# ChicyChen/LOCO-Edit

Measured on AMD Instinct MI355X. Metric: edit-directions/sec (top-5 PMP-Jacobian SVD @256^2) + vT cos-sim vs ref, higher is better.
Workload: dtype bf16x3 (split-bf16 MFMA operands, fp32 accumulate + fp32 storage); 1 GPU; CelebA-HQ DDPM 256x256 top-5 local basis (l_eye-sized mask, L=2400), t=0.6T, 12 power iterations, one GPU; multi_gpu_form=single, probes_total=5, probes_per_gpu=5, kept=5, n_iter=12, mask_L=2400, weights=synthetic seed 0, streams=2

## Files before the change

include/loco_hip_diag.h:

```cpp
#ifndef LOCO_HIP_DIAG_H
#define LOCO_HIP_DIAG_H
#include "loco_hip.h"
#ifdef __cplusplus
extern "C" {
#endif

int  loco_bench_conv(loco_ctx* ctx, int32_t cin, int32_t cout, int32_t H, int32_t W, int32_t B, int32_t mode,
                     int32_t taps, int32_t tile, int32_t iters, float* ms_avg, void* stream);

int64_t loco_debug_tensor(loco_ctx* ctx, const char* name, float* dst, int64_t cap, void* stream);

#ifdef __cplusplus
}
#endif
#endif
```

loco-edit_amd/csrc/conv_bf16.hip:

```cpp
#include "kernels.h"
#include <cstdio>
#include <cstdlib>

namespace loco {

enum : int { PR_BF16X3 = 0, PR_F16 = 1 };
template <int PR, int TAPS, int MODE> void launch_tile_b(const ConvArgs& a, hipStream_t st);
template <int PR, int MODE> void launch_kcat_b(const ConvArgs& a, hipStream_t st);
template <int PR, int MODE> void launch_pair_b(const ConvArgs& a, hipStream_t st);
template <int PR, int MODE> void launch_dual_b(const ConvArgs& a, hipStream_t st);
void launch_conv_gemm(const ConvArgs& a, hipStream_t st);

template <int PR>
static void launch_lowp(const ConvArgs& a, int taps, hipStream_t st) {
#ifdef LOCO_DIAG
    if (a.cot_d && (taps != 1 || a.gemm || a.nsplit > 1 || a.Cin2 > 0 || (a.Cout % conv_bf16_tile_couts(a)) != 0 || a.st_kind == ST_TAN || a.st_kind == ST_COT)) {
        fprintf(stderr, "loco: ConvArgs::cot_d on a launch whose epilogue has no norm-cotangent term (taps %d, gemm %d, nsplit %d, Cout %d, st_kind %d)\n",
                taps, a.gemm, a.nsplit, a.Cout, a.st_kind);
        abort();
    }
#endif
    if constexpr (PR == PR_BF16X3) {
        if (taps == 1 && a.gemm) { launch_conv_gemm(a, st); return; }
    }
    if (taps == 9 && a.Cin2 > 0) {
        if (a.mode == CM_GN_SILU) launch_kcat_b<PR, CM_GN_SILU>(a, st);
        else if (a.mode == CM_GN_GELU) launch_kcat_b<PR, CM_GN_GELU>(a, st);
        else launch_kcat_b<PR, CM_TAN_SILU>(a, st);
        return;
    }
#ifdef LOCO_DIAG
    if constexpr (PR == PR_BF16X3) {
        if (taps == 9 && a.dual) {
            switch (a.mode) {
                case CM_NONE: launch_dual_b<PR, CM_NONE>(a, st); break;
                case CM_GN_SILU: launch_dual_b<PR, CM_GN_SILU>(a, st); break;
                case CM_TAN_SILU: launch_dual_b<PR, CM_TAN_SILU>(a, st); break;
                default: launch_dual_b<PR, CM_COT_SILU>(a, st); break;
            }
            return;
        }
    }
#endif
    if constexpr (PR == PR_BF16X3) {
        if (taps == 9 && a.pair) {
            switch (a.mode) {
                case CM_NONE: launch_pair_b<PR, CM_NONE>(a, st); break;
                case CM_GN_SILU: launch_pair_b<PR, CM_GN_SILU>(a, st); break;
                case CM_TAN_SILU: launch_pair_b<PR, CM_TAN_SILU>(a, st); break;
                default: launch_pair_b<PR, CM_COT_SILU>(a, st); break;
            }
            return;
        }
    }
    if (taps == 9) {
        switch (a.mode) {
            case CM_NONE: launch_tile_b<PR, 9, CM_NONE>(a, st); break;
            case CM_GN_SILU: launch_tile_b<PR, 9, CM_GN_SILU>(a, st); break;
            case CM_GN_GELU: launch_tile_b<PR, 9, CM_GN_GELU>(a, st); break;
            case CM_TAN_SILU: launch_tile_b<PR, 9, CM_TAN_SILU>(a, st); break;
            case CM_COT_SILU: launch_tile_b<PR, 9, CM_COT_SILU>(a, st); break;
            default: launch_tile_b<PR, 9, CM_GN>(a, st); break;
        }
    } else {
        switch (a.mode) {
            case CM_NONE: launch_tile_b<PR, 1, CM_NONE>(a, st); break;
            default: launch_tile_b<PR, 1, CM_GN>(a, st); break;
        }
    }
}
void launch_conv_bf16x3(const ConvArgs& a, int taps, hipStream_t st) { launch_lowp<PR_BF16X3>(a, taps, st); }
void launch_conv_f16(const ConvArgs& a, int taps, hipStream_t st) { launch_lowp<PR_F16>(a, taps, st); }

}
```

loco-edit_amd/csrc/conv_bf16_kernel.h:

```cpp
#pragma once
#include "kernels.h"
#include <cstdlib>
#include <type_traits>

namespace loco {


typedef float f32x16 __attribute__((ext_vector_type(16)));
typedef float f32x4 __attribute__((ext_vector_type(4)));
typedef f32x4 f32x4_u __attribute__((aligned(4)));
typedef float f32x2 __attribute__((ext_vector_type(2)));
typedef f32x2 f32x2_u __attribute__((aligned(4)));
typedef __bf16 bf16x8 __attribute__((ext_vector_type(8)));
typedef _Float16 f16x8 __attribute__((ext_vector_type(8)));
typedef short s16x8 __attribute__((ext_vector_type(8)));

enum : int { PR_BF16X3 = 0, PR_F16 = 1 };

constexpr int BKC = 16;
constexpr bool LIVE_MASK = true;
constexpr bool EARLY_W = true;
constexpr int NDUMMY = 8;

__device__ __forceinline__ float sigmoidf2_(float y) { return __builtin_amdgcn_rcpf(1.0f + __expf(-y)); }

__device__ __forceinline__ int idiv_small(int n, int d) {
    int q = (int)((float)n * __builtin_amdgcn_rcpf((float)d));
    const int r = n - q * d;
    q += (r >= d) ? 1 : ((r < 0) ? -1 : 0);
    return q;
}
__device__ __forceinline__ void idivmod_small(int n, int d, int& q, int& r) { q = idiv_small(n, d); r = n - q * d; }

template <int PR>
__device__ __forceinline__ int rec_off(int p, int q) {
    if constexpr (PR == PR_F16) return p * 32 + ((q ^ ((p >> 3) & 1)) << 4);
    else return p * 64 + ((q ^ ((p >> 2) & 3)) << 4);
}
template <int PR> constexpr int halo_pitch() { return PR == PR_F16 ? 48 : 80; }
template <int PR> constexpr int rec_bytes() { return PR == PR_F16 ? 32 : 64; }
template <int PR>
__device__ __forceinline__ int hrec_off(int p, int q) { return p * halo_pitch<PR>() + (q << 4); }

template <int PR>
__device__ __forceinline__ void cvt2(float a, float b, unsigned& hi, unsigned& lo) {
    if constexpr (PR == PR_F16) {
        _Float16 ha = (_Float16)a, hb = (_Float16)b;
        hi = (unsigned)__builtin_bit_cast(unsigned short, ha) | ((unsigned)__builtin_bit_cast(unsigned short, hb) << 16);
        lo = 0;
    } else {
        typedef float f32x2_ __attribute__((ext_vector_type(2)));
        typedef __bf16 bf16x2_ __attribute__((ext_vector_type(2)));
        hi = __builtin_bit_cast(unsigned, __builtin_convertvector((f32x2_){a, b}, bf16x2_));
        const float ha = __builtin_bit_cast(float, hi << 16), hb = __builtin_bit_cast(float, hi & 0xffff0000u);
        float da = a - ha;
        asm volatile("" : "+v"(da));
        const float db = b - hb;
        lo = __builtin_bit_cast(unsigned, __builtin_convertvector((f32x2_){da, db}, bf16x2_));
    }
}

template <int PR>
__device__ __forceinline__ void split8(const float* v, uint4& hi, uint4& lo) {
    cvt2<PR>(v[0], v[1], hi.x, lo.x);
    cvt2<PR>(v[2], v[3], hi.y, lo.y);
    cvt2<PR>(v[4], v[5], hi.z, lo.z);
    cvt2<PR>(v[6], v[7], hi.w, lo.w);
}

constexpr int max_halo(int NT, int taps, bool s2) {
    if (taps == 1) return NT;
    if (NT >= 128) {
        int th = NT / 32;
        return s2 ? (2 * th + 1) * 65 : (th + 2) * 34;
    }
    return s2 ? 5 * 65 : 4 * 34;
}

constexpr int rs_steps(int n, int lw) { int s = 0; while ((1 << s) < lw && (n >> s) > 1) ++s; return s; }
template <int N, int M, int LW>
__device__ __forceinline__ void rs_reduce(float* av, const int lane) {
    if constexpr (M < LW && N > 1) {
        constexpr int H = N / 2;
        const bool up = (lane & M) != 0;
#pragma unroll
        for (int i = 0; i < H; ++i) {
            const float keep = up ? av[i + H] : av[i];
            const float send = up ? av[i] : av[i + H];
            av[i] = keep + __shfl_xor(send, M, 64);
        }
        rs_reduce<H, M * 2, LW>(av, lane);
    } else if constexpr (M < LW) {
#pragma unroll
        for (int i = 0; i < N; ++i) av[i] += __shfl_xor(av[i], M, 64);
        rs_reduce<N, M * 2, LW>(av, lane);
    }
}

constexpr int EPI_COT1 = 1, EPI_STATS = 2;
template <int WM, int WN, int TM, int TN, int EPI = EPI_STATS, class StageRound>
__device__ __forceinline__ void conv_lowp_epilogue_staged(const ConvArgs& a, StageRound&& stage_round, unsigned char* smem_b, const int co0,
                                                          const int oy0, const int ox0, const int TW, const int tile_id, const int b,
                                                          const int split);
template <int WM, int WN, int TM, int TN>
__device__ __forceinline__ void conv_lowp_epilogue_direct(const ConvArgs& a, f32x16 (&acc)[TM][TN], const int co0, const int oy0,
                                                          const int ox0, const int TW, const int b, const int split);
template <int WM, int WN, int TM, int TN, int EPI = EPI_STATS>
__device__ __forceinline__ void conv_lowp_epilogue(const ConvArgs& a, f32x16 (&acc)[TM][TN], unsigned char* smem_b, const int co0,
                                                   const int oy0, const int ox0, const int TW, const int tile_id, const int b,
                                                   const int split) {
    constexpr int NT = WN * TN * 32;
    const int lane = threadIdx.x & 63, wave = threadIdx.x >> 6;
    const int l31 = lane & 31, khalf = lane >> 5, wm = wave / WN, wn = wave % WN;
    if (co0 + WM * TM * 32 <= a.Cout) {
        conv_lowp_epilogue_staged<WM, WN, TM, TN, EPI>(a, [&](const int h, float* S) {
#pragma unroll
            for (int j = 0; j < TN; ++j)
#pragma unroll
                for (int r = 0; r < 16; ++r)
                    S[(wm * 32 + (r & 3) + 8 * (r >> 2) + 4 * khalf) * NT + (wn * TN + j) * 32 + l31] = acc[h][j][r];
        }, smem_b, co0, oy0, ox0, TW, tile_id, b, split);
        return;
    }
    conv_lowp_epilogue_direct<WM, WN, TM, TN>(a, acc, co0, oy0, ox0, TW, b, split);
}
template <int WM, int WN, int TM, int TN, int EPI, class StageRound>
__device__ __forceinline__ void conv_lowp_epilogue_staged(const ConvArgs& a, StageRound&& stage_round, unsigned char* smem_b, const int co0,
                                                          const int oy0, const int ox0, const int TW, const int tile_id, const int b,
                                                          const int split) {
    constexpr int NTHR = WM * WN * 64;
    constexpr bool COT1 = (EPI & EPI_COT1) != 0, STATS = (EPI & EPI_STATS) != 0;
    constexpr int MT = WM * TM * 32;
    constexpr int NT = WN * TN * 32;
    const int tid = threadIdx.x;
    const int lane = tid & 63;
    const int wave = tid >> 6;
    const int l31 = lane & 31;
    const int khalf = lane >> 5;
    const int wm = wave / WN, wn = wave % WN;
    const long out_plane = (long)a.Hout * a.Wout;
    {
        constexpr int SROWS = WM * 32, NQ = NT / 4, NTASK = (SROWS * NQ) / NTHR;
        static_assert((SROWS * NQ) % NTHR == 0 && (NQ & (NQ - 1)) == 0, "epilogue task split");
        float* const S = reinterpret_cast<float*>(smem_b);
        const bool part = a.nsplit > 1;
        float* const ob = part ? a.partial + (((long)split * a.B + b) * a.Cout) * out_plane : a.out + (long)b * a.out_bs;
        const float* const rb = (!part && a.res) ? a.res + (long)b * a.res_bs : nullptr;
        const float* const b2 = (!part && a.bias2) ? a.bias2 + (long)b * a.bias2_bs : nullptr;
        const float* const b1 = part ? nullptr : a.bias;
        const bool accu = !part && a.accumulate;
        const int twsh = 31 - __builtin_clz((unsigned)TW);
        const bool lin_st = STATS && (a.st_kind == ST_TAN || a.st_kind == ST_COT) && !part;
        const bool lin_cot = a.st_kind == ST_COT;
        const bool cot_ep = COT1 && a.cot_d && !part && !lin_st;
        const float* const cot_db = cot_ep ? a.cot_d + (long)b * a.cot_d_bs : nullptr;
        const f32x2* const cot_tb = cot_ep ? reinterpret_cast<const f32x2*>(a.cot_tc + (long)b * a.cot_tc_bs) : nullptr;
        constexpr int RSTEP = NTHR / NQ;
        static_assert(NTHR % NQ == 0 && 32 % RSTEP == 0, "epilogue task rows");
        const int row0 = tid / NQ, quad0 = tid & (NQ - 1);
        const unsigned pix0 = (unsigned)((oy0 + ((quad0 * 4) >> twsh)) * a.Wout + ox0 + ((quad0 * 4) & (TW - 1)));
        auto co_of = [&](int h, int q) -> int { return co0 + row0 + (((q * RSTEP) >> 5) * TM + h) * 32 + ((q * RSTEP) & 31); };
        auto off_of = [&](int h, int q) -> unsigned {
            const unsigned crow = (unsigned)((((q * RSTEP) >> 5) * TM + h) * 32 + ((q * RSTEP) & 31));
            return (unsigned)(co0 + row0) * (unsigned)out_plane + pix0 + crow * (unsigned)out_plane;
        };
        constexpr int NV = 2 * TM * NTASK;
        float av[STATS ? NV : 1];
#pragma unroll
        for (int h = 0; h < TM; ++h) {
            if (h > 0) {
                asm volatile("s_waitcnt lgkmcnt(0)" ::: "memory");
                __builtin_amdgcn_s_barrier();
            }
            stage_round(h, S);
            f32x4 xs[(STATS || COT1) ? NTASK : 1][2];
            f32x4 cd[COT1 ? NTASK : 1];
            if constexpr (COT1) {
                if (cot_ep) {
#pragma unroll
                    for (int q = 0; q < NTASK; ++q) {
                        const unsigned o = off_of(h, q);
                        cd[q] = *reinterpret_cast<const f32x4*>(cot_db + o);
                        const f32x4* sp4 = reinterpret_cast<const f32x4*>(a.cot_sx + o);
                        xs[q][0] = sp4[0];
                        xs[q][1] = sp4[1];
                    }
                }
            }
            if constexpr (STATS) if (lin_st) {
#pragma unroll
                for (int q = 0; q < NTASK; ++q) {
                    const unsigned o = off_of(h, q);
                    if (lin_cot) {
                        const f32x4* sp4 = reinterpret_cast<const f32x4*>(a.st_sx + o);
                        xs[q][0] = sp4[0];
                        xs[q][1] = sp4[1];
                    } else {
                        xs[q][0] = *reinterpret_cast<const f32x4*>(a.st_x + o);
                    }
                }
            }
            asm volatile("s_waitcnt lgkmcnt(0)" ::: "memory");
            __builtin_amdgcn_s_barrier();
            f32x4 v[NTASK], rv[NTASK];
#pragma unroll
            for (int q = 0; q < NTASK; ++q) v[q] = *reinterpret_cast<const f32x4*>(&S[(q * RSTEP + row0) * NT + quad0 * 4]);
            if (rb || accu) {
#pragma unroll
                for (int q = 0; q < NTASK; ++q) {
                    f32x4 t4 = {0.f, 0.f, 0.f, 0.f};
                    if (rb) t4 = a.res_scale * *reinterpret_cast<const f32x4*>(rb + off_of(h, q));
                    if (accu) t4 += *reinterpret_cast<const f32x4*>(ob + off_of(h, q));
                    rv[q] = t4;
                }
#pragma unroll
                for (int q = 0; q < NTASK; ++q) v[q] += rv[q];
            }
            if constexpr (COT1) {
                if (cot_ep) {
#pragma unroll
                    for (int q = 0; q < NTASK; ++q) {
                        const f32x2 tc2 = cot_tb[co_of(h, q)];
                        const float c1 = tc2[0], c2 = tc2[1];
                        v[q][0] += fmaf(xs[q][0][0], cd[q][0], -fmaf(xs[q][0][1], c2, c1));
                        v[q][1] += fmaf(xs[q][0][2], cd[q][1], -fmaf(xs[q][0][3], c2, c1));
                        v[q][2] += fmaf(xs[q][1][0], cd[q][2], -fmaf(xs[q][1][1], c2, c1));
                        v[q][3] += fmaf(xs[q][1][2], cd[q][3], -fmaf(xs[q][1][3], c2, c1));
                    }
                }
            }
#pragma unroll
            for (int q = 0; q < NTASK; ++q) {
                float add = 0.f;
                if (b1) add += b1[co_of(h, q)];
                if (b2) add += b2[co_of(h, q)];
                v[q] += add;
                __builtin_nontemporal_store(v[q], reinterpret_cast<f32x4*>(ob + off_of(h, q)));
            }
            if constexpr (STATS) if (lin_st) {
#pragma unroll
                for (int q = 0; q < NTASK; ++q) {
                    const f32x4 vv = v[q];
                    float s1, s2;
                    if (!lin_cot) {
                        const f32x4 xv = xs[q][0];
                        s1 = (vv[0] + vv[1]) + (vv[2] + vv[3]);
                        s2 = fmaf(xv[0], vv[0], xv[1] * vv[1]) + fmaf(xv[2], vv[2], xv[3] * vv[3]);
                    } else {
                        const float z0 = xs[q][0][0] * vv[0], z1 = xs[q][0][2] * vv[1], z2 = xs[q][1][0] * vv[2], z3 = xs[q][1][2] * vv[3];
                        s1 = (z0 + z1) + (z2 + z3);
                        s2 = fmaf(xs[q][0][1], z0, xs[q][0][3] * z1) + fmaf(xs[q][1][1], z2, xs[q][1][3] * z3);
                    }
                    av[(h * NTASK + q) * 2] = s1;
                    av[(h * NTASK + q) * 2 + 1] = s2;
                }
            }
            if (STATS && a.st_kind == ST_FWD && !part) {
                const int ntile = (a.Hout * a.Wout) / NT;
                float* const sp = a.st_part + (long)b * a.Cout * ntile * 2;
#pragma unroll
                for (int q = 0; q < NTASK; ++q) {
                    const float pivot = __shfl(v[q][0], lane & ~(NQ - 1) & 63, 64);
                    const float d0 = v[q][0] - pivot, d1 = v[q][1] - pivot, d2 = v[q][2] - pivot, d3 = v[q][3] - pivot;
                    float s1 = (d0 + d1) + (d2 + d3);
                    float s2 = (d0 * d0 + d1 * d1) + (d2 * d2 + d3 * d3);
#pragma unroll
                    for (int m = 1; m < (NQ < 64 ? NQ : 64); m <<= 1) {
                        s1 += __shfl_xor(s1, m, 64);
                        s2 += __shfl_xor(s2, m, 64);
                    }
                    const float m = s1 * (1.0f / NT);
                    const int t = q * NTHR + tid;
                    if ((t & (NQ - 1)) == 0)
                        *reinterpret_cast<f32x2*>(sp + ((long)co_of(h, q) * ntile + tile_id) * 2) = f32x2{pivot + m, s2 - s1 * m};
                }
            }
        }
        if constexpr (STATS) if (lin_st) {
            constexpr int LW = NQ < 64 ? NQ : 64, STEPS = rs_steps(NV, LW), LEFT = NV >> STEPS;
            static_assert((NV & (NV - 1)) == 0, "row sums per lane");
            rs_reduce<NV, 1, LW>(av, lane);
            const int gl = lane & (LW - 1);
            if (gl < (1 << STEPS)) {
                int base = 0;
#pragma unroll
                for (int sb = 0; sb < STEPS; ++sb) base += ((gl >> sb) & 1) * (NV >> (sb + 1));
                const int ntile = (a.Hout * a.Wout) / NT;
                float* const sp = a.st_part + (long)b * a.Cout * ntile * 2;
#pragma unroll
                for (int i = 0; i < LEFT; ++i) {
                    const int idx = base + i, hq = idx >> 1;
                    const int h = hq / NTASK, q = hq - h * NTASK;
                    const int row = (q * NTHR + tid) / NQ;
                    const int co = co0 + ((row >> 5) * TM + h) * 32 + (row & 31);
                    sp[((long)co * ntile + tile_id) * 2 + (idx & 1)] = av[i];
                }
            }
        }
    }
}
template <int WM, int WN, int TM, int TN>
__device__ __forceinline__ void conv_lowp_epilogue_direct(const ConvArgs& a, f32x16 (&acc)[TM][TN], const int co0, const int oy0,
                                                          const int ox0, const int TW, const int b, const int split) {
    const int lane = threadIdx.x & 63, wave = threadIdx.x >> 6;
    const int l31 = lane & 31, khalf = lane >> 5, wm = wave / WN, wn = wave % WN;
    const long out_plane = (long)a.Hout * a.Wout;
    const bool full_co = false;
#pragma unroll
    for (int j = 0; j < TN; ++j) {
        int p = (wn * TN + j) * 32 + l31;
        int ty = p / TW, tx = p - ty * TW;
        int oy = oy0 + ty, ox = ox0 + tx;
        const unsigned pix = (unsigned)(oy * a.Wout + ox);
#pragma unroll
        for (int i = 0; i < TM; ++i) {
            const int cob = co0 + (wm * TM + i) * 32 + 4 * khalf;
            if (a.nsplit > 1) {
                float* pb = a.partial + (((long)split * a.B + b) * a.Cout) * out_plane;
#pragma unroll
                for (int r = 0; r < 16; ++r) {
                    int co = cob + (r & 3) + 8 * (r >> 2);
                    if (full_co || co < a.Cout) pb[(long)co * out_plane + pix] = acc[i][j][r];
                }
            } else {
                float* ob = a.out + (long)b * a.out_bs;
                const float* rb = a.res ? a.res + (long)b * a.res_bs : nullptr;
                const float* b2 = a.bias2 ? a.bias2 + (long)b * a.bias2_bs : nullptr;
                if (rb || a.accumulate) {
                    float rv[16];
#pragma unroll
                    for (int r = 0; r < 16; ++r) {
                        int co = cob + (r & 3) + 8 * (r >> 2);
                        const bool ok = full_co || co < a.Cout;
                        const long off = (long)(ok ? co : a.Cout - 1) * out_plane + pix;
                        float t = 0.f;
                        if (rb) t = a.res_scale * rb[off];
                        if (a.accumulate) t += ob[off];
                        rv[r] = t;
                    }
#pragma unroll
                    for (int r = 0; r < 16; ++r) {
                        int co = cob + (r & 3) + 8 * (r >> 2);
                        if (!(full_co || co < a.Cout)) continue;
                        float v = acc[i][j][r] + rv[r];
                        if (a.bias) v += a.bias[co];
                        if (b2) v += b2[co];
                        __builtin_nontemporal_store(v, &ob[(long)co * out_plane + pix]);
                    }
                } else {
#pragma unroll
                    for (int r = 0; r < 16; ++r) {
                        int co = cob + (r & 3) + 8 * (r >> 2);
                        if (!(full_co || co < a.Cout)) continue;
                        float v = acc[i][j][r];
                        if (a.bias) v += a.bias[co];
                        if (b2) v += b2[co];
                        __builtin_nontemporal_store(v, &ob[(long)co * out_plane + pix]);
                    }
                }
            }
        }
    }
}

template <int WM, int WN, int TM, int TN, int RPW>
__device__ __forceinline__ void conv_lowp_epilogue_rounds(const ConvArgs& a, f32x16 (&acc)[TM][TN], float* const S, const int co0,
                                                          const int oy0, const int ox0, const int TW, const int tile_id, const int b) {
    constexpr int NTHR = WM * WN * 64, NT = WN * TN * 32, NQ = NT / 4;
    constexpr int SROWS = WM * RPW, NTASK = (SROWS * NQ) / NTHR, NRB = RPW / 8;
    static_assert((RPW == 8 || RPW == 16 || RPW == 32) && (SROWS * NQ) % NTHR == 0 && NQ == 64, "round geometry");
    const int tid = threadIdx.x, lane = tid & 63, wave = tid >> 6;
    const int l31 = lane & 31, khalf = lane >> 5;
    const int wm = wave / WN, wn = wave % WN;
    const unsigned out_plane = (unsigned)(a.Hout * a.Wout);
    float* const ob = a.out + (long)b * a.out_bs;
    const float* const rb = a.res ? a.res + (long)b * a.res_bs : nullptr;
    const float* const b2 = a.bias2 ? a.bias2 + (long)b * a.bias2_bs : nullptr;
    const bool accu = a.accumulate != 0;
    const int twsh = TW == 32 ? 5 : (TW == 16 ? 4 : 3);
    const int ntile = (a.Hout * a.Wout) / NT;
    float* const sp = (a.st_kind == ST_FWD) ? a.st_part + (long)b * a.Cout * ntile * 2 : nullptr;
#pragma unroll
    for (int h = 0; h < TM; ++h) {
#pragma unroll
        for (int g0 = 0; g0 < 4; g0 += NRB) {
#pragma unroll
            for (int j = 0; j < TN; ++j)
#pragma unroll
                for (int g = 0; g < NRB; ++g)
#pragma unroll
// ... 1015 lines not shown
```

loco-edit_amd/csrc/conv_plan.hip:

```cpp
#include "kernels.h"
#include <cstdio>
#include <cstdlib>

namespace loco {

constexpr int BKC = 16;
constexpr int BKF = 8;

static const int kMT[7] = {128, 128, 32, 64, 128, 128, 128}, kNT[7] = {128, 64, 128, 64, 256, 256, 128};

static int env_int(const char* name, int dflt) {
    const char* e = getenv(name);
    return e ? atoi(e) : dflt;
}
static int diag_switch(const char* name) {
#ifdef LOCO_DIAG
    return env_int(name, 0);
#else
    (void)name;
    return 0;
#endif
}

static int pick_tile(int Cout, int HW) {
    if (HW >= 128) return Cout > 32 ? 0 : 2;
    return Cout > 64 ? 1 : 3;
}

static int conv_pick_nsplit(int Cin, int Cout, int Hout, int Wout, int B) {
    const int t = pick_tile(Cout, Hout * Wout);
    long blocks = (long)((Hout * Wout) / kNT[t]) * ((Cout + kMT[t] - 1) / kMT[t]) * B;
    int nchunks = (Cin + BKF - 1) / BKF;
    if (blocks >= 384 || nchunks < 8) return 1;
    int want = (int)((512 + blocks - 1) / blocks);
    int maxs = nchunks / 4;
    if (want > maxs) want = maxs;
    if (want > 32) want = 32;
    return want < 1 ? 1 : want;
}

static int conv_bf16_pick_tile(int Cout, int HW, int B, int tile_override) {
    if (B <= 1 && HW <= 1024 && HW >= 64 && (Cout % 64) == 0) return 3;
    int t = pick_tile(Cout, HW);
    if (t == 0 && HW >= 256) {
        if (tile_override >= 0) return tile_override;
        return 5;
    }
    return t;
}

constexpr int kTile0MaxHW = 65536;

static int bf16_tile_of(const ConvArgs& a, int tile_override = -1) {
    static const bool two_per_cu = diag_switch("LOCO_CONV_2WG") != 0;
    int tile = conv_bf16_pick_tile(a.Cout, a.Hout * a.Wout, a.B, tile_override);
    if (tile == 4) tile = 5;
    if (tile == 5 && a.taps == 1 && !a.gemm && a.B >= 2 && a.Hout * a.Wout <= kTile0MaxHW) return 0;
    if (tile == 5 && two_per_cu && a.taps == 9 && a.stride == 1 && !a.upsample && !a.zins && (a.Cin % BKC) == 0 &&
        a.in_padded && a.pad == 1 && a.Wout >= 32) return 6;
    if (a.stride == 2 && tile == 5) tile = 0;
    return tile;
}
static int tile_for(const ConvArgs& a, int prec, int tile_override) {
    return prec ? bf16_tile_of(a, tile_override) : pick_tile(a.Cout, a.Hout * a.Wout);
}
static int conv_bf16_tile_pixels(const ConvArgs& a) { return a.gemm ? 256 : kNT[a.tile]; }
int conv_bf16_tile_couts(const ConvArgs& a) { return a.gemm ? 64 * a.gemm_tm : kMT[a.tile]; }

static int conv_bf16_pick_nsplit(int Cin, int Cout, int Hout, int Wout, int B, int chip_share, int taps, int lanes) {
    const int HW = Hout * Wout;
    int t = conv_bf16_pick_tile(Cout, HW, B, -1);
    if (t == 4) t = 5;
    if (taps == 1 && t == 5 && B >= 2 && HW <= kTile0MaxHW) t = 0;
    long blocks = (long)(HW / kNT[t]) * ((Cout + kMT[t] - 1) / kMT[t]) * B;
    int nchunks = (Cin + BKC - 1) / BKC;
    int target = chip_share > 1 ? 256 / chip_share : (lanes == 2 ? 240 : 256);
    if (target < 32) target = 32;
    if (blocks >= target / 2 || nchunks < 8) return 1;
    int want = (int)(target / blocks);
    int maxs = nchunks / 4;
    if (want > maxs) want = maxs;
    if (want > 32) want = 32;
    return want < 1 ? 1 : want;
}

static bool conv_lowp_can_kcat(const ConvArgs& a) {
    static const bool on = env_int("LOCO_KCAT", 1) != 0;
    return on && a.Cin2 > 0 && a.nsplit == 1 && bf16_tile_of(a) == 5 && a.stride == 1 && !a.upsample && !a.zins && a.pad == 1 &&
           (a.Cin % BKC) == 0 && (a.Cin2 % BKC) == 0 && a.in_padded &&
           (a.mode == CM_GN_SILU || a.mode == CM_GN_GELU || a.mode == CM_TAN_SILU);
}
static bool conv_lowp_can_fuse_stats(const ConvArgs& a) {
    return a.nsplit <= 1 && !a.gemm && (a.Cout % conv_bf16_tile_couts(a)) == 0;
}

static bool conv_pair_ok(const ConvArgs& a) {
    static const bool on = env_int("LOCO_CONV_PAIR", 1) != 0;
    if (!on || a.Hout * a.Wout < 16384 || a.taps != 9 || a.Cin2 > 0 || a.nsplit != 1 || a.stride != 1 || a.upsample || a.zins ||
        a.pad != 1 || !a.in_padded || (a.Cin % (2 * BKC)) != 0 || (a.Cout % 128) != 0 || (a.Wout % 32) != 0 || (a.Hout % 8) != 0 ||
        a.pers_groups || a.dual)
        return false;
    if (!(a.mode == CM_NONE || a.mode == CM_GN_SILU || a.mode == CM_TAN_SILU || a.mode == CM_COT_SILU)) return false;
    return a.tile == 5;
}

static bool conv_dual_ok(const ConvArgs& a) {
    static const bool on = diag_switch("LOCO_CONV_DUAL") != 0;
    if (!on || a.taps != 9 || a.Cin2 > 0 || a.nsplit != 1 || a.stride != 1 || a.upsample || a.zins || a.pad != 1 || (a.Cin % BKC) != 0 ||
        !a.in_padded || a.Wout < 32 || (a.Wout % 32) != 0 || (a.Hout % 8) != 0 || (a.Cout % 128) != 0 || a.B < 2 || a.cot_d)
        return false;
    if (!(a.mode == CM_NONE || a.mode == CM_GN_SILU || a.mode == CM_TAN_SILU || a.mode == CM_COT_SILU)) return false;
    if (a.tile != 5) return false;
    const long units = (long)((a.Hout * a.Wout) / 256) * (a.Cout / 128) * (a.B / 2);
    return units >= 192;
}

static ConvArgs conv_shift_batch(const ConvArgs& a, int nb) {
    ConvArgs t = a;
    t.B = a.B - nb;
    t.in += (long)nb * a.in_bs; t.out += (long)nb * a.out_bs;
    if (t.prim) t.prim += (long)nb * a.prim_bs;
    if (t.bias2) t.bias2 += (long)nb * a.bias2_bs;
    if (t.res) t.res += (long)nb * a.res_bs;
    if (t.sc) { t.sc += (long)nb * a.scsh_bs; t.sh += (long)nb * a.scsh_bs; }
    if (t.mr) t.mr += (long)nb * a.mr_bs;
    if (t.tst) t.tst += (long)nb * a.tst_bs;
    if (t.tc) t.tc += (long)nb * a.tc_bs;
    if (t.in2) t.in2 += (long)nb * a.in2_bs;
    if (t.cot_d) { t.cot_d += (long)nb * a.cot_d_bs; t.cot_tc += (long)nb * a.cot_tc_bs; }
    if (t.st_part) t.st_part += (long)nb * a.Cout * ((a.Hout * a.Wout) / conv_bf16_tile_pixels(a)) * 2;
    return t;
}

static void conv_pers_plan(ConvArgs& a) {
    a.pers_groups = 0;
    static const int on = diag_switch("LOCO_CONV_PERS");
    if (!on || a.taps != 9 || a.Cin2 > 0 || a.nsplit != 1 || a.stride != 1 || a.upsample || a.zins || a.pad != 1 || !a.in_padded ||
        (a.Cin % (2 * BKC)) != 0 || (a.Cout % 128) != 0 || a.B < 2 || a.cot_d || bf16_tile_of(a) != 5)
        return;
    if (!(a.mode == CM_NONE || a.mode == CM_GN_SILU || a.mode == CM_GN_GELU ||
          (on == 2 && (a.mode == CM_TAN_SILU || a.mode == CM_COT_SILU)))) return;
    const long wg0 = (long)((a.Hout * a.Wout) / 256) * (a.Cout / 128);
    int G = wg0 >= 256 ? 1 : (int)(256 / wg0);
    if (G > a.B) G = a.B;
    const int per = (a.B + G - 1) / G;
    if (per < 2 || a.B * 10 < G * per * 8 || wg0 * G < 192) return;
    a.pers_groups = G;
}

static void conv_gemm_plan(ConvArgs& a) {
    static const bool on = env_int("LOCO_CONV_GEMM", 1) != 0;
    a.gemm = 0;
    const long HW = (long)a.Hout * a.Wout;
    if (!on || a.stride != 1 || a.upsample || a.zins || (a.Cin % BKC) != 0 || a.Cin < 320 || (HW % 256) != 0 || (a.Wout % 16) != 0 ||
        a.Cout < 128 || !a.partial || a.Cin2 > 0 || !(a.mode == CM_NONE || a.mode == CM_GN) || a.cot_d)
        return;
    {
        const int TW = a.Wout < 32 ? a.Wout : 32;
        if ((256 % TW) != 0 || (a.Wout % TW) != 0 || (a.Hout % (256 / TW)) != 0) return;
    }
    static const int all_shapes = env_int("LOCO_GEMM_ALL", 0);
    if (!all_shapes && !(a.Cout >= 640 && (a.Cout >= 4 * a.Cin || a.Cin >= 2560))) return;
    const int pad256 = (a.Cout + 255) / 256 * 256;
    const int tm = (pad256 * 10 <= a.Cout * 11) ? 4 : 2;
    const int mt = 64 * tm;
    const long tiles = (HW / 256) * ((a.Cout + mt - 1) / mt) * a.B;
    const size_t rec_floats = (size_t)a.B * a.Cin * HW;
    int ns = 1;
    if (tiles < 192) {
        const int nchunks = a.Cin / BKC;
        ns = (int)((256 + tiles - 1) / tiles);
        if (ns > 8) ns = 8;
        while (ns > 1 && nchunks / ns < 8) --ns;
        while (ns > 1 && (size_t)ns * a.B * a.Cout * HW + rec_floats > a.partial_floats) --ns;
    }
    if ((ns > 1 ? (size_t)ns * a.B * a.Cout * HW : 0) + rec_floats > a.partial_floats) return;
    a.gemm = 1; a.gemm_tm = tm; a.nsplit = ns;
}

void conv_plan_family(ConvArgs& a, int prec) {
    if (prec == 1 && a.taps == 1) conv_gemm_plan(a);
    if (prec == 1 && a.taps == 9) conv_pers_plan(a);
}

int conv_plan_parts(ConvArgs& a, int prec, int tile_override, ConvArgs parts[2]) {
    a.dual = 0;
    a.tile = tile_for(a, prec, tile_override);
    a.pair = 0;
    parts[0] = a;
    int n = 1;
    if (prec == 1 && a.taps == 9 && conv_dual_ok(a)) {
        parts[0].B = a.B & ~1;
        parts[0].dual = 1;
        if (a.B & 1) {
            parts[1] = conv_shift_batch(a, a.B - 1);
            parts[1].pers_groups = 0;
            n = 2;
        }
    }
    for (int i = 0; i < n; ++i) {
        ConvArgs& p = parts[i];
        p.tile = tile_for(p, prec, tile_override);
        p.pair = prec == 1 && conv_pair_ok(p);
    }
    return n;
}

static bool short_tail(long per_probe, int B) {
    const long total = per_probe * B, r = total % 256;
    return total > 256 && r > 0 && r <= 160;
}

static int tail_split(const ConvArgs& a, size_t partial_floats, int* split) {
    const long per_probe = (long)((a.Hout * a.Wout) / conv_bf16_tile_pixels(a)) * ((a.Cout + 127) / 128);
    const long r = per_probe * a.B % 256;
    if (!short_tail(per_probe, a.B) || per_probe <= 0 || r % per_probe != 0 || r / per_probe >= a.B) return 0;
    int s = (int)(256 / r);
    if (s > 4) s = 4;
    const int nchunks = (a.Cin + 15) / 16;
    while (s > 1 && nchunks / s < 4) --s;
    const size_t one = (size_t)(r / per_probe) * a.Cout * a.Hout * a.Wout;
    while (s > 1 && (size_t)s * one > partial_floats) --s;
    *split = s;
    return s > 1 ? (int)(r / per_probe) : 0;
}

static int stats_route(const ConvEnv& e, const StatAsk* q, bool want, ConvArgs& x, int s0, int B, int* keep_ntile) {
    if (!q || q->kind == ST_NONE) return SR_NONE;
    const int alone = q->norm ? SR_ALONE : SR_NONE;
    if (!want) return alone;
    if (x.nsplit > 1) return !q->norm ? SR_NONE : ((x.Hout * x.Wout) % 4 == 0 ? SR_SPLITK : SR_ALONE);
    const int ntile = (x.Hout * x.Wout) / conv_bf16_tile_pixels(x);
    const size_t need = (size_t)x.B * x.Cout * ntile * 2;
    const int epi = q->norm ? SR_EPI : SR_KEEP;
    const bool kept = q->keep && s0 == 0 && x.B == B && need <= q->keep_floats;
    if (q->kind == ST_FWD && conv_lowp_can_fuse_stats(x) && (kept || (q->norm && need <= e.stpart_floats))) {
        x.st_part = kept ? q->keep : e.stpart; x.st_kind = ST_FWD;
        if (kept) *keep_ntile = ntile;
        return epi;
    }
    const bool cot_cache = q->kind == ST_COT && q->norm && q->sx;
    if ((q->kind == ST_TAN || cot_cache) && e.fuse_lin && !x.cot_d && conv_lowp_can_fuse_stats(x) && !x.pers_groups &&
        !conv_dual_ok(x)) {
        const size_t lane_off = (size_t)e.lane_s0 * (q->keep_floats / e.max_batch);
        const bool keptl = q->kind == ST_TAN && q->keep && s0 == 0 && x.B == B && lane_off + need <= q->keep_floats;
        if (keptl || (q->norm && need <= e.stpart_floats)) {
            x.st_part = keptl ? q->keep + lane_off : e.stpart; x.st_kind = q->kind; x.st_x = q->prim;
            if (q->kind == ST_COT) x.st_sx = q->sx;
            if (keptl) *keep_ntile = ntile;
            return epi;
        }
    }
    return alone;
}

static ConvLaunch plan_launch(const ConvEnv& e, const StatAsk* q, bool want, const ConvArgs& x, int s0, int B, int* keep_ntile) {
    ConvLaunch l;
    l.args = x;
    l.s0 = s0;
    l.args.tile = tile_for(x, e.prec, -1);
    l.stats = stats_route(e, q, want, l.args, s0, B, keep_ntile);
    if (l.stats == SR_EPI || l.stats == SR_KEEP) l.ntile = (x.Hout * x.Wout) / conv_bf16_tile_pixels(l.args);
    l.nparts = conv_plan_parts(l.args, e.prec, -1, l.parts);
    return l;
}

ConvPlan plan_conv(const ConvEnv& e, const ConvArgs& a0, int taps, const StatAsk* q, const ConvArgs* sc) {
    ConvPlan p;
    ConvArgs a = a0;
    a.taps = taps;
    a.dual = 0; a.pers_groups = 0; a.gemm = 0;
    if (sc) {
        ConvArgs t = a;
        t.nsplit = e.prec >= 1 ? conv_bf16_pick_nsplit(a.Cin, a.Cout, a.Hout, a.Wout, a.B, e.chip_share, 9, e.lanes) : 2;
        t.in2 = sc->in; t.in2_bs = sc->in_bs; t.Cin2 = sc->Cin;
        const long per_probe = (long)((a.Hout * a.Wout) / 256) * ((a.Cout + 127) / 128);
        if (e.prec >= 1 && taps == 9 && !short_tail(per_probe, a.B) && !a.bias2 && conv_lowp_can_kcat(t)) {
            a.in2 = sc->in; a.in2_bs = sc->in_bs; a.Cin2 = sc->Cin; a.in2_padded = sc->in_padded;
            a.wb2 = e.prec == 2 ? sc->wh : sc->wb;
            a.bias2 = sc->bias; a.bias2_bs = 0;
            a.res = nullptr;
        } else {
            p.sc_first = true;
            a.res = sc->out; a.res_bs = sc->out_bs;
        }
    }
    if (e.prec == 2) a.wb = a.wh;
    a.no_deep = e.deep1 ? 0 : 1;
    a.nsplit = e.prec >= 1 ? conv_bf16_pick_nsplit(a.Cin, a.Cout, a.Hout, a.Wout, a.B, e.chip_share, taps, e.lanes)
                           : conv_pick_nsplit(a.Cin, a.Cout, a.Hout, a.Wout, a.B);
    if (a.cot_d) {
        ConvArgs t = a;
        t.tile = bf16_tile_of(t);
        const long per_probe = (long)((a.Hout * a.Wout) / conv_bf16_tile_pixels(t)) * ((a.Cout + 127) / 128);
        p.cot = e.prec >= 1 && taps == 1 && a.nsplit == 1 && !short_tail(per_probe, a.B) && conv_lowp_can_fuse_stats(t);
        if (!p.cot) { a.cot_d = nullptr; a.cot_d_bs = 0; a.cot_sx = nullptr; a.cot_tc = nullptr; a.cot_tc_bs = 0; }
    }
    while (a.nsplit > 1 && (size_t)a.nsplit * a.B * a.Cout * a.Hout * a.Wout > e.partial_floats) a.nsplit >>= 1;
    if (a.nsplit < 1) a.nsplit = 1;
    a.partial = e.partial;
    a.partial_floats = e.partial_floats;
    conv_plan_family(a, e.prec);
    a.tile = tile_for(a, e.prec, -1);
    int split = 1;
    const int tail = e.prec >= 1 && a.nsplit == 1 && a.B >= 2 && !a.gemm && !a.pers_groups ? tail_split(a, e.partial_floats, &split) : 0;
    const bool want = q && q->kind != ST_NONE && e.prec >= 1 && e.fuse_stats;
    if (!tail) {
        p.l[0] = plan_launch(e, q, want, a, 0, a.B, &p.keep_ntile);
        return p;
    }
    const bool per_part = want && q->norm && (q->kind == ST_FWD || (e.fuse_lin && (a.Hout * a.Wout) % 4 == 0));
    p.stats_all = !per_part && q && q->kind != ST_NONE && q->norm;
    const StatAsk* ql = per_part ? q : nullptr;
    const int nb = a.B - tail;
    ConvArgs m = a, t = conv_shift_batch(a, nb);
    m.B = nb;
    t.nsplit = split;
    p.nl = 2;
    p.l[0] = plan_launch(e, ql, want, m, 0, a.B, &p.keep_ntile);
    p.l[1] = plan_launch(e, ql, want, t, nb, a.B, &p.keep_ntile);
    return p;
}

const char* conv_variant_name(const ConvArgs& a, int taps, int prec) {
    static const char* tiles[6] = {"2,2,2,2", "4,1,1,2", "1,4,1,1", "2,2,1,1", "2,2,2,4", "2,4,2,2"};
    static char names[3][2][6][6][56];
    static char others[5][3][6][40];
    const int mode = (a.mode < 0 || a.mode > 5) ? 2 : a.mode;
    const char* other = nullptr;
    int k = 0, v = mode;
    if (prec && taps == 9 && a.Cin2 > 0) other = prec == 1 ? "conv_kcat_bf16x3<2,4,2,2,%d>" : "conv_kcat_f16<2,4,2,2,%d>";
    else if (prec == 1 && taps == 1 && a.gemm) { k = 1; other = "conv_gemm_bf16x3<%d>"; v = a.gemm_tm; }
    else if (prec == 1 && taps == 9 && a.pers_groups > 0 && !a.dual) { k = 2; other = "conv_pers_bf16x3<9,2,4,2,2,%d>"; }
    else if (prec == 1 && taps == 9 && a.pair) { k = 3; other = "conv_pair_bf16x3<%d>"; }
    else if (prec == 1 && taps == 9 && a.dual) { k = 4; other = "conv_dual_bf16x3<%d>"; }
    if (other) {
        char* n = others[k][prec][v];
        if (!n[0]) snprintf(n, 40, other, v);
        return n;
    }
    int t = a.tile == 6 ? 0 : a.tile;
    if (t < 0 || t > 5) t = 0;
    int m = mode;
    if (taps != 9 && m != CM_NONE) m = CM_GN;
    if (!prec && m == CM_GN_GELU) m = CM_GN_SILU;
    char* n = names[prec][taps == 9 ? 0 : 1][t][m];
    static const char* kn[3] = {"conv_mfma_f32", "conv_mfma_bf16x3", "conv_mfma_f16"};
    if (!n[0]) snprintf(n, 56, "%s<%d,%s,%d>", kn[prec], taps, tiles[t], m);
    return n;
}

}
```

loco-edit_amd/csrc/engine.hip:

```cpp
#include <hip/hip_runtime.h>

#include <algorithm>
#include <array>
#include <cmath>
#include <cstdio>
#include <cstdlib>
#include <cstring>
#include <map>
#include <memory>
#include <thread>
#include <atomic>
#include <string>
#include <vector>

#include "../../include/loco_hip.h"
#ifdef LOCO_DIAG
#include "../../include/loco_hip_diag.h"
#endif
#include "kernels.h"
#include "program.h"

using namespace loco;


#define HIPCHK(ctx, call)                                                                    \
    do {                                                                                     \
        hipError_t e_ = (call);                                                              \
        if (e_ != hipSuccess) {                                                              \
            (ctx)->err = std::string(#call) + ": " + hipGetErrorString(e_);                  \
            return -1;                                                                       \
        }                                                                                    \
    } while (0)

namespace {

struct ConvP {
    float* wf = nullptr;
    float* wd = nullptr;
    float* wbf = nullptr;
    float* wbd = nullptr;
    float* whf = nullptr;
    float* whd = nullptr;
    float* bias = nullptr;
    int cin = 0, cout = 0, taps = 0;
};
struct NormW { float* gamma = nullptr; float* beta = nullptr; };

struct OpWeights {
    ConvP c1, c2, nin, qkvc, proj, conv;
    ConvP xqc, xproj;
    ConvP pj_in, to_out1, to_out2, ff1, ff2, pj_out;
    NormW g1, g2, gx;
    float *xkw = nullptr, *xkb = nullptr, *xvw = nullptr, *xvb = nullptr;
    float *xng = nullptr, *xnb = nullptr;
    float *lng[3] = {nullptr, nullptr, nullptr}, *lnb[3] = {nullptr, nullptr, nullptr};
    long tproj_off = 0;
};
struct Weights {
    std::vector<OpWeights> op;
    float *freq = nullptr, *td0w = nullptr, *td0b = nullptr, *td1w = nullptr, *td1b = nullptr;
    float *tp_w = nullptr, *tp_b = nullptr;
    long tproj_total = 0;
    double flops = 0.0;
};

struct Tens : TensPlan {
    float* keep = nullptr; size_t keep_floats = 0; int keep_ntile = 0;
};
struct NormP : NormPlan, NormW {
    bool ready = false;
};
struct Op : OpPlan, OpWeights {
    NormP n1, n2, nx;
    float *xK = nullptr, *xV = nullptr;
};

struct HostParam { std::vector<float> data; std::vector<int64_t> shape; bool loaded = false; };

}


struct loco_ctx {
    loco_unet_cfg cfg;
    std::string err;
    std::map<std::string, HostParam> params;
    bool finalized = false;

    std::shared_ptr<const Program> prog;
    std::shared_ptr<Weights> wts;
    std::vector<Tens> tens;
    std::vector<Op> ops;


    float *arenaP = nullptr, *arenaT = nullptr;
    float *statsP = nullptr, *statsT = nullptr;
    double* red = nullptr;
    bool fuse_cot = true;
    float *stpart = nullptr, *stpart2 = nullptr;
    size_t stpart_floats = 0;
    bool fuse_stats = true;
    bool fuse_xattn = true;
    bool deep1 = true;
    bool flash_attn = true;
    float* attn_delta = nullptr;
    float* partial = nullptr;
    size_t partial_floats = 0;
    const float* bench_out = nullptr; int64_t bench_out_count = 0;
    float *tact = nullptr, *tproj = nullptr;
    float* eps_buf = nullptr;
    float* gx0 = nullptr;
    float* ge = nullptr;
    float* tmpA = nullptr;
    double *G = nullptr, *Q = nullptr, *W = nullptr, *gscratch = nullptr;
    float* alphas = nullptr;
    float* ctx_colbias = nullptr;
    bool has_ctx = false;
    float* cond_add = nullptr;
    float* ctx_norm = nullptr;
    bool has_cond = false;
    float2* sxcache = nullptr;
    int prec = 0;
    std::vector<float*> owned;
    size_t bytes = 0;

    bool primal_ok = false;
    float p_cv = 0.f, p_ce = 0.f;
    uint8_t* mask = nullptr;
    bool has_mask = false;
    uint8_t* mask2 = nullptr;
    bool has_mask2 = false;
    int mask2_from = 0;
    int* mask_idx = nullptr;
    int* mask_L_dev = nullptr;
    long mask_L = 0;
    hipStream_t mask_stream = nullptr;
    int primal_B = 0;
    hipEvent_t ev0 = nullptr, ev1 = nullptr;
    int n_streams = 1;
    hipStream_t st2 = nullptr;
    hipStream_t st2_user = nullptr;
    hipEvent_t ev_fork = nullptr, ev_join = nullptr;
    double* red2 = nullptr;
    struct FwdGraph { hipGraph_t graph = nullptr; hipGraphExec_t exec = nullptr; int calls = 0; };
    std::map<int, FwdGraph> fwd_graphs;
    bool graph_on = false;
    bool gemm_lowp = true;
    unsigned char* gemm_ws[2] = {nullptr, nullptr}; size_t gemm_ws_bytes[2] = {0, 0}; int lane = 0;
    loco_ctx* weights_of = nullptr;
    int forks = 0;
    bool zombie = false;
    bool fuse_lin = true;
    int lanes_active = 1;
    int lane_s0 = 0;
    int chip_share = 1;
    hipStream_t cap_st = nullptr;
    float* xin_buf = nullptr;
    float* t_dev = nullptr;
    bool prof_on = false;
    struct ProfRec { const char* name; double flops; hipEvent_t e0, e1; int cin, cout, h, b, ns, mode, taps; };
    bool prof_shapes = false;
    std::vector<ProfRec> prof;
    std::vector<hipEvent_t> ev_pool;
    size_t ev_used = 0;
    hipEvent_t next_event() {
        if (ev_used == ev_pool.size()) {
            hipEvent_t e; (void)hipEventCreate(&e); ev_pool.push_back(e);
        }
        return ev_pool[ev_used++];
    }
};

namespace {

template <typename T>
int dalloc(loco_ctx* c, T** p, size_t count) {
    void* q = nullptr;
    HIPCHK(c, hipMalloc(&q, count * sizeof(T)));
    *p = reinterpret_cast<T*>(q);
    c->owned.push_back(reinterpret_cast<float*>(q));
    c->bytes += count * sizeof(T);
    return 0;
}

inline float eps_of(const loco_ctx* c, const NormP& n) { return n.eps > 0.f ? n.eps : c->cfg.gn_eps; }


int upload(loco_ctx* c, float** dst, const std::vector<float>& h) {
    if (dalloc(c, dst, h.size() ? h.size() : 1)) return -1;
    HIPCHK(c, hipMemcpy(*dst, h.data(), h.size() * sizeof(float), hipMemcpyHostToDevice));
    return 0;
}

static inline uint16_t f2bf(float f) {
    uint32_t u; std::memcpy(&u, &f, 4);
    u += 0x7FFFu + ((u >> 16) & 1u);
    return (uint16_t)(u >> 16);
}
static inline float bf2f(uint16_t h) {
    uint32_t u = (uint32_t)h << 16; float f; std::memcpy(&f, &u, 4); return f;
}
template <typename F>
static void parallel_for(int n, size_t work, F fn) {
    unsigned nt = std::thread::hardware_concurrency();
    if (nt > 16) nt = 16;
    if ((int)nt > n) nt = (unsigned)n;
    if (nt <= 1 || work < ((size_t)1 << 18)) { for (int i = 0; i < n; ++i) fn(i); return; }
    std::atomic<int> next{0};
    std::vector<std::thread> th;
    for (unsigned t = 0; t < nt; ++t)
        th.emplace_back([&]() { int i; while ((i = next.fetch_add(1)) < n) fn(i); });
    for (auto& t : th) t.join();
}

template <typename F>
static std::vector<float> build_records(int nin, int nout, int taps, F get) {
    int nch = (nin + 15) / 16, noutP = (nout + 31) & ~31;
    std::vector<uint16_t> rec((size_t)nch * taps * noutP * 32, 0);
    parallel_for(nch, (size_t)nin * nout * taps, [&](int ck) {
        for (int t = 0; t < taps; ++t)
            for (int o = 0; o < nout; ++o) {
                uint16_t* r = rec.data() + (((size_t)ck * taps + t) * noutP + o) * 32;
                int sw = (o >> 2) & 3;
                for (int k = 0; k < 16; ++k) {
                    int i = ck * 16 + k;
                    float v = (i < nin) ? get(o, i, t) : 0.f;
                    uint16_t h = f2bf(v);
                    uint16_t l = f2bf(v - bf2f(h));
                    int qh = (k >> 3) ^ sw, ql = (2 + (k >> 3)) ^ sw;
                    r[qh * 8 + (k & 7)] = h;
                    r[ql * 8 + (k & 7)] = l;
                }
            }
    });
    std::vector<float> out(rec.size() / 2);
    std::memcpy(out.data(), rec.data(), rec.size() * 2);
    return out;
}

template <typename F>
static std::vector<float> build_records_f16(int nin, int nout, int taps, F get) {
    int nch = (nin + 15) / 16, noutP = (nout + 31) & ~31;
    std::vector<_Float16> rec((size_t)nch * taps * noutP * 16, (_Float16)0.f);
    parallel_for(nch, (size_t)nin * nout * taps, [&](int ck) {
        for (int t = 0; t < taps; ++t)
            for (int o = 0; o < nout; ++o) {
                _Float16* r = rec.data() + (((size_t)ck * taps + t) * noutP + o) * 16;
                int sw = (o >> 3) & 1;
                for (int k = 0; k < 16; ++k) {
                    int i = ck * 16 + k;
                    float v = (i < nin) ? get(o, i, t) : 0.f;
                    r[((k >> 3) ^ sw) * 8 + (k & 7)] = (_Float16)v;
                }
            }
    });
    std::vector<float> out(rec.size() / 2);
    std::memcpy(out.data(), rec.data(), rec.size() * 2);
    return out;
}

int make_conv(loco_ctx* c, const std::vector<const HostParam*>& ws, const std::vector<const HostParam*>& bs,
              ConvP* out, int row_limit = -1) {
    int cin = (int)ws[0]->shape[1], k = ws[0]->shape.size() > 2 ? (int)ws[0]->shape[2] : 1;
    int taps = ws[0]->shape.size() == 4 ? k * k : k;
    int cout = 0;
    for (auto* w : ws) cout += (int)w->shape[0];
    if (row_limit > 0 && ws.size() == 1 && row_limit < cout) cout = row_limit;
    int coutP = (cout + 31) & ~31, cinP = (cin + 31) & ~31;
    std::vector<float> wf((size_t)cin * taps * coutP, 0.f), wd((size_t)cout * taps * cinP, 0.f), bias(cout);
    int co0 = 0;
    for (size_t wi = 0; wi < ws.size(); ++wi) {
        const HostParam* w = ws[wi];
        int co_n = (int)w->shape[0];
        if (co_n > cout - co0) co_n = cout - co0;
        parallel_for(co_n, (size_t)co_n * cin * taps, [&](int co) {
            for (int ci = 0; ci < cin; ++ci)
                for (int t = 0; t < taps; ++t)
                    wd[((size_t)(co0 + co) * taps + (taps - 1 - t)) * cinP + ci] = w->data[((size_t)co * cin + ci) * taps + t];
        });
        parallel_for(cin, (size_t)co_n * cin * taps, [&](int ci) {
            for (int t = 0; t < taps; ++t)
                for (int co = 0; co < co_n; ++co)
                    wf[((size_t)ci * taps + t) * coutP + co0 + co] = w->data[((size_t)co * cin + ci) * taps + t];
        });
        for (int co = 0; co < co_n; ++co) bias[co0 + co] = bs[wi]->data[co];
        co0 += co_n;
    }
    out->cin = cin; out->cout = cout; out->taps = taps;
    if (upload(c, &out->wf, wf) || upload(c, &out->wd, wd) || upload(c, &out->bias, bias)) return -1;
    auto fwd = [&](int o, int i, int t) { return wf[((size_t)i * taps + t) * coutP + o]; };
    auto dgr = [&](int o, int i, int t) { return wd[((size_t)i * taps + t) * cinP + o]; };
    std::vector<float> rf = build_records(cin, cout, taps, fwd);
    std::vector<float> rd = build_records(cout, cin, taps, dgr);
    if (upload(c, &out->wbf, rf) || upload(c, &out->wbd, rd)) return -1;
    std::vector<float> hf = build_records_f16(cin, cout, taps, fwd);
    std::vector<float> hd = build_records_f16(cout, cin, taps, dgr);
    if (upload(c, &out->whf, hf) || upload(c, &out->whd, hd)) return -1;
    return 0;
}
int make_conv1(loco_ctx* c, const std::string& name, ConvP* out, int row_limit = -1) {
    return make_conv(c, {&c->params[name + ".weight"]}, {&c->params[name + ".bias"]}, out, row_limit);
}
int make_conv1_scaled(loco_ctx* c, const std::string& name, ConvP* out, float s) {
    if (s == 1.f) return make_conv1(c, name, out);
    HostParam w = c->params[name + ".weight"], b = c->params[name + ".bias"];
    for (float& v : w.data) v *= s;
    for (float& v : b.data) v *= s;
    return make_conv(c, {&w}, {&b}, out);
}
int make_norm(loco_ctx* c, const std::string& name, NormW* n) {
    if (upload(c, &n->gamma, c->params[name + ".weight"].data)) return -1;
    if (upload(c, &n->beta, c->params[name + ".bias"].data)) return -1;
    return 0;
}

int bind_weights(loco_ctx* c) {
    const Weights& W = *c->wts;
    for (size_t i = 0; i < c->ops.size(); ++i) {
        Op& v = c->ops[i];
        static_cast<OpWeights&>(v) = W.op[i];
        static_cast<NormW&>(v.n1) = v.g1; static_cast<NormW&>(v.n2) = v.g2; static_cast<NormW&>(v.nx) = v.gx;
    }
    if (dalloc(c, &c->tact, (size_t)c->cfg.ch * 4) || dalloc(c, &c->tproj, (size_t)(W.tproj_total > 0 ? W.tproj_total : 1))) return -1;
    c->finalized = true;
    return 0;
}

int finalize_params(loco_ctx* c) {
    if (c->finalized) return 0;
    for (const ParamDecl& d : c->prog->params)
        if (!c->params[d.name].loaded) { c->err = "parameter not loaded: " + d.name; return -1; }
    Weights& W = *c->wts;
    const loco_unet_cfg& cfg = c->cfg;
    int temb_ch = cfg.ch * 4;
    const bool adm = cfg.arch == 1;
    const std::string te0 = adm ? "time_embed.0" : "temb.dense.0", te1 = adm ? "time_embed.2" : "temb.dense.1";
    if (cfg.arch < 2) {
        if (upload(c, &W.td0w, c->params[te0 + ".weight"].data)) return -1;
        if (upload(c, &W.td0b, c->params[te0 + ".bias"].data)) return -1;
        if (upload(c, &W.td1w, c->params[te1 + ".weight"].data)) return -1;
        if (upload(c, &W.td1b, c->params[te1 + ".bias"].data)) return -1;
    }
    {
        int half = cfg.ch / 2;
        std::vector<float> f(half);
        for (int i = 0; i < half; ++i) {
            float x;
            if (adm) x = ((float)(-std::log(10000.0)) * (float)i) / (float)half;
            else x = (float)i * (float)(-(std::log(10000.0) / (double)(half - 1)));
            f[i] = (float)std::exp((double)x);
        }
        if (upload(c, &W.freq, f)) return -1;
    }
    std::vector<float> tpw, tpb;
    for (size_t oi = 0; oi < W.op.size(); ++oi) {
        const OpPlan& op = c->prog->ops[oi];
        OpWeights& ow = W.op[oi];
        switch (op.kind) {
            case OP_CONV_IN: case OP_CONV: if (make_conv1(c, op.pn_conv, &ow.conv)) return -1; break;
            case OP_RES: {
                if (make_norm(c, op.pn_n1, &ow.g1) || make_norm(c, op.pn_n2, &ow.g2)) return -1;
                if (make_conv1(c, op.pn_c1, &ow.c1) || make_conv1_scaled(c, op.pn_c2, &ow.c2, c->prog->res_scale)) return -1;
                if (op.has_nin && make_conv1_scaled(c, op.pn_skip, &ow.nin, c->prog->res_scale)) return -1;
                if (!op.has_temb) break;
                ow.tproj_off = (long)tpb.size();
                auto& w = c->params[op.pn_emb + ".weight"].data;
                auto& b = c->params[op.pn_emb + ".bias"].data;
                tpw.insert(tpw.end(), w.begin(), w.end());
                tpb.insert(tpb.end(), b.begin(), b.end());
                break;
            }
            case OP_ATTN: {
                if (make_norm(c, op.pn_n1, &ow.g1)) return -1;
                if (adm) {
                    if (make_conv1(c, op.pn_qkv, &ow.qkvc)) return -1;
                } else if (make_conv(c, {&c->params[op.name + ".q.weight"], &c->params[op.name + ".k.weight"],
                                         &c->params[op.name + ".v.weight"]},
                                     {&c->params[op.name + ".q.bias"], &c->params[op.name + ".k.bias"],
                                      &c->params[op.name + ".v.bias"]}, &ow.qkvc)) return -1;
                if (make_conv1(c, op.pn_proj, &ow.proj)) return -1;
                if (op.added_kv) {
                    const int C = c->tens[op.in].C, NH = op.heads, CH = C / NH, D = c->cfg.context_dim;
                    const HostParam& w = c->params[op.name + ".encoder_kv.weight"];
                    const HostParam& b = c->params[op.name + ".encoder_kv.bias"];
                    std::vector<float> kw((size_t)C * D), vw((size_t)C * D), kb(C), vb(C);
                    for (int h = 0; h < NH; ++h)
                        for (int i = 0; i < CH; ++i) {
                            const size_t rk = (size_t)h * 2 * CH + i, rv = rk + CH, r = (size_t)h * CH + i;
                            std::copy(w.data.begin() + rk * D, w.data.begin() + (rk + 1) * D, kw.begin() + r * D);
                            std::copy(w.data.begin() + rv * D, w.data.begin() + (rv + 1) * D, vw.begin() + r * D);
                            kb[r] = b.data[rk]; vb[r] = b.data[rv];
                        }
                    if (upload(c, &ow.xkw, kw) || upload(c, &ow.xkb, kb) || upload(c, &ow.xvw, vw) || upload(c, &ow.xvb, vb) ||
                        upload(c, &ow.xng, c->params[op.name + ".norm_encoder.weight"].data) ||
                        upload(c, &ow.xnb, c->params[op.name + ".norm_encoder.bias"].data)) return -1;
                }
                if (op.has_x) {
                    const std::string x = op.name + ".xattn";
                    if (make_norm(c, x + ".norm", &ow.gx) || make_conv1(c, x + ".q", &ow.xqc) ||
                        make_conv1(c, x + ".proj_out", &ow.xproj)) return -1;
                    if (upload(c, &ow.xkw, c->params[x + ".k.weight"].data) || upload(c, &ow.xkb, c->params[x + ".k.bias"].data) ||
                        upload(c, &ow.xvw, c->params[x + ".v.weight"].data) || upload(c, &ow.xvb, c->params[x + ".v.bias"].data))
                        return -1;
                }
                break;
            }
            case OP_DOWN: case OP_UP: if (make_conv1(c, op.pn_conv, &ow.conv)) return -1; break;
            case OP_XFMR: {
                const int C = c->tens[op.in].C, NH = op.heads, CH = C / NH;
                const std::string b = op.name + ".transformer_blocks.0";
                HostParam zb; zb.shape = {8 * C}; zb.data.assign((size_t)8 * C, 0.f);
                auto nobias = [&](const std::string& w, ConvP* out) { return make_conv(c, {&c->params[w + ".weight"]}, {&zb}, out); };
                if (make_norm(c, op.pn_n1, &ow.g1) || make_conv1(c, op.name + ".proj_in", &ow.pj_in) ||
                    make_conv1(c, op.name + ".proj_out", &ow.pj_out)) return -1;
                const char* lnn[3] = {".norm1", ".norm2", ".norm3"};
                for (int i = 0; i < 3; ++i)
                    if (upload(c, &ow.lng[i], c->params[b + lnn[i] + ".weight"].data) ||
                        upload(c, &ow.lnb[i], c->params[b + lnn[i] + ".bias"].data)) return -1;
                {
                    HostParam w; w.shape = {3 * C, C}; w.data.resize((size_t)3 * C * C);
                    const char* nm[3] = {".attn1.to_q.weight", ".attn1.to_k.weight", ".attn1.to_v.weight"};
                    for (int which = 0; which < 3; ++which) {
                        const std::vector<float>& src = c->params[b + nm[which]].data;
                        for (int h = 0; h < NH; ++h)
                            for (int j = 0; j < CH; ++j)
                                std::memcpy(&w.data[((size_t)(h * 3 + which) * CH + j) * C], &src[(size_t)(h * CH + j) * C], (size_t)C * 4);
                    }
                    if (make_conv(c, {&w}, {&zb}, &ow.qkvc)) return -1;
                }
                if (make_conv1(c, b + ".attn1.to_out.0", &ow.to_out1) || nobias(b + ".attn2.to_q", &ow.xqc) ||
                    make_conv1(c, b + ".attn2.to_out.0", &ow.to_out2) || make_conv1(c, b + ".ff.net.0.proj", &ow.ff1) ||
                    make_conv1(c, b + ".ff.net.2", &ow.ff2)) return -1;
                std::vector<float> z0((size_t)C, 0.f);
                if (upload(c, &ow.xkw, c->params[b + ".attn2.to_k.weight"].data) || upload(c, &ow.xkb, z0) ||
                    upload(c, &ow.xvw, c->params[b + ".attn2.to_v.weight"].data) || upload(c, &ow.xvb, z0)) return -1;
                break;
            }
            case OP_OUT:
                if (make_norm(c, op.pn_n1, &ow.g1) || make_conv1(c, op.pn_conv, &ow.conv, cfg.out_ch)) return -1;
                break;
        }
    }
    W.tproj_total = (long)tpb.size();
    if (upload(c, &W.tp_w, tpw) || upload(c, &W.tp_b, tpb)) return -1;
    double fl = 0.0;
    for (size_t oi = 0; oi < W.op.size(); ++oi) {
        const OpPlan& op = c->prog->ops[oi];
        const OpWeights& ow = W.op[oi];
        auto convf = [&](const ConvP& p, int H, int W) { fl += 2.0 * p.cin * p.cout * p.taps * (double)H * W; };
        const Tens& to = c->tens[op.out];
        switch (op.kind) {
            case OP_CONV_IN: case OP_CONV: case OP_DOWN: case OP_UP: case OP_OUT: convf(ow.conv, to.H, to.W); break;
            case OP_RES:
                convf(ow.c1, to.H, to.W); convf(ow.c2, to.H, to.W);
                if (op.has_nin) convf(ow.nin, to.H, to.W);
                break;
            case OP_XFMR: {
                for (const ConvP* p : {&ow.pj_in, &ow.qkvc, &ow.to_out1, &ow.xqc, &ow.to_out2, &ow.ff1, &ow.ff2, &ow.pj_out}) convf(*p, to.H, to.W);
                double T = (double)to.H * to.W;
                fl += 2.0 * 2.0 * T * T * to.C + 2.0 * 2.0 * T * c->cfg.context_len * to.C;
                break;
            }
            case OP_ATTN: {
                convf(ow.qkvc, to.H, to.W); convf(ow.proj, to.H, to.W);
                double T = (double)to.H * to.W;
                fl += 2.0 * 2.0 * T * T * to.C;
                if (op.has_x) {
                    convf(ow.xqc, to.H, to.W); convf(ow.xproj, to.H, to.W);
                    fl += 2.0 * 2.0 * T * c->cfg.context_len * to.C;
                }
                break;
            }
        }
    }
    W.flops = fl;
    for (auto& kv : c->params) { std::vector<float>().swap(kv.second.data); }
    return bind_weights(c);
}

struct Pass {
    loco_ctx* c;
    hipStream_t st;
    int B;
    float* arena;
    float* stats;
    float* T(int id) const { return arena + c->tens[id].off; }
    long bs() const { return c->prog->per_sample; }
};

static void drop_graphs(loco_ctx* c) {
    for (auto& kv : c->fwd_graphs) {
        if (kv.second.exec) (void)hipGraphExecDestroy(kv.second.exec);
        if (kv.second.graph) (void)hipGraphDestroy(kv.second.graph);
    }
    c->fwd_graphs.clear();
}
inline unsigned char* gemm_ws_get(loco_ctx* c, size_t need, hipStream_t st) {
    const int l = c->lane;
    if (c->gemm_ws_bytes[l] >= need) return c->gemm_ws[l];
    hipStreamCaptureStatus cs = hipStreamCaptureStatusNone;
    if (hipStreamIsCapturing(st, &cs) != hipSuccess || cs != hipStreamCaptureStatusNone) return nullptr;
    if (c->gemm_ws[l]) {
        (void)hipDeviceSynchronize();
        drop_graphs(c);
        (void)hipFree(c->gemm_ws[l]);
        c->bytes -= c->gemm_ws_bytes[l];
        c->gemm_ws[l] = nullptr; c->gemm_ws_bytes[l] = 0;
    }
    void* p = nullptr;
    if (hipMalloc(&p, need) != hipSuccess) { (void)hipGetLastError(); return nullptr; }
    c->gemm_ws[l] = static_cast<unsigned char*>(p); c->gemm_ws_bytes[l] = need; c->bytes += need;
    return c->gemm_ws[l];
}
inline bool attn_gemm_rec(const loco_ctx* c, const GemmArgs& g) { return c->prec >= 1 && c->gemm_lowp && gemm_rec_eligible(g); }
inline void attn_gemm(loco_ctx* c, const GemmArgs& g, hipStream_t st) {
    if (attn_gemm_rec(c, g)) {
        if (unsigned char* ws = gemm_ws_get(c, gemm_rec_ws_bytes(g), st)) { launch_gemm_rec(g, ws, st); return; }
    }
    if (c->prec >= 1 && c->gemm_lowp && gemm_prefers_bf16x3(g)) launch_gemm_bf16x3(g, st); else launch_gemm(g, st);
}

void conv_defaults(ConvArgs& a) {
    std::memset(&a, 0, sizeof(a));
    a.stride = 1; a.pad = 1; a.nsplit = 1; a.mode = CM_NONE; a.res_scale = 1.f;
}

struct NS { float *sc, *sh, *mr, *tst, *tc; };
NS nstats(const loco_ctx* c, float* base, const NormP& n) {
    NS s;
    s.sc = base + n.soff; s.sh = s.sc + n.C; s.mr = s.sh + n.C; s.tst = s.mr + 2 * c->cfg.gn_groups;
    s.tc = s.tst + 2 * c->cfg.gn_groups;
    return s;
}

struct StatReq {
    int kind = ST_NONE;
    NormP* n = nullptr;
    float* stats = nullptr;
    const float* prim = nullptr;
    const float* ss_scale = nullptr; const float* ss_shift = nullptr;
    float* keep = nullptr; size_t keep_floats = 0; int* keep_ntile = nullptr;
};

void stats_standalone(loco_ctx* c, const StatReq& rq, const float* x, long xbs, int B, int HW, int s0, hipStream_t st) {
    const NormP& n = *rq.n;
    const long SB = c->prog->stats_per_sample;
    const int G = c->cfg.gn_groups;
    if (rq.kind == ST_FWD) {
        NS s = nstats(c, rq.stats + (long)s0 * SB, n);
        launch_gn_stats(x, xbs, B, n.C, HW, G, eps_of(c, n), n.gamma, n.beta, s.mr, s.sc, s.sh, SB, c->red, st, rq.ss_scale,
                        rq.ss_shift);
    } else {
        NS sp = nstats(c, c->statsP, n);
        NS stt = nstats(c, rq.stats + (long)s0 * SB, n);
        launch_gn_tstats(x, xbs, rq.prim, 0, B, n.C, HW, G, sp.sc, sp.sh, sp.mr, 0, 0, rq.kind == ST_TAN ? 0 : 1, stt.tst,
                         stt.tc, SB, c->red, st, c->cfg.act);
    }
}

bool run_conv(loco_ctx* c, const ConvArgs& a0, int taps, hipStream_t st, const StatReq* rq = nullptr,
              const ConvArgs* second = nullptr) {
    const size_t span = (size_t)c->cfg.max_batch * c->prog->per_sample;
    auto padded = [&](const float* p) { return (p >= c->arenaP && p < c->arenaP + span) || (p >= c->arenaT && p < c->arenaT + span); };
    ConvArgs a = a0, sc;
    a.act = c->cfg.act;
    if (a.mode == CM_GN_SILU && c->cfg.act == ACT_GELU) a.mode = CM_GN_GELU;
    a.in_padded = padded(a.in);
    if (second) { sc = *second; sc.in_padded = padded(sc.in); }
    ConvEnv e;
    e.prec = c->prec; e.chip_share = c->chip_share; e.lanes = c->lanes_active; e.lane_s0 = c->lane_s0;
    e.partial = c->partial; e.partial_floats = c->partial_floats; e.stpart = c->stpart; e.stpart_floats = c->stpart_floats;
    e.fuse_stats = c->fuse_stats; e.fuse_lin = c->fuse_lin; e.deep1 = c->deep1; e.max_batch = c->cfg.max_batch;
    StatAsk q;
    if (rq) {
        q.kind = rq->kind; q.norm = rq->n != nullptr; q.prim = rq->prim; q.keep = rq->keep; q.keep_floats = rq->keep_floats;
        if (rq->n && rq->n->sx_off >= 0 && c->sxcache) q.sx = c->sxcache + rq->n->sx_off;
    }
    const ConvPlan p = plan_conv(e, a, taps, rq ? &q : nullptr, second ? &sc : nullptr);
    if (p.sc_first) run_conv(c, *second, 1, st);
    if (rq && rq->kind != ST_NONE && rq->n) rq->n->ready = true;
    if (rq && rq->keep_ntile) *rq->keep_ntile = p.keep_ntile;
    const int HWo = a.Hout * a.Wout, Gn = c->cfg.gn_groups;
    const long SBs = c->prog->stats_per_sample;
    auto timed = [&](const char* name, double flops, const ConvArgs& y, auto&& launch) {
        loco_ctx::ProfRec r;
        if (c->prof_on) {
            r.name = name; r.flops = flops;
            r.cin = y.Cin; r.cout = y.Cout; r.h = y.Hout; r.b = y.B; r.ns = y.nsplit; r.mode = y.mode; r.taps = taps;
            r.e0 = c->next_event(); r.e1 = c->next_event();
            (void)hipEventRecord(r.e0, st);
        }
        launch();
        if (c->prof_on) { (void)hipEventRecord(r.e1, st); c->prof.push_back(r); }
    };
    for (int li = 0; li < p.nl; ++li) {
        const ConvLaunch& l = p.l[li];
        const ConvArgs& x = l.args;
        for (int pi = 0; pi < l.nparts; ++pi) {
            const ConvArgs& y = l.parts[pi];
            double flops = 2.0 * (y.Cin * taps + y.Cin2) * y.Cout * (double)y.Hout * y.Wout * y.B;
            if (y.zins) flops *= 0.25;
            timed(c->prof_on ? conv_variant_name(y, taps, c->prec) : nullptr, flops, y, [&] {
                if (c->prec == 1) launch_conv_bf16x3(y, taps, st);
                else if (c->prec == 2) launch_conv_f16(y, taps, st);
                else launch_conv(y, taps, st);
            });
        }
        if (x.nsplit > 1) {
            timed("conv_splitk_reduce", 0.0, x, [&] {
                if (l.stats != SR_SPLITK) { launch_conv_splitk_reduce(x, st); return; }
                const NormP& n = *rq->n;
                NS sp = nstats(c, c->statsP, n);
                NS so = nstats(c, rq->stats + (long)l.s0 * SBs, n);
                launch_conv_splitk_reduce_stats(x, rq->kind, Gn, eps_of(c, n), n.gamma, n.beta, so.mr, so.sc, so.sh, SBs, rq->ss_scale,
                                                rq->ss_shift, rq->prim, sp.sc, sp.sh, sp.mr, so.tst, so.tc, SBs, c->red, st);
            });
        }
        if (l.stats == SR_ALONE) stats_standalone(c, *rq, x.out, x.out_bs, x.B, HWo, l.s0, st);
        if (l.stats == SR_EPI) {
            const NormP& n = *rq->n;
            NS so = nstats(c, rq->stats + (long)l.s0 * SBs, n);
            if (rq->kind != ST_FWD) {
                NS sp = nstats(c, c->statsP, n);
                launch_gn_lin_fused_finalize(rq->kind, x.st_part, n.C, l.ntile, nullptr, 0, x.B, n.C, HWo, Gn, sp.mr, so.tst, so.tc,
                                             SBs, st);
            } else {
                launch_gn_fused_finalize(x.st_part, l.ntile, x.B, n.C, HWo, Gn, eps_of(c, n), n.gamma, n.beta, so.mr, so.sc, so.sh,
                                         SBs, rq->ss_scale, rq->ss_shift, st);
            }
        }
    }
    if (p.stats_all) stats_standalone(c, *rq, a.out, a.out_bs, a.B, HWo, 0, st);
    return p.cot;
}

inline void setw(ConvArgs& a, const ConvP& p, bool dgrad) {
    a.w = dgrad ? p.wd : p.wf;
    a.wb = dgrad ? (const void*)p.wbd : (const void*)p.wbf;
    a.wh = dgrad ? (const void*)p.whd : (const void*)p.whf;
}

NormP* consumer_norm(loco_ctx* c, int tid) {
    const Tens& t = c->tens[tid];
    if (t.cons_op < 0) return nullptr;
    Op& op = c->ops[t.cons_op];
    return t.cons_norm == 2 ? &op.nx : &op.n1;
}
StatReq req_fwd(NormP* n, float* stats, const float* ss_scale = nullptr, const float* ss_shift = nullptr) {
    StatReq r;
    if (n) { r.kind = ST_FWD; r.n = n; r.stats = stats; r.ss_scale = ss_scale; r.ss_shift = ss_shift; }
    return r;
}
StatReq req_lin(loco_ctx* c, int kind, NormP* n, const float* prim) {
    StatReq r;
    if (n) { r.kind = kind; r.n = n; r.stats = c->statsT; r.prim = prim; }
    return r;
}
void clear_ready(loco_ctx* c) {
    for (auto& op : c->ops) op.n1.ready = op.n2.ready = op.nx.ready = false;
    for (auto& t : c->tens) t.keep_ntile = 0;
}
StatReq req_fwd_of(loco_ctx* c, int tid, float* stats) {
    StatReq r = req_fwd(consumer_norm(c, tid), stats);
    Tens& t = c->tens[tid];
    if (t.cat_of >= 0 && t.keep) {
        r.kind = ST_FWD; r.stats = stats;
        r.keep = t.keep; r.keep_floats = t.keep_floats; r.keep_ntile = &t.keep_ntile;
    }
    return r;
}
bool cat_fused_stats(loco_ctx* c, const NormP& n, int tid, float* stats, int B, hipStream_t st) {
    const Tens& q = c->tens[tid];
    if (q.cat_a < 0 || c->prec < 1 || !c->fuse_stats) return false;
    const Tens& A = c->tens[q.cat_a];
    const Tens& Bt = c->tens[q.cat_b];
    if (A.keep_ntile <= 0 || Bt.keep_ntile <= 0) return false;
    NS s = nstats(c, stats, n);
    launch_gn_fused_finalize_cat(A.keep, A.C, A.keep_ntile, Bt.keep, Bt.keep_ntile, B, q.C, q.H * q.W, c->cfg.gn_groups,
                                 eps_of(c, n), n.gamma, n.beta, s.mr, s.sc, s.sh, c->prog->stats_per_sample, st);
    return true;
}

bool cat_fused_tstats(loco_ctx* c, const NormP& n, int tid, int B, hipStream_t st) {
    const Tens& q = c->tens[tid];
    if (q.cat_a < 0 || c->prec < 1 || !c->fuse_stats || !c->fuse_lin) return false;
    const Tens& A = c->tens[q.cat_a];
    const Tens& Bt = c->tens[q.cat_b];
    if (A.keep_ntile <= 0 || Bt.keep_ntile <= 0) return false;
    NS sp = nstats(c, c->statsP, n);
    NS stt = nstats(c, c->statsT, n);
    const size_t MB = c->cfg.max_batch;
    launch_gn_lin_fused_finalize(ST_TAN, A.keep + c->lane_s0 * (A.keep_floats / MB), A.C, A.keep_ntile,
                                 Bt.keep + c->lane_s0 * (Bt.keep_floats / MB), Bt.keep_ntile, B, q.C, q.H * q.W,
                                 c->cfg.gn_groups, sp.mr, stt.tst, stt.tc, c->prog->stats_per_sample, st);
    return true;
}

void gn_forward_stats(const Pass& p, const NormP& n, const float* x, long xbs, int HW) {
    NS s = nstats(p.c, p.stats, n);
    launch_gn_stats(x, xbs, p.B, n.C, HW, p.c->cfg.gn_groups, eps_of(p.c, n), n.gamma, n.beta, s.mr, s.sc, s.sh,
                    p.c->prog->stats_per_sample, p.c->red, p.st);
}


struct XA {
    loco_ctx* c; const Op* op; hipStream_t st; int B; int C, T, NH, CH, Lp;
    float scale;
};
XA xa_of(loco_ctx* c, const Op& op, int B, hipStream_t st) {
    XA x; x.c = c; x.op = &op; x.st = st; x.B = B;
    const Tens& t = c->tens[op.in];
    x.C = t.C; x.T = t.H * t.W; x.NH = op.heads; x.CH = x.C / x.NH; x.Lp = c->prog->ctx_Lp;
    x.scale = 1.0f / std::sqrt((float)x.CH);
    return x;
}
void xa_scores(const XA& x, const float* X, long x_bs, const float* K, float* S, long s_bs, float alpha, bool mask) {
    GemmArgs g; std::memset(&g, 0, sizeof(g));
    g.A = X; g.sam = 1; g.sak = x.T; g.sab = x_bs; g.sah = (long)x.CH * x.T;
    g.Bm = K; g.sbk = x.Lp; g.sbn = 1; g.sbb = 0; g.sbh = (long)x.CH * x.Lp;
    g.C = S; g.scm = x.Lp; g.scn = 1; g.scb = s_bs; g.sch = (long)x.T * x.Lp;
    g.M = x.T; g.N = x.Lp; g.K = x.CH; g.batch = x.B; g.batch2 = x.NH; g.alpha = alpha; g.beta = 0.f;
    g.colbias = mask ? x.c->ctx_colbias : nullptr;
    launch_gemm(g, x.st);
}
void xa_values(const XA& x, const float* K, const float* S, long s_bs, float* O, long o_bs) {
    GemmArgs g; std::memset(&g, 0, sizeof(g));
    g.A = K; g.sam = x.Lp; g.sak = 1; g.sab = 0; g.sah = (long)x.CH * x.Lp;
    g.Bm = S; g.sbk = 1; g.sbn = x.Lp; g.sbb = s_bs; g.sbh = (long)x.T * x.Lp;
    g.C = O; g.scm = x.T; g.scn = 1; g.scb = o_bs; g.sch = (long)x.CH * x.T;
    g.M = x.CH; g.N = x.T; g.K = x.Lp; g.batch = x.B; g.batch2 = x.NH; g.alpha = 1.f; g.beta = 0.f;
    launch_gemm(g, x.st);
}
bool xa_fused(const XA& x, int kind, const float* X, long x_bs, const float* K1, const float* K2, float* P, long p_bs,
              float* O, long o_bs) {
    loco_ctx* c = x.c;
    if (!c->fuse_xattn || !xattn_fused_supported(x.T, x.CH, c->cfg.context_len, x.Lp)) return false;
    XAttnArgs a; std::memset(&a, 0, sizeof(a));
    a.T = x.T; a.NH = x.NH; a.B = x.B; a.CH = x.CH; a.L = c->cfg.context_len; a.Lp = x.Lp; a.fwd = kind == 0;
    a.alpha = x.scale; a.X = X; a.x_bs = x_bs; a.K1 = K1; a.K2 = K2; a.P = P; a.p_bs = p_bs; a.O = O; a.o_bs = o_bs;
    launch_xattn_fused(a, x.st);
    return true;
}
void xa_conv1x1(loco_ctx* c, const ConvP& w, bool dgrad, const float* in, long in_bs, float* out, long out_bs, int C, int H,
                int W, int B, const float* res, long res_bs, bool with_bias, hipStream_t st, const StatReq* rq = nullptr) {
    ConvArgs a; conv_defaults(a);
    a.in = in; a.in_bs = in_bs; a.Cin = C; a.Hin = H; a.Win = W;
    setw(a, w, dgrad); a.pad = 0;
    if (with_bias) a.bias = w.bias;
    a.res = res; a.res_bs = res_bs;
    a.out = out; a.out_bs = out_bs; a.Cout = C; a.Hout = H; a.Wout = W; a.B = B;
    run_conv(c, a, 1, st, rq);
}

struct SA { loco_ctx* c; const Op* op; int B, T, NH, CH; hipStream_t st; };
void sa_forward(const SA& s, float* ar) {
    loco_ctx* c = s.c;
    const long PS = c->prog->per_sample, HS = 3L * s.CH * s.T, SS = (long)s.T * s.T;
    float* q = ar + c->tens[s.op->qkv].off; float* k = q + (long)s.CH * s.T; float* v = k + (long)s.CH * s.T;
    float* S = ar + c->tens[s.op->S].off; float* o = ar + c->tens[s.op->o].off;
    GemmArgs g; std::memset(&g, 0, sizeof(g));
    g.A = q; g.sam = 1; g.sak = s.T; g.sab = PS; g.sah = HS;
    g.Bm = k; g.sbk = s.T; g.sbn = 1; g.sbb = PS; g.sbh = HS;
    g.C = S; g.scm = s.T; g.scn = 1; g.scb = PS; g.sch = SS;
    g.M = s.T; g.N = s.T; g.K = s.CH; g.batch = s.B; g.batch2 = s.NH; g.alpha = 1.0f / std::sqrt((float)s.CH); g.beta = 0.f;
    attn_gemm(c, g, s.st);
    launch_softmax_rows(S, (long)s.NH * s.T, s.T, s.st, s.B, PS);
    GemmArgs h; std::memset(&h, 0, sizeof(h));
    h.A = v; h.sam = s.T; h.sak = 1; h.sab = PS; h.sah = HS;
    h.Bm = S; h.sbk = 1; h.sbn = s.T; h.sbb = PS; h.sbh = SS;
    h.C = o; h.scm = s.T; h.scn = 1; h.scb = PS; h.sch = (long)s.CH * s.T;
    h.M = s.CH; h.N = s.T; h.K = s.T; h.batch = s.B; h.batch2 = s.NH; h.alpha = 1.f; h.beta = 0.f;
    attn_gemm(c, h, s.st);
}
void sa_tangent(const SA& s) {
    loco_ctx* c = s.c;
    const int T = s.T, CH = s.CH, NH = s.NH, B = s.B;
    const long PS = c->prog->per_sample, HS = 3L * CH * T, SS = (long)T * T;
    float* q = c->arenaP + c->tens[s.op->qkv].off; float* k = q + (long)CH * T; float* v = k + (long)CH * T;
    float* dq = c->arenaT + c->tens[s.op->qkv].off; float* dk = dq + (long)CH * T; float* dv = dk + (long)CH * T;
    float* SP = c->arenaP + c->tens[s.op->S].off; float* ST = c->arenaT + c->tens[s.op->S].off;
    float* oP = c->arenaP + c->tens[s.op->o].off; float* oT = c->arenaT + c->tens[s.op->o].off;
    const float scale = 1.0f / std::sqrt((float)CH);
    if (c->flash_attn && c->prec >= 1 && attn_flash_supported(T, CH)) {
        AttnFlashArgs fa; std::memset(&fa, 0, sizeof(fa));
        fa.ws = reinterpret_cast<unsigned char*>(c->partial); fa.ws_bytes = c->partial_floats * sizeof(float);
        fa.T = T; fa.NH = NH; fa.B = B; fa.CH = CH; fa.scale = scale; fa.q = q; fa.k = k; fa.v = v; fa.hs = HS; fa.P = SP; fa.o = oP;
        fa.dq = dq; fa.dk = dk; fa.dv = dv; fa.bs_d = PS; fa.out = oT; fa.bs_out = PS;
        launch_attn_flash_tangent(fa, s.st);
        return;
    }
    GemmArgs g; std::memset(&g, 0, sizeof(g));
    g.A = dq; g.sam = 1; g.sak = T; g.sab = PS; g.sah = HS;
// ... 515 lines not shown
                g.C = TT(op.S); g.scm = T; g.scn = 1; g.scb = PS; g.sch = SS;
                g.M = T; g.N = T; g.K = CH; g.batch = B; g.batch2 = NH; g.alpha = 1.f; g.beta = 0.f;
                bool kcat = T <= 256;
                if (!kcat && !flash) { GemmArgs g2 = g; g2.A2 = q; g2.Bm2 = dk; g2.sbb2 = PS; kcat = attn_gemm_rec(c, g2); }
                if (kcat) { g.A2 = q; g.sab2 = 0; g.Bm2 = dk; g.sbb2 = PS; }
                if (!flash) {
                attn_gemm(c, g, st);
                if (!kcat) { g.A = q; g.sab = 0; g.Bm = dk; g.sbb = PS; g.beta = 1.f; attn_gemm(c, g, st); }
                launch_softmax_jac(TT(op.S), TP(op.S), (long)NH * T, T, (long)NH * T, 1.0f / std::sqrt((float)CH), st, B, PS);
                }
                GemmArgs h; std::memset(&h, 0, sizeof(h));
                h.A = dv; h.sam = T; h.sak = 1; h.sab = PS; h.sah = HS;
                h.Bm = TP(op.S); h.sbk = 1; h.sbn = T; h.sbb = 0; h.sbh = SS;
                h.C = TT(op.o); h.scm = T; h.scn = 1; h.scb = PS; h.sch = (long)CH * T;
                h.M = CH; h.N = T; h.K = T; h.batch = B; h.batch2 = NH; h.alpha = 1.f; h.beta = 0.f;
                if (kcat) { h.A2 = v; h.sab2 = 0; h.Bm2 = TT(op.S); h.sbb2 = PS; }
                if (!flash) {
                attn_gemm(c, h, st);
                if (!kcat) { h.A = v; h.sab = 0; h.Bm = TT(op.S); h.sbb = PS; h.beta = 1.f; attn_gemm(c, h, st); }
                }
                ConvArgs pr; conv_defaults(pr);
                pr.in = TT(op.o); pr.in_bs = PS; pr.Cin = C; pr.Hin = to.H; pr.Win = to.W;
                setw(pr, op.proj, false); pr.pad = 0; pr.res = TT(op.in); pr.res_bs = PS;
                pr.out = TT(op.has_x ? op.xmid : op.out); pr.out_bs = PS; pr.Cout = C; pr.Hout = to.H; pr.Wout = to.W; pr.B = B;
                {
                    const StatReq rq = next_tan(op.has_x ? op.xmid : op.out);
                    run_conv(c, pr, 1, st, &rq);
                }
                if (op.has_x) {
                    const XA x = xa_of(c, op, B, st);
                    if (!op.nx.ready) tangent_stats(c, op.nx, TT(op.xmid), PS, TP(op.xmid), HW, B, st);
                    op.nx.ready = false;
                    NS spx = nstats(c, c->statsP, op.nx);
                    NS stx = nstats(c, c->statsT, op.nx);
                    launch_gn_apply(1, TT(op.xmid), PS, TP(op.xmid), 0, nullptr, 0, TT(op.xhn), PS, 0, B, C, HW,
                                    cfg.gn_groups, spx.sc, spx.sh, spx.mr, 0, 0, stx.tst, c->prog->stats_per_sample, st);
                    xa_conv1x1(c, op.xqc, false, TT(op.xhn), PS, TT(op.xq), PS, C, to.H, to.W, B, nullptr, 0, false, st);
                    if (!xa_fused(x, 1, TT(op.xq), PS, op.xK, op.xV, TP(op.xS), 0, TT(op.xo), PS)) {
                        xa_scores(x, TT(op.xq), PS, op.xK, TT(op.xS), PS, 1.f, false);
                        launch_softmax_jac(TT(op.xS), TP(op.xS), (long)NH * T, x.Lp, (long)NH * T, x.scale, st, B, PS);
                        xa_values(x, op.xV, TT(op.xS), PS, TT(op.xo), PS);
                    }
                    const StatReq rqx = next_tan(op.out);
                    xa_conv1x1(c, op.xproj, false, TT(op.xo), PS, TT(op.out), PS, C, to.H, to.W, B, TT(op.xmid), PS, false, st, &rqx);
                }
                break;
            }
            case OP_XFMR: {
                const int C = to.C, T = HW, NH = op.heads, H = to.H, W = to.W;
                auto XP = [&](int i) { return TP(op.xt[i]); };
                auto XT_ = [&](int i) { return TT(op.xt[i]); };
                if (!op.n1.ready) tangent_stats(c, op.n1, TT(op.in), PS, TP(op.in), HW, B, st);
                op.n1.ready = false;
                NS sp = nstats(c, c->statsP, op.n1);
                NS stt = nstats(c, c->statsT, op.n1);
                launch_gn_apply(1, TT(op.in), PS, TP(op.in), 0, nullptr, 0, XT_(X_G0), PS, 0, B, C, HW,
                                cfg.gn_groups, sp.sc, sp.sh, sp.mr, 0, 0, stt.tst, c->prog->stats_per_sample, st);
                lin1x1(c, op.pj_in, false, XT_(X_G0), PS, C, XT_(X_H0), PS, C, H, W, B, nullptr, 0, false, st);
                const SA sa{c, &op, B, T, NH, C / NH, st};
                const XA xa = xa_of(c, op, B, st);
                launch_ln_tan(XT_(X_H0), PS, XP(X_H0), XP(X_LN1), B, C, T, op.lng[0], XT_(X_A1), PS, st);
                lin1x1(c, op.qkvc, false, XT_(X_A1), PS, C, XT_(X_QKV), PS, 3 * C, H, W, B, nullptr, 0, false, st);
                sa_tangent(sa);
                lin1x1(c, op.to_out1, false, XT_(X_O), PS, C, XT_(X_H1), PS, C, H, W, B, XT_(X_H0), PS, false, st);
                launch_ln_tan(XT_(X_H1), PS, XP(X_H1), XP(X_LN2), B, C, T, op.lng[1], XT_(X_A2), PS, st);
                lin1x1(c, op.xqc, false, XT_(X_A2), PS, C, XT_(X_XQ), PS, C, H, W, B, nullptr, 0, false, st);
                if (!xa_fused(xa, 1, XT_(X_XQ), PS, op.xK, op.xV, XP(X_XS), 0, XT_(X_XO), PS)) {
                    xa_scores(xa, XT_(X_XQ), PS, op.xK, XT_(X_XS), PS, 1.f, false);
                    launch_softmax_jac(XT_(X_XS), XP(X_XS), (long)NH * T, xa.Lp, (long)NH * T, xa.scale, st, B, PS);
                    xa_values(xa, op.xV, XT_(X_XS), PS, XT_(X_XO), PS);
                }
                lin1x1(c, op.to_out2, false, XT_(X_XO), PS, C, XT_(X_H2), PS, C, H, W, B, XT_(X_H1), PS, false, st);
                launch_ln_tan(XT_(X_H2), PS, XP(X_H2), XP(X_LN3), B, C, T, op.lng[2], XT_(X_A3), PS, st);
                lin1x1(c, op.ff1, false, XT_(X_A3), PS, C, XT_(X_F), PS, 8 * C, H, W, B, nullptr, 0, false, st);
                launch_geglu(1, XT_(X_F), PS, XP(X_F), B, 4L * C * T, XT_(X_GG), PS, st);
                lin1x1(c, op.ff2, false, XT_(X_GG), PS, 4 * C, XT_(X_H3), PS, C, H, W, B, XT_(X_H2), PS, false, st);
                const StatReq rq = next_tan(op.out);
                lin1x1(c, op.pj_out, false, XT_(X_H3), PS, C, TT(op.out), PS, C, H, W, B, TT(op.in), PS, false, st, &rq);
                break;
            }
            case OP_DOWN: case OP_UP: {
                const Tens& ti = c->tens[op.in];
                ConvArgs a; conv_defaults(a);
                a.in = TT(op.in); a.in_bs = PS; a.Cin = ti.C; a.Hin = ti.H; a.Win = ti.W;
                setw(a, op.conv, false);
                if (op.kind == OP_DOWN) { a.stride = 2; a.pad = op.sym_down ? 1 : 0; } else { a.upsample = 1; }
                a.out = TT(op.out); a.out_bs = PS; a.Cout = to.C; a.Hout = to.H; a.Wout = to.W; a.B = B;
                const StatReq rq = next_tan(op.out);
                run_conv(c, a, 9, st, &rq);
                break;
            }
            case OP_OUT: {
                const Tens& ti = c->tens[op.in];
                if (!op.n1.ready) tangent_stats(c, op.n1, TT(op.in), PS, TP(op.in), ti.H * ti.W, B, st);
                op.n1.ready = false;
                ConvArgs a; conv_defaults(a);
                a.in = TT(op.in); a.in_bs = PS; a.Cin = ti.C; a.Hin = ti.H; a.Win = ti.W;
                setw(a, op.conv, false);
                set_tan(c, a, op.n1, TP(op.in));
                a.out = TT(op.out); a.out_bs = PS; a.Cout = to.C; a.Hout = to.H; a.Wout = to.W; a.B = B;
                run_conv(c, a, 9, st);
                break;
            }
        }
    }
    return 0;
}

void cot_stats(loco_ctx* c, const NormP& n, const float* d, long dbs, const float* x, int HW, int B, int kind,
               hipStream_t st) {
    NS sp = nstats(c, c->statsP, n);
    NS stt = nstats(c, c->statsT, n);
    launch_gn_tstats(d, dbs, x, 0, B, n.C, HW, c->cfg.gn_groups, sp.sc, sp.sh, sp.mr, 0, 0, kind, stt.tst,
                     stt.tc, c->prog->stats_per_sample, c->red, st, c->cfg.act);
}

int cotangent_pass(loco_ctx* c, const float* ge, const float* gx0, float* Aout, int B, hipStream_t st) {
    const loco_unet_cfg& cfg = c->cfg;
    const long PS = c->prog->per_sample;
    const int G = cfg.gn_groups;
    auto TP = [&](int id) { return c->arenaP + c->tens[id].off; };
    auto TG = [&](int id) { return c->arenaT + c->tens[id].off; };
    auto GO = [&](const Op& o) -> const float* { return o.out == c->prog->eps_t ? ge : TG(o.out); };
    auto GOS = [&](const Op& o) -> long { return o.out == c->prog->eps_t ? (long)c->prog->n_out : PS; };
    clear_ready(c);
    for (int oi = (int)c->ops.size() - 1; oi >= 0; --oi) {
        Op& op = c->ops[oi];
        const Tens& to = c->tens[op.out];
        const int HW = to.H * to.W;
        switch (op.kind) {
            case OP_OUT: {
                const Tens& ti = c->tens[op.in];
                ConvArgs a; conv_defaults(a);
                a.in = GO(op); a.in_bs = GOS(op); a.Cin = to.C; a.Hin = to.H; a.Win = to.W;
                setw(a, op.conv, true);
                a.out = TG(op.a1); a.out_bs = PS; a.Cout = ti.C; a.Hout = ti.H; a.Wout = ti.W; a.B = B;
                {
                    const StatReq rq = req_lin(c, ST_COT, &op.n1, TP(op.in));
                    run_conv(c, a, 9, st, &rq);
                    op.n1.ready = false;
                }
                NS sp = nstats(c, c->statsP, op.n1);
                NS stt = nstats(c, c->statsT, op.n1);
                launch_gn_apply(2, TG(op.a1), PS, TP(op.in), 0, nullptr, 0, TG(op.in), PS, 0, B, ti.C, ti.H * ti.W, G,
                                sp.sc, sp.sh, sp.mr, 0, 0, stt.tst, c->prog->stats_per_sample, st, cfg.act);
                break;
            }
            case OP_UP: {
                const Tens& ti = c->tens[op.in];
                ConvArgs a; conv_defaults(a);
                a.in = TG(op.out); a.in_bs = PS; a.Cin = to.C; a.Hin = to.H; a.Win = to.W;
                setw(a, op.conv, true);
                a.out = TG(op.up); a.out_bs = PS; a.Cout = ti.C; a.Hout = to.H; a.Wout = to.W; a.B = B;
                run_conv(c, a, 9, st);
                launch_pool2x2_sum(TG(op.up), PS, TG(op.in), PS, 0, B, ti.C, ti.H, ti.W, st);
                break;
            }
            case OP_DOWN: {
                const Tens& ti = c->tens[op.in];
                ConvArgs a; conv_defaults(a);
                a.in = TG(op.out); a.in_bs = PS; a.Cin = to.C; a.Hin = to.H; a.Win = to.W;
                setw(a, op.conv, true); a.zins = 1; a.pad = op.sym_down ? 1 : 2; a.accumulate = op.in_is_skip ? 1 : 0;
                a.out = TG(op.in); a.out_bs = PS; a.Cout = ti.C; a.Hout = ti.H; a.Wout = ti.W; a.B = B;
                run_conv(c, a, 9, st);
                break;
            }
            case OP_RES: {
                const Tens& ti = c->tens[op.in];
                const int HWi = ti.H * ti.W;
                ConvArgs a; conv_defaults(a);
                a.in = TG(op.out); a.in_bs = PS; a.Cin = to.C; a.Hin = to.H; a.Win = to.W;
                setw(a, op.c2, true);
                a.out = TG(op.h1); a.out_bs = PS; a.Cout = to.C; a.Hout = to.H; a.Wout = to.W; a.B = B;
                {
                    const StatReq rq2 = req_lin(c, ST_COT, &op.n2, TP(op.h1));
                    run_conv(c, a, 9, st, &rq2);
                    op.n2.ready = false;
                }
                ConvArgs b; conv_defaults(b);
                b.in = TG(op.h1); b.in_bs = PS; b.Cin = to.C; b.Hin = to.H; b.Win = to.W;
                setw(b, op.c1, true);
                set_tan(c, b, op.n2, TP(op.h1));
                b.mode = CM_COT_SILU;
                b.out_bs = PS; b.Cout = ti.C; b.Hout = to.H; b.Wout = to.W; b.B = B;
                if (op.updown == 0) {
                    b.out = TG(op.a1);
                    const StatReq rq1 = req_lin(c, ST_COT, &op.n1, TP(op.in));
                    run_conv(c, b, 9, st, &rq1);
                } else if (op.updown == 1) {
                    b.out = TG(op.ap);
                    run_conv(c, b, 9, st);
                    launch_upsample2x(TG(op.ap), PS, TG(op.a1), PS, 0, 0.25f, B, ti.C, to.H, to.W, st);
                } else {
                    b.out = TG(op.xu);
                    run_conv(c, b, 9, st);
                    launch_pool2x2_sum(TG(op.xu), PS, TG(op.a1), PS, 0, B, ti.C, ti.H, ti.W, st);
                }
                if (!op.n1.ready) cot_stats(c, op.n1, TG(op.a1), PS, TP(op.in), HWi, B, 1, st);
                op.n1.ready = false;
                NS sp = nstats(c, c->statsP, op.n1);
                NS stt = nstats(c, c->statsT, op.n1);
                int acc = op.in_is_skip ? 1 : 0;
                const float* gsk = TG(op.out);
                bool cot_in_epilogue = false;
                if (op.has_nin) {
                    ConvArgs n; conv_defaults(n);
                    n.in = TG(op.out); n.in_bs = PS; n.Cin = to.C; n.Hin = to.H; n.Win = to.W;
                    setw(n, op.nin, true); n.pad = 0;
                    n.Cout = ti.C; n.Hout = to.H; n.Wout = to.W; n.B = B; n.out_bs = PS;
                    n.out = TG(op.in); n.accumulate = acc;
                    if (op.updown == 0 && c->prec >= 1 && c->fuse_cot && op.n1.sx_off >= 0 && c->sxcache) {
                        n.cot_d = TG(op.a1); n.cot_d_bs = PS; n.cot_sx = c->sxcache + op.n1.sx_off;
                        n.cot_tc = stt.tc; n.cot_tc_bs = c->prog->stats_per_sample;
                    }
                    cot_in_epilogue = run_conv(c, n, 1, st);
                    gsk = nullptr;
                }
                if (op.updown == 0) {
                    if (cot_in_epilogue) {  }
                    else if (op.has_nin)
                        launch_gn_apply(2, TG(op.a1), PS, TP(op.in), 0, nullptr, 0, TG(op.in), PS, 1, B, ti.C, HWi, G,
                                        sp.sc, sp.sh, sp.mr, 0, 0, stt.tst, c->prog->stats_per_sample, st, cfg.act);
                    else
                        launch_gn_apply(2, TG(op.a1), PS, TP(op.in), 0, gsk, PS, TG(op.in), PS, acc, B, ti.C, HWi, G,
                                        sp.sc, sp.sh, sp.mr, 0, 0, stt.tst, c->prog->stats_per_sample, st, cfg.act, c->prog->res_scale);
                } else {
                    launch_gn_apply(2, TG(op.a1), PS, TP(op.in), 0, nullptr, 0, TG(op.in), PS, acc, B, ti.C, HWi, G,
                                    sp.sc, sp.sh, sp.mr, 0, 0, stt.tst, c->prog->stats_per_sample, st, cfg.act);
                    if (op.updown == 1) launch_upsample2x(gsk, PS, TG(op.in), PS, 1, 0.25f * c->prog->res_scale, B, ti.C, to.H, to.W, st);
                    else launch_pool2x2_sum(gsk, PS, TG(op.in), PS, 1, B, ti.C, ti.H, ti.W, st, c->prog->res_scale);
                }
                break;
            }
            case OP_ATTN: {
                const int C = to.C, T = HW, NH = op.heads, CH = C / NH;
                const long HS = 3L * CH * T, SS = (long)T * T, OS = (long)CH * T;
                float* q = TP(op.qkv); float* k = q + (long)CH * T; float* v = k + (long)CH * T;
                float* gq = TG(op.qkv); float* gk = gq + (long)CH * T; float* gv = gk + (long)CH * T;
                const int so = op.has_x ? op.xmid : op.out;
                if (op.has_x) {
                    const XA x = xa_of(c, op, B, st);
                    xa_conv1x1(c, op.xproj, true, TG(op.out), PS, TG(op.xo), PS, C, to.H, to.W, B, nullptr, 0, false, st);
                    if (!xa_fused(x, 1, TG(op.xo), PS, op.xV, op.xK, TP(op.xS), 0, TG(op.xq), PS)) {
                        xa_scores(x, TG(op.xo), PS, op.xV, TG(op.xS), PS, 1.f, false);
                        launch_softmax_jac(TG(op.xS), TP(op.xS), (long)NH * T, x.Lp, (long)NH * T, x.scale, st, B, PS);
                        xa_values(x, op.xK, TG(op.xS), PS, TG(op.xq), PS);
                    }
                    xa_conv1x1(c, op.xqc, true, TG(op.xq), PS, TG(op.xhn), PS, C, to.H, to.W, B, nullptr, 0, false, st);
                    cot_stats(c, op.nx, TG(op.xhn), PS, TP(op.xmid), HW, B, 2, st);
                    NS spx = nstats(c, c->statsP, op.nx);
                    NS stx = nstats(c, c->statsT, op.nx);
                    launch_gn_apply(3, TG(op.xhn), PS, TP(op.xmid), 0, TG(op.out), PS, TG(op.xmid), PS, 0, B, C, HW, G,
                                    spx.sc, spx.sh, spx.mr, 0, 0, stx.tst, c->prog->stats_per_sample, st);
                }
                ConvArgs pr; conv_defaults(pr);
                pr.in = TG(so); pr.in_bs = PS; pr.Cin = C; pr.Hin = to.H; pr.Win = to.W;
                setw(pr, op.proj, true); pr.pad = 0;
                pr.out = TG(op.o); pr.out_bs = PS; pr.Cout = C; pr.Hout = to.H; pr.Wout = to.W; pr.B = B;
                run_conv(c, pr, 1, st);
                const bool flash = (c->flash_attn && c->prec >= 1 && attn_flash_supported(T, CH)) || op.added_kv;
                if (op.added_kv) akv_cotangent(akv_of(c, op, B, st));
                else if (flash) {
                    AttnFlashArgs fa; std::memset(&fa, 0, sizeof(fa));
                    fa.ws = reinterpret_cast<unsigned char*>(c->partial); fa.ws_bytes = c->partial_floats * sizeof(float);
                    fa.T = T; fa.NH = NH; fa.B = B; fa.CH = CH; fa.scale = 1.0f / std::sqrt((float)CH);
                    fa.q = q; fa.k = k; fa.v = v; fa.hs = HS; fa.P = TP(op.S); fa.o = TP(op.o);
                    fa.go = TG(op.o); fa.bs_go = PS; fa.gq = gq; fa.gk = gk; fa.gv = gv; fa.bs_g = PS; fa.delta = c->attn_delta;
                    launch_attn_flash_cotangent(fa, st);
                }
                GemmArgs g; std::memset(&g, 0, sizeof(g));
                g.A = TG(op.o); g.sam = T; g.sak = 1; g.sab = PS; g.sah = OS;
                g.Bm = TP(op.S); g.sbk = T; g.sbn = 1; g.sbb = 0; g.sbh = SS;
                g.C = gv; g.scm = T; g.scn = 1; g.scb = PS; g.sch = HS;
                g.M = CH; g.N = T; g.K = T; g.batch = B; g.batch2 = NH; g.alpha = 1.f; g.beta = 0.f;
                if (!flash) attn_gemm(c, g, st);
                GemmArgs h; std::memset(&h, 0, sizeof(h));
                h.A = TG(op.o); h.sam = 1; h.sak = T; h.sab = PS; h.sah = OS;
                h.Bm = v; h.sbk = T; h.sbn = 1; h.sbb = 0; h.sbh = HS;
                h.C = TG(op.S); h.scm = T; h.scn = 1; h.scb = PS; h.sch = SS;
                h.M = T; h.N = T; h.K = CH; h.batch = B; h.batch2 = NH; h.alpha = 1.f; h.beta = 0.f;
                if (!flash) {
                attn_gemm(c, h, st);
                launch_softmax_jac(TG(op.S), TP(op.S), (long)NH * T, T, (long)NH * T, 1.0f / std::sqrt((float)CH), st, B, PS);
                }
                GemmArgs gq_; std::memset(&gq_, 0, sizeof(gq_));
                gq_.A = k; gq_.sam = T; gq_.sak = 1; gq_.sab = 0; gq_.sah = HS;
                gq_.Bm = TG(op.S); gq_.sbk = 1; gq_.sbn = T; gq_.sbb = PS; gq_.sbh = SS;
                gq_.C = gq; gq_.scm = T; gq_.scn = 1; gq_.scb = PS; gq_.sch = HS;
                gq_.M = CH; gq_.N = T; gq_.K = T; gq_.batch = B; gq_.batch2 = NH; gq_.alpha = 1.f; gq_.beta = 0.f;
                if (!flash) attn_gemm(c, gq_, st);
                GemmArgs gk_ = gq_;
                gk_.A = q; gk_.Bm = TG(op.S); gk_.sbk = T; gk_.sbn = 1; gk_.C = gk;
                if (!flash) attn_gemm(c, gk_, st);
                ConvArgs a; conv_defaults(a);
                a.in = TG(op.qkv); a.in_bs = PS; a.Cin = 3 * C; a.Hin = to.H; a.Win = to.W;
                setw(a, op.qkvc, true); a.pad = 0;
                a.out = TG(op.hn); a.out_bs = PS; a.Cout = C; a.Hout = to.H; a.Wout = to.W; a.B = B;
                run_conv(c, a, 1, st);
                cot_stats(c, op.n1, TG(op.hn), PS, TP(op.in), HW, B, 2, st);
                NS sp = nstats(c, c->statsP, op.n1);
                NS stt = nstats(c, c->statsT, op.n1);
                launch_gn_apply(3, TG(op.hn), PS, TP(op.in), 0, TG(so), PS, TG(op.in), PS,
                                op.in_is_skip ? 1 : 0, B, C, HW, G, sp.sc, sp.sh, sp.mr, 0, 0, stt.tst, c->prog->stats_per_sample, st);
                break;
            }
            case OP_XFMR: {
                const int C = to.C, T = HW, NH = op.heads, H = to.H, W = to.W;
                auto XP = [&](int i) { return TP(op.xt[i]); };
// ... 660 lines not shown
    launch_latent_sample(moments, noise, scale, z, B, c->prog->n_out / 2, (hipStream_t)stream);
    HIPCHK(c, hipGetLastError());
    return 0;
}

int loco_lincomb(loco_ctx* c, const float* const* src, const float* coef, int32_t n, float* out, int64_t count,
                 void* stream) {
    if (!c) return -2;
    if (n < 1 || n > 4) { c->err = "lincomb: 1..4 terms"; return -2; }
    launch_lincomb(src, coef, n, out, (long)count, (hipStream_t)stream);
    HIPCHK(c, hipGetLastError());
    return 0;
}

int loco_diffedit_mask(loco_ctx* c, const float* eps_a, const float* eps_b, float scale, int32_t B, int32_t C, int64_t HW,
                       int32_t rule, float* m_out, uint8_t* mask_out, void* stream) {
    if (!c) return -2;
    if (!eps_a || !eps_b || !mask_out || B < 1 || C < 1 || HW < 1) { c->err = "diffedit_mask: bad arguments"; return -2; }
    if (rule != 0 && rule != 1) { c->err = "diffedit_mask: rule is 0 (reference) or 1 (intended)"; return -2; }
    float* ws = reinterpret_cast<float*>(c->gscratch);
    const size_t cap = 2 * ((((size_t)c->prog->n_in + 255) / 256) * 64 * 64 + 4096);
    float* m = m_out;
    if (!m) {
        if (1024 + (size_t)HW > cap) { c->err = "diffedit_mask: map larger than the reduction workspace; pass m_out"; return -2; }
        m = ws + 1024;
    }
    hipStream_t st = (hipStream_t)stream;
    launch_diffedit_mask(eps_a, eps_b, scale, B, C, (long)HW, rule, m, mask_out, ws, ws + 768, st);
    HIPCHK(c, hipGetLastError());
    float status[3] = {0.f, 0.f, 0.f};
    HIPCHK(c, hipMemcpyAsync(status, ws + 768, sizeof(status), hipMemcpyDeviceToHost, st));
    HIPCHK(c, hipStreamSynchronize(st));
    if (status[0] == 1.f) {
        c->err = "diffedit_mask: constant map (max == min = " + std::to_string(status[1]) + "): the two noise predictions do not differ";
        return -4;
    }
    if (status[0] != 0.f) { c->err = "diffedit_mask: non-finite map"; return -5; }
    return 0;
}

int loco_cfg_masked_step(loco_ctx* c, const float* x, const float* eps_for, const float* eps_edit, const float* eps_null,
                         float g, float at, float at_next, const uint8_t* mask, int32_t B, int64_t n, float* x_next,
                         void* stream) {
    if (!c) return -2;
    if (!x || !eps_for || !eps_edit || !eps_null || !mask || !x_next || B < 1 || n < 1) {
        c->err = "cfg_masked_step: bad arguments";
        return -2;
    }
    float s1, s2, s3, ce, cn;
    sched_coeffs(at, at_next, 0.f, &s1, &s2, &s3, &ce, &cn);
    launch_cfg_masked_step(x, eps_for, eps_edit, eps_null, mask, x_next, B, (long)n, g, s2, s1, s3, ce, (hipStream_t)stream);
    HIPCHK(c, hipGetLastError());
    return 0;
}

#ifdef LOCO_DIAG
}
__global__ void diag_fill_records(unsigned char* rec, long nrec, int wpitch, unsigned seed, float scale) {
    const long r = (long)blockIdx.x * 256 + threadIdx.x;
    if (r >= nrec) return;
    const int idx = (int)(r % wpitch);
    unsigned short hi[16], lo[16];
    for (int k = 0; k < 16; ++k) {
        unsigned h = (unsigned)(r * 16 + k) * 2654435761u + seed * 40503u;
        h ^= h >> 15; h *= 2246822519u; h ^= h >> 13; h *= 3266489917u; h ^= h >> 16;
        const float v = scale * ((float)(h & 0xffffff) * (1.0f / 8388608.0f) - 1.0f);
        const __bf16 hb = (__bf16)v;
        const __bf16 lb = (__bf16)(v - (float)hb);
        hi[k] = __builtin_bit_cast(unsigned short, hb);
        lo[k] = __builtin_bit_cast(unsigned short, lb);
    }
    const int sw = (idx >> 2) & 3;
    unsigned short* base = reinterpret_cast<unsigned short*>(rec + r * 64);
    for (int k = 0; k < 8; ++k) {
        base[((0 ^ sw) << 3) + k] = hi[k];
        base[((1 ^ sw) << 3) + k] = hi[8 + k];
        base[((2 ^ sw) << 3) + k] = lo[k];
        base[((3 ^ sw) << 3) + k] = lo[8 + k];
    }
}
extern "C" {
int loco_bench_conv(loco_ctx* c, int32_t cin, int32_t cout, int32_t H, int32_t W, int32_t B, int32_t mode,
                    int32_t taps, int32_t tile, int32_t iters, float* ms_avg, void* stream) {
    if (!c) return -2;
    if (finalize_params(c)) return -3;
    hipStream_t st = (hipStream_t)stream;
    const long HW = (long)H * W;
    const long in_e = (long)cin * HW, out_e = (long)cout * HW;
    if ((in_e + out_e) * B > (long)c->cfg.max_batch * c->prog->per_sample || 2 * in_e > (long)c->prog->per_sample ||
        in_e > c->prog->sx_total) { c->err = "bench_conv: shape exceeds the arenas"; return -2; }
    float* in = c->arenaT;
    float* out = c->arenaT + in_e * B;
    const int bz = getenv("LOCO_BENCH_ZERO") ? atoi(getenv("LOCO_BENCH_ZERO")) : 0;
    const float zs = (bz & 1) ? 0.0f : 1.0f, zw = (bz & 2) ? 0.0f : 1.0f;
    launch_fill_random(in, in_e * B, 1u, zs, st);
    launch_fill_random(c->arenaP, in_e, 2u, zs, st);
    launch_fill_random(reinterpret_cast<float*>(c->sxcache), 2 * in_e, 3u, zs, st);
    launch_fill_random(c->statsP, c->prog->stats_per_sample, 4u, 1.0f, st);
    launch_fill_random(c->statsT, c->prog->stats_per_sample * B, 5u, 0.01f, st);
    size_t wfl = (size_t)((cin + 15) / 16) * 16 * taps * ((cout + 31) & ~31);
    if (wfl * 2 > c->partial_floats) { c->err = "bench_conv: weights exceed workspace"; return -2; }
    float* wf = c->partial + c->partial_floats - wfl * 2;
    launch_fill_random(wf, (long)wfl * 2, 6u, 0.05f * zw, st);
    if (c->prec == 1) {
        const long nrec = (long)((cin + 15) / 16) * taps * ((cout + 31) & ~31);
        hipLaunchKernelGGL(diag_fill_records, dim3((unsigned)((nrec + 255) / 256)), dim3(256), 0, st,
                           reinterpret_cast<unsigned char*>(wf), nrec, (cout + 31) & ~31, 7u, 0.05f * zw);
    }
    ConvArgs a; conv_defaults(a);
    a.in = in; a.in_bs = in_e; a.Cin = cin; a.Hin = H; a.Win = W;
    a.prim = c->arenaP; a.prim_bs = 0; a.sx = c->sxcache;
    a.w = wf; a.wb = wf; a.wh = wf;
    a.out = out; a.out_bs = out_e; a.Cout = cout; a.Hout = H; a.Wout = W; a.B = B;
    a.mode = mode; a.pad = taps == 9 ? 1 : 0; a.in_padded = 1; a.taps = taps;
    a.sc = c->statsP; a.sh = c->statsP + cin; a.scsh_bs = 0; a.mr = c->statsP + 2 * cin; a.mr_bs = 0;
    a.gamma_ = c->statsP; a.tst = c->statsT; a.tst_bs = c->prog->stats_per_sample; a.cpg = cin / c->cfg.gn_groups;
    a.tc = c->statsT + 64; a.tc_bs = c->prog->stats_per_sample;
    if (a.cpg < 1) a.cpg = 1;
    a.nsplit = 1; a.partial = c->partial;
    a.partial_floats = c->partial_floats - wfl * 2;
    if (getenv("LOCO_BENCH_COT") && atoi(getenv("LOCO_BENCH_COT")) && taps == 1) {
        if ((in_e + 2 * out_e) * B > (long)c->cfg.max_batch * c->prog->per_sample || out_e > c->prog->sx_total ||
            2L * cout > c->prog->stats_per_sample) { c->err = "bench_conv: cot operands exceed the arenas"; return -2; }
        launch_fill_random(out + out_e * B, out_e * B, 8u, zs, st);
        if (out_e > in_e) launch_fill_random(reinterpret_cast<float*>(c->sxcache), 2 * out_e, 3u, zs, st);
        a.cot_d = out + out_e * B; a.cot_d_bs = out_e; a.cot_sx = c->sxcache; a.cot_tc = c->statsT; a.cot_tc_bs = c->prog->stats_per_sample;
    }
    if (getenv("LOCO_BENCH_ACC") && atoi(getenv("LOCO_BENCH_ACC"))) a.accumulate = 1;
    conv_plan_family(a, c->prec);
    if (const char* e = getenv("LOCO_DUAL_WHATIF")) a.no_deep = atoi(e);
    ConvArgs parts[2];
    const int nparts = conv_plan_parts(a, c->prec, tile, parts);
    auto run = [&]() {
        for (int pi = 0; pi < nparts; ++pi) {
            if (c->prec == 1) launch_conv_bf16x3(parts[pi], taps, st);
            else if (c->prec == 2) launch_conv_f16(parts[pi], taps, st);
            else launch_conv(parts[pi], taps, st);
        }
        launch_conv_splitk_reduce(a, st);
    };
    run();
    HIPCHK(c, hipEventRecord(c->ev0, st));
    for (int i = 0; i < iters; ++i) run();
    HIPCHK(c, hipEventRecord(c->ev1, st));
    HIPCHK(c, hipEventSynchronize(c->ev1));
    c->bench_out = out; c->bench_out_count = (int64_t)out_e * B;
    float ms = 0.f;
    HIPCHK(c, hipEventElapsedTime(&ms, c->ev0, c->ev1));
    *ms_avg = ms / iters;
    HIPCHK(c, hipGetLastError());
    return 0;
}

#endif

int loco_set_streams(loco_ctx* c, int32_t n) {
    if (!c || (n != 1 && n != 2)) return -2;
    c->n_streams = n;
    return 0;
}

int loco_set_chip_share(loco_ctx* c, int32_t n) {
    if (!c || n < 1 || n > 8) return -2;
    c->chip_share = n;
    return 0;
}

int loco_set_side_stream(loco_ctx* c, void* stream) {
    if (!c) return -2;
    c->st2_user = (hipStream_t)stream;
    return 0;
}

int loco_profile_enable(loco_ctx* c, int32_t on) {
    if (!c) return -2;
    c->prof_on = on != 0;
    c->prof_shapes = on == 2;
    if (on) { c->prof.clear(); c->ev_used = 0; }
    return 0;
}

int loco_profile_report(loco_ctx* c, char* buf, int64_t cap) {
    if (!c || !buf || cap < 1) return -2;
    HIPCHK(c, hipDeviceSynchronize());
    std::map<std::string, std::array<double, 3>> agg;
    for (auto& r : c->prof) {
        float ms = 0.f;
        if (hipEventElapsedTime(&ms, r.e0, r.e1) != hipSuccess) continue;
        std::string key = r.name;
        if (c->prof_shapes) {
            char sb[96];
            snprintf(sb, sizeof(sb), "|t%d_m%d_ci%d_co%d_h%d_b%d_s%d", r.taps, r.mode, r.cin, r.cout, r.h, r.b, r.ns);
            key += sb;
        }
        auto& a = agg[key];
        a[0] += 1.0; a[1] += ms; a[2] += r.flops;
    }
    std::string out;
    char line[256];
    for (auto& kv : agg) {
        snprintf(line, sizeof(line), "%s %.0f %.6f %.6e\n", kv.first.c_str(), kv.second[0], kv.second[1], kv.second[2]);
        out += line;
    }
    if ((int64_t)out.size() + 1 > cap) { c->err = "profile buffer too small"; return -4; }
    std::memcpy(buf, out.c_str(), out.size() + 1);
    return 0;
}

#ifdef LOCO_DIAG
int64_t loco_debug_tensor(loco_ctx* c, const char* name, float* dst, int64_t cap, void* stream) {
    if (!c) return -2;
    std::string nm(name);
    if (nm == "bench_out") {
        if (!c->bench_out) { c->err = "no loco_bench_conv yet"; return -3; }
        int64_t cnt = cap < c->bench_out_count ? cap : c->bench_out_count;
        HIPCHK(c, hipMemcpyAsync(dst, c->bench_out, (size_t)cnt * sizeof(float), hipMemcpyDeviceToDevice, (hipStream_t)stream));
        return cnt;
    }
    if (nm == "workspace") {
        int64_t cnt = cap < (int64_t)c->partial_floats ? cap : (int64_t)c->partial_floats;
        HIPCHK(c, hipMemcpyAsync(dst, c->partial, (size_t)cnt * sizeof(float), hipMemcpyDeviceToDevice, (hipStream_t)stream));
        return cnt;
    }
    int arena = 0;
    if (nm.rfind("T:", 0) == 0) { arena = 1; nm = nm.substr(2); }
    bool want_h1 = false;
    if (nm.rfind("h1:", 0) == 0) { want_h1 = true; nm = nm.substr(3); }
    for (auto& op : c->ops) {
        if (op.name != nm) continue;
        int id = want_h1 ? op.h1 : op.out;
        if (id < 0) return -3;
        const Tens& t = c->tens[id];
        int64_t cnt = (int64_t)t.C * t.H * t.W;
        int B = arena ? 1 : (c->primal_B > 0 ? c->primal_B : 1);
        if (cnt * B > cap) { c->err = "debug buffer too small"; return -4; }
        float* base = (arena ? c->arenaT : c->arenaP) + t.off;
        launch_copy(base, c->prog->per_sample, dst, cnt, 0, B, cnt, (hipStream_t)stream);
        return cnt * B;
    }
    c->err = "no such op: " + nm;
    return -3;
}

#endif

}
```

loco-edit_amd/csrc/kernels.h:

```cpp
#pragma once
#include <hip/hip_runtime.h>
#include <stdint.h>

namespace loco {

struct DeviceOnce { bool seen[64] = {}; };
inline bool first_on_device(DeviceOnce& f) {
    int d = 0;
    (void)hipGetDevice(&d);
    d &= 63;
    if (f.seen[d]) return false;
    f.seen[d] = true;
    return true;
}


enum ConvMode : int {
    CM_NONE = 0,
    CM_GN_SILU = 1,
    CM_GN = 2,
    CM_TAN_SILU = 3,
    CM_COT_SILU = 4,
    CM_GN_GELU = 5,
};
enum ActKind : int { ACT_SILU = 0, ACT_GELU = 1 };
__device__ __forceinline__ float act_fwd(float y, int act) {
    if (act == ACT_GELU) return 0.5f * y * (1.0f + erff(y * 0.70710678118654752f));
    return y * (1.0f / (1.0f + __expf(-y)));
}
__device__ __forceinline__ float act_der(float y, int act) {
    if (act == ACT_GELU) return 0.5f * (1.0f + erff(y * 0.70710678118654752f)) + y * 0.39894228040143268f * __expf(-0.5f * y * y);
    const float sg = 1.0f / (1.0f + __expf(-y));
    return sg * (1.0f + y * (1.0f - sg));
}

enum StatKind : int { ST_NONE = 0, ST_FWD = 1, ST_TAN = 2, ST_COT = 3 };

struct ConvArgs {
    const float* in; long in_bs; int Cin, Hin, Win;
    const float* prim; long prim_bs;
    const float* w;
    const void* wb;
    const void* wh;
    const float2* sx;
    float* out; long out_bs; int Cout, Hout, Wout;
    const float* bias;
    const float* bias2; long bias2_bs;
    const float* res; long res_bs;
    const float* sc; const float* sh; long scsh_bs;
    const float* mr; long mr_bs;
    const float* gamma_;
    const float* tst; long tst_bs;
    const float* tc; long tc_bs;
    int cpg;
    int mode;
    int stride;
    int pad;
    int upsample;
    int zins;
    int in_padded;
    int accumulate;
    int nsplit;
    int taps;
    int no_deep;
    float* partial;
    int B;
    float* st_part; int st_kind;
    const float* st_x; const float2* st_sx;
    const float* in2; long in2_bs; int Cin2; int in2_padded;
    const void* wb2;
    const float* cot_d; long cot_d_bs; const float2* cot_sx; const float* cot_tc; long cot_tc_bs;
    int act;
    float res_scale;
    int dual;
    int gemm, gemm_tm;
    size_t partial_floats;
    int pers_groups;
    int tile, pair;
};

void launch_conv(const ConvArgs& a, int taps, hipStream_t st);
void launch_conv_bf16x3(const ConvArgs& a, int taps, hipStream_t st);
void launch_conv_f16(const ConvArgs& a, int taps, hipStream_t st);
void launch_conv_splitk_reduce(const ConvArgs& a, hipStream_t st);

struct ConvEnv {
    int prec = 1;
    int chip_share = 1;
    int lanes = 1, lane_s0 = 0;
    float* partial = nullptr; size_t partial_floats = 0;
    float* stpart = nullptr; size_t stpart_floats = 0;
    bool fuse_stats = true, fuse_lin = true, deep1 = true;
    int max_batch = 1;
};

struct StatAsk {
    int kind = ST_NONE;
    bool norm = false;
    const float2* sx = nullptr;
    const float* prim = nullptr;
    float* keep = nullptr; size_t keep_floats = 0;
};

enum StatRoute : int {
    SR_NONE = 0,
    SR_EPI = 1,
    SR_SPLITK = 2,
    SR_ALONE = 3,
    SR_KEEP = 4,
};

struct ConvLaunch {
    ConvArgs args;
    ConvArgs parts[2]; int nparts = 1;
    int s0 = 0;
    int stats = SR_NONE;
    int ntile = 0;
};

struct ConvPlan {
    bool sc_first = false;
    int nl = 1;
    ConvLaunch l[2];
    bool stats_all = false;
    int keep_ntile = 0;
    bool cot = false;
};

ConvPlan plan_conv(const ConvEnv& env, const ConvArgs& a, int taps, const StatAsk* ask, const ConvArgs* shortcut);
void conv_plan_family(ConvArgs& a, int prec);
int conv_plan_parts(ConvArgs& a, int prec, int tile_override, ConvArgs parts[2]);

int conv_bf16_tile_couts(const ConvArgs& a);
const char* conv_variant_name(const ConvArgs& a, int taps, int prec);

void launch_fill_random(float* p, long count, unsigned seed, float scale, hipStream_t st);
void launch_gn_cache(const float* x, int C, int HW, int cpg, const float* sc, const float* sh, const float* mr,
                     float2* sx, hipStream_t st, int act = 0);

struct GemmArgs {
    const float* A; long sam, sak, sab;
    const float* Bm; long sbk, sbn, sbb;
    float* C; long scm, scn, scb;
    const float* bias;
    const float* colbias;
    const float* R; long srb;
    int M, N, K, batch;
    float alpha, beta;
    int batch2; long sah, sbh, sch;
    const float* A2; long sab2; const float* Bm2; long sbb2;
};
void launch_gemm(const GemmArgs& g, hipStream_t st);
enum GemmAct : int { GEMM_ACT_NONE = 0, GEMM_ACT_QUICK_GELU = 1, GEMM_ACT_GELU = 2 };
void launch_gemm_fixed(const GemmArgs& g, int act, hipStream_t st);
void launch_gemm_bf16x3(const GemmArgs& g, hipStream_t st);
bool gemm_prefers_bf16x3(const GemmArgs& g);
bool gemm_rec_eligible(const GemmArgs& g);
size_t gemm_rec_ws_bytes(const GemmArgs& g);
void launch_gemm_rec(const GemmArgs& g, unsigned char* ws, hipStream_t st);

struct AttnFlashArgs {
    int T, NH, B, CH; float scale;
    const float *q, *k, *v; long hs;
    const float* P;
    const float* o;
    const float *dq, *dk, *dv; long bs_d;
    float* out; long bs_out;
    const float* go; long bs_go;
    float *gq, *gk, *gv; long bs_g;
    float* delta;
    int Lt; const float *kt, *vt;
    unsigned char* ws; size_t ws_bytes;
};
size_t attn_flash_ws_bytes(const AttnFlashArgs& a);
bool attn_flash_supported(int T, int CH);
bool attn_flash_text_supported(int T, int CH, int Lt);
void launch_attn_flash_tangent(const AttnFlashArgs& a, hipStream_t st);
void launch_attn_flash_cotangent(const AttnFlashArgs& a, hipStream_t st);

void launch_ln_fwd(const float* x, long xbs, int B, int C, int T, const float* gamma, const float* beta, float eps, float* y,
                   long ybs, float* stats, long sbs, hipStream_t st);
void launch_ln_tan(const float* dx, long dbs, const float* xprim, const float* sprim, int B, int C, int T, const float* gamma,
                   float* dy, long ybs, hipStream_t st);
void launch_ln_cot(const float* gy, long gbs, const float* xprim, const float* sprim, int B, int C, int T, const float* gamma,
                   const float* base, long base_bs, float* gx, long xbs, hipStream_t st);
struct XAttnArgs {
    int T, NH, B, CH, L, Lp, fwd;
    float alpha;
    const float* X; long x_bs;
    const float* K1; const float* K2;
    float* P; long p_bs;
    float* O; long o_bs;
};
bool xattn_fused_supported(int T, int CH, int L, int Lp);
void launch_xattn_fused(const XAttnArgs& a, hipStream_t st);
void launch_geglu(int kind, const float* in, long in_bs, const float* fprim, int B, long n4, float* out, long out_bs,
                  hipStream_t st);

void launch_gn_stats(const float* x, long bs, int B, int C, int HW, int G, float eps,
                     const float* gamma, const float* beta,
                     float* mr, float* sc, float* sh, long stats_bs, double* scratch, hipStream_t st,
                     const float* ss_scale = nullptr, const float* ss_shift = nullptr);
void launch_gn_fused_finalize_cat(const float* partA, int C1, int ntA, const float* partB, int ntB, int B, int C, int HW, int G,
                                  float eps, const float* gamma, const float* beta, float* mr, float* sc, float* sh,
                                  long stats_bs, hipStream_t st);
void launch_gn_fused_finalize(const float* part, int ntile, int B, int C, int HW, int G, float eps, const float* gamma,
                              const float* beta, float* mr, float* sc, float* sh, long stats_bs, const float* ss_scale,
                              const float* ss_shift, hipStream_t st);
void launch_gn_lin_fused_finalize(int kind, const float* partA, int C1, int ntA, const float* partB, int ntB, int B, int C, int HW,
                                  int G, const float* mr, float* tst, float* tc, long tst_bs, hipStream_t st);
void launch_conv_splitk_reduce_stats(const ConvArgs& a, int kind, int G, float eps, const float* gamma, const float* beta,
                                     float* mr, float* sc, float* sh, long stats_bs, const float* ss_scale,
                                     const float* ss_shift, const float* prim, const float* sc_prim, const float* sh_prim,
                                     const float* mr_prim, float* tst, float* tc, long tst_bs, double* scratch,
                                     hipStream_t st);
void launch_gn_tstats(const float* d, long d_bs, const float* x, long x_bs, int B, int C, int HW, int G,
                      const float* sc, const float* sh, const float* mr, long pbs_c, long pbs_g,
                      int kind, float* tst, float* tc, long tst_bs, double* scratch, hipStream_t st, int act = 0);
void launch_gn_apply(int kind, const float* d, long d_bs, const float* x, long x_bs,
                     const float* base, long base_bs, float* out, long out_bs, int accumulate,
                     int B, int C, int HW, int G, const float* sc, const float* sh, const float* mr,
                     long pbs_c, long pbs_g, const float* tst, long tst_bs, hipStream_t st, int act = 0,
                     float base_scale = 1.0f);

void launch_ctx_groupnorm(const float* tok, int L, int D, int G, float eps, const float* gamma, const float* beta,
                          float* out, hipStream_t st);

void launch_softmax_rows(float* S, long rows, int T, hipStream_t st, int B = 1, long bs = 0);
void launch_softmax_jac(float* dS, const float* P, long rows, int T, long p_rows, float scale, hipStream_t st,
                        int B = 1, long bs = 0);

// ... 55 lines not shown
```

loco-edit_amd/hip.py:

```python
from __future__ import annotations

import ctypes as C
import os
from typing import Dict, Optional

import numpy as np
import torch

from .config import UNetConfig

_LIB_PATH = os.environ.get("LOCO_HIP_LIB") or os.path.join(os.path.dirname(os.path.abspath(__file__)), "libloco_hip.so")
_lib = None

DIAG_SYMBOLS = ["loco_bench_conv", "loco_debug_tensor"]

SYMBOLS = [
    "loco_version", "loco_device_count", "loco_create", "loco_fork", "loco_destroy", "loco_last_error",
    "loco_load_param", "loco_params_missing", "loco_unet_forward", "loco_ddim_step", "loco_sched_step",
    "loco_pmp_primal", "loco_pmp_set_second_mask", "loco_pmp_jvp", "loco_pmp_vjp", "loco_orthonormalize", "loco_qr_rows",
    "loco_convergence", "loco_convergence_rows", "loco_null_project", "loco_edit_axpy", "loco_mask_gather", "loco_mask_count",
    "loco_unet_flops", "loco_workspace_bytes", "loco_clock_stamp", "loco_set_side_stream", "loco_timer_start", "loco_timer_stop",
    "loco_profile_enable", "loco_profile_report", "loco_set_precision", "loco_get_precision", "loco_set_streams", "loco_set_chip_share",
    "loco_set_cond", "loco_set_context", "loco_lincomb", "loco_masked_axpby", "loco_latent_sample",
    "loco_text_create", "loco_text_load_param", "loco_text_params_missing", "loco_text_encode", "loco_text_last_error",
    "loco_text_destroy", "loco_t5_create", "loco_text_encode_masked",
    "loco_diffedit_mask", "loco_cfg_masked_step",
]

DIFFEDIT_RULES = {"reference": 0, "intended": 1}


class LocoCfg(C.Structure):
    _fields_ = [
        ("struct_size", C.c_int32), ("resolution", C.c_int32), ("in_channels", C.c_int32), ("out_ch", C.c_int32), ("ch", C.c_int32),
        ("num_levels", C.c_int32), ("ch_mult", C.c_int32 * 8), ("num_res_blocks", C.c_int32),
        ("num_attn_res", C.c_int32), ("attn_resolutions", C.c_int32 * 8), ("gn_groups", C.c_int32),
        ("gn_eps", C.c_float), ("max_batch", C.c_int32),
        ("arch", C.c_int32), ("num_head_channels", C.c_int32), ("learn_sigma", C.c_int32),
        ("context_dim", C.c_int32), ("context_len", C.c_int32),
        ("scale_shift_norm", C.c_int32), ("resblock_updown", C.c_int32), ("num_heads", C.c_int32),
        ("transformer_depth", C.c_int32),
        ("act", C.c_int32), ("res_scale", C.c_float), ("added_kv", C.c_int32),
    ]


class LocoTextCfg(C.Structure):
    _fields_ = [("vocab", C.c_int32), ("width", C.c_int32), ("layers", C.c_int32), ("heads", C.c_int32), ("ffn", C.c_int32),
                ("positions", C.c_int32), ("act", C.c_int32), ("ln_eps", C.c_float)]


class LocoT5Cfg(C.Structure):
    _fields_ = [("vocab", C.c_int32), ("d_model", C.c_int32), ("d_kv", C.c_int32), ("heads", C.c_int32), ("d_ff", C.c_int32),
                ("layers", C.c_int32), ("positions", C.c_int32), ("buckets", C.c_int32), ("max_distance", C.c_int32),
                ("act", C.c_int32), ("ln_eps", C.c_float)]


def library_path() -> str:
    return _LIB_PATH


def load_library():
    global _lib
    if _lib is not None:
        return _lib
    if not os.path.exists(_LIB_PATH):
        raise RuntimeError(
            f"{_LIB_PATH} not found: build it with `python -c 'import __graft_entry__ as g; g.build()'` "
            "(hipcc --offload-arch=gfx950). There is no CPU fallback.")
    lib = C.CDLL(_LIB_PATH)
    vp, i32, i64, f32 = C.c_void_p, C.c_int32, C.c_int64, C.c_float
    lib.loco_version.restype = C.c_char_p
    lib.loco_device_count.restype = C.c_int
    lib.loco_create.argtypes = [C.POINTER(LocoCfg), C.POINTER(vp)]
    if hasattr(lib, "loco_fork"):
        lib.loco_fork.argtypes = [vp, C.c_int32, C.POINTER(vp)]
    lib.loco_destroy.argtypes = [vp]
    lib.loco_destroy.restype = None
    lib.loco_last_error.argtypes = [vp]
    lib.loco_last_error.restype = C.c_char_p
    lib.loco_load_param.argtypes = [vp, C.c_char_p, vp, C.POINTER(i64), i32, i32]
    lib.loco_params_missing.argtypes = [vp]
    lib.loco_unet_forward.argtypes = [vp, vp, f32, i32, vp, vp]
    lib.loco_ddim_step.argtypes = [vp, vp, f32, f32, f32, f32, vp, i32, vp, vp]
    lib.loco_sched_step.argtypes = [vp, vp, vp, f32, f32, f32, vp, i64, vp, vp, vp]
    lib.loco_pmp_primal.argtypes = [vp, vp, f32, f32, vp, i32, vp]
    lib.loco_pmp_set_second_mask.argtypes = [vp, vp, i32, vp]
    lib.loco_pmp_jvp.argtypes = [vp, vp, i32, vp, vp]
    lib.loco_pmp_vjp.argtypes = [vp, vp, i32, vp, vp]
    lib.loco_orthonormalize.argtypes = [vp, vp, i32, i64, vp, vp]
    lib.loco_qr_rows.argtypes = [vp, vp, i32, i64, vp]
    lib.loco_convergence.argtypes = [vp, vp, vp, i64, f32, vp, vp]
    lib.loco_convergence_rows.argtypes = [vp, vp, vp, i32, i64, f32, vp, vp]
    lib.loco_null_project.argtypes = [vp, vp, i32, vp, i32, i64, vp, vp]
    lib.loco_edit_axpy.argtypes = [vp, vp, vp, C.POINTER(f32), i32, i64, vp, vp]
    lib.loco_mask_gather.argtypes = [vp, vp, i32, vp, vp]
    lib.loco_mask_count.argtypes = [vp]
    lib.loco_mask_count.restype = i64
    lib.loco_clock_stamp.argtypes = [vp, vp, vp]
    lib.loco_set_side_stream.argtypes = [vp, vp]
    lib.loco_unet_flops.argtypes = [vp]
    lib.loco_unet_flops.restype = C.c_double
    lib.loco_workspace_bytes.argtypes = [vp]
    lib.loco_workspace_bytes.restype = i64
    lib.loco_timer_start.argtypes = [vp, vp]
    lib.loco_timer_stop.argtypes = [vp, vp, C.POINTER(f32)]
    lib.loco_set_precision.argtypes = [vp, i32]
    lib.loco_get_precision.argtypes = [vp]
    lib.loco_set_streams.argtypes = [vp, i32]
    lib.loco_set_chip_share.argtypes = [vp, i32]
    lib.loco_set_cond.argtypes = [vp, vp, vp]
    lib.loco_set_context.argtypes = [vp, vp, vp]
    lib.loco_masked_axpby.argtypes = [vp, vp, vp, f32, f32, i32, vp, vp]
    lib.loco_latent_sample.argtypes = [vp, vp, vp, f32, i32, vp, vp]
    lib.loco_lincomb.argtypes = [vp, C.POINTER(vp), C.POINTER(f32), i32, vp, i64, vp]
    lib.loco_diffedit_mask.argtypes = [vp, vp, vp, f32, i32, i32, i64, i32, vp, vp, vp]
    lib.loco_cfg_masked_step.argtypes = [vp, vp, vp, vp, vp, f32, f32, f32, vp, i32, i64, vp, vp]
    lib.loco_profile_enable.argtypes = [vp, i32]
    lib.loco_profile_report.argtypes = [vp, C.c_char_p, i64]
    if hasattr(lib, "loco_text_create"):
        lib.loco_text_create.argtypes = [C.POINTER(LocoTextCfg), i32, i32, C.POINTER(vp)]
        lib.loco_text_load_param.argtypes = [vp, C.c_char_p, vp, C.POINTER(i64), i32]
        lib.loco_text_params_missing.argtypes = [vp]
        lib.loco_text_encode.argtypes = [vp, vp, i32, vp, vp]
        lib.loco_text_last_error.argtypes = [vp]
        lib.loco_text_last_error.restype = C.c_char_p
        lib.loco_text_destroy.argtypes = [vp]
        lib.loco_text_destroy.restype = None
    if hasattr(lib, "loco_t5_create"):
        lib.loco_t5_create.argtypes = [C.POINTER(LocoT5Cfg), i32, i32, C.POINTER(vp)]
        lib.loco_text_encode_masked.argtypes = [vp, vp, C.POINTER(i32), i32, vp, vp]
    if hasattr(lib, "loco_bench_conv"):
        lib.loco_bench_conv.argtypes = [vp, i32, i32, i32, i32, i32, i32, i32, i32, i32, C.POINTER(f32), vp]
        lib.loco_debug_tensor.argtypes = [vp, C.c_char_p, vp, i64, vp]
        lib.loco_debug_tensor.restype = i64
    _lib = lib
    return lib


def _ptr(t: Optional[torch.Tensor]):
    return None if t is None else C.c_void_p(t.data_ptr())


def _stream():
    return C.c_void_p(torch.cuda.current_stream().cuda_stream)


def _chk_dev(t: torch.Tensor, dtype=torch.float32):
    if not t.is_cuda:
        raise ValueError("loco_hip operates on device tensors only")
    if t.dtype != dtype:
        raise ValueError(f"expected {dtype}, got {t.dtype}")
    if not t.is_contiguous():
        raise ValueError("tensor must be contiguous")


def c_cfg(cfg: UNetConfig, max_batch: int) -> LocoCfg:
    c = LocoCfg()
    c.struct_size = C.sizeof(LocoCfg)
    c.resolution, c.in_channels, c.out_ch, c.ch = cfg.resolution, cfg.in_channels, cfg.out_ch, cfg.ch
    c.num_levels = len(cfg.ch_mult)
    for i, m in enumerate(cfg.ch_mult):
        c.ch_mult[i] = m
    c.num_res_blocks = cfg.num_res_blocks
    c.num_attn_res = len(cfg.attn_resolutions)
    for i, r in enumerate(cfg.attn_resolutions):
        c.attn_resolutions[i] = r
    c.gn_groups, c.gn_eps, c.max_batch = cfg.gn_groups, cfg.gn_eps, int(max_batch)
    c.arch = {"ddpm": 0, "adm": 1, "dec": 2, "enc": 3}[cfg.arch]
    c.num_head_channels, c.learn_sigma = cfg.num_head_channels, int(cfg.learn_sigma)
    c.context_dim, c.context_len = cfg.context_dim, cfg.context_len
    c.scale_shift_norm, c.resblock_updown = int(cfg.scale_shift_norm), int(cfg.resblock_updown)
    c.num_heads, c.transformer_depth = cfg.num_heads, cfg.transformer_depth
    c.act, c.res_scale, c.added_kv = {"silu": 0, "gelu": 1}[cfg.act], float(cfg.res_scale), int(cfg.added_kv)
    return c


class LocoEngine:

    def __init__(self, cfg: UNetConfig, max_batch: int = 8, device: Optional[torch.device] = None):
        self.lib = load_library()
        if not torch.cuda.is_available() or self.lib.loco_device_count() < 1:
            raise RuntimeError("loco_hip: no HIP device visible; the hot path has no CPU fallback")
        self.device = torch.device(device if device is not None else "cuda:0")
        torch.cuda.set_device(self.device)
        self.cfg = cfg
        self.max_batch = int(max_batch)
        c = c_cfg(cfg, self.max_batch)
        self._ctx = C.c_void_p()
        rc = self.lib.loco_create(C.byref(c), C.byref(self._ctx))
        if rc != 0:
            msg = self.lib.loco_last_error(self._ctx).decode() if self._ctx else "?"
            raise RuntimeError(f"loco_create failed ({rc}): {msg}")
        self.n = cfg.n
        self.n_out = cfg.n_out

    def fork(self, max_batch: Optional[int] = None) -> "LocoEngine":
        child = object.__new__(LocoEngine)
        child.lib, child.cfg, child.device = self.lib, self.cfg, self.device
        child.max_batch = int(max_batch or self.max_batch)
        child.n, child.n_out = self.n, self.n_out
        for k, v in self.__dict__.items():
            if k not in child.__dict__ and k != "_ctx":
                child.__dict__[k] = v
        child._ctx = C.c_void_p()
        torch.cuda.set_device(self.device)
        rc = self.lib.loco_fork(self._ctx, child.max_batch, C.byref(child._ctx))
        if rc != 0:
            msg = self.lib.loco_last_error(child._ctx).decode() if child._ctx else self.lib.loco_last_error(self._ctx).decode()
            raise RuntimeError(f"loco_fork failed ({rc}): {msg}")
        return child

    def __del__(self):
        try:
            if getattr(self, "_ctx", None):
                self.lib.loco_destroy(self._ctx)
                self._ctx = None
        except Exception:
            pass

    def _check(self, rc, what):
        if rc != 0:
            raise RuntimeError(f"{what} failed ({rc}): {self.lib.loco_last_error(self._ctx).decode()}")

    def load_state_dict(self, sd: Dict[str, "np.ndarray | torch.Tensor"]):
        for name, v in sd.items():
            if self.cfg.encoder_dim > 0 and name.startswith(("encoder_proj.", "encoder_pooling.")):
                continue
            a = v.detach().cpu().numpy() if isinstance(v, torch.Tensor) else np.asarray(v)
            a = np.ascontiguousarray(a, dtype=np.float32)
            shape = (C.c_int64 * a.ndim)(*a.shape)
            rc = self.lib.loco_load_param(self._ctx, name.encode(), a.ctypes.data_as(C.c_void_p), shape, a.ndim, 0)
            self._check(rc, f"loco_load_param({name})")
        miss = self.lib.loco_params_missing(self._ctx)
        if miss != 0:
            raise RuntimeError(f"{miss} parameters missing: {self.lib.loco_last_error(self._ctx).decode()}")

    def _chk_input(self, x: torch.Tensor):
        want = (self.cfg.in_channels, self.cfg.resolution, self.cfg.resolution)
        if x.dim() != 4 or tuple(x.shape[1:]) != want:
            raise ValueError(f"input must be [B, {want[0]}, {want[1]}, {want[2]}], got {tuple(x.shape)}")

    def unet_forward(self, x: torch.Tensor, t: float, out: Optional[torch.Tensor] = None) -> torch.Tensor:
        _chk_dev(x)
        self._chk_input(x)
        if out is not None:
            _chk_dev(out)
            if out.numel() != x.shape[0] * self.n_out:
                raise ValueError(f"out must hold {x.shape[0]} x {self.n_out} elements, got {tuple(out.shape)}")
            eps = out
        elif self.cfg.arch in ("dec", "enc"):
            eps = torch.empty(x.shape[0], self.cfg.out_ch, self.cfg.out_resolution, self.cfg.out_resolution,
                              device=x.device, dtype=torch.float32)
        else:
            eps = torch.empty_like(x)
        self._check(self.lib.loco_unet_forward(self._ctx, _ptr(x), float(t), x.shape[0], _ptr(eps), _stream()),
                    "loco_unet_forward")
        return eps

    def ddim_step(self, x, t, at, at_next, eta=0.0, noise=None, out=None):
        _chk_dev(x)
        self._chk_input(x)
        if noise is not None:
            _chk_dev(noise)
        out = torch.empty_like(x) if out is None else out
        self._check(self.lib.loco_ddim_step(self._ctx, _ptr(x), float(t), float(at), float(at_next), float(eta),
                                            _ptr(noise), x.shape[0], _ptr(out), _stream()), "loco_ddim_step")
        return out

    def sched_step(self, x, et, at, at_next, eta=0.0, noise=None, want_x0=False):
        _chk_dev(x)
        _chk_dev(et)
        out = torch.empty_like(x)
        x0 = torch.empty_like(x) if want_x0 else None
        self._check(self.lib.loco_sched_step(self._ctx, _ptr(x), _ptr(et), float(at), float(at_next), float(eta),
                                             _ptr(noise), x.numel(), _ptr(out), _ptr(x0), _stream()),
                    "loco_sched_step")
        return out, x0

    def pmp_primal(self, x, t, at, mask: Optional[torch.Tensor] = None, use_et: bool = False):
        _chk_dev(x)
        if x.numel() != self.n:
            raise ValueError(f"the linearisation point is one sample of {self.n} elements, got {tuple(x.shape)}")
        m8 = None
        if mask is not None:
            m8 = mask.to(device=x.device, dtype=torch.uint8).contiguous().view(-1)
            if m8.numel() != self.n_out:
                raise ValueError("mask must have C*H*W elements (of the network output)")
# ... 103 lines not shown
            if emb_add.numel() != 4 * self.cfg.ch:
                raise ValueError("conditioning embedding must have 4*ch elements")
        self._check(self.lib.loco_set_cond(self._ctx, _ptr(emb_add), _stream()), "loco_set_cond")

    def set_context(self, tokens: torch.Tensor):
        _chk_dev(tokens)
        if tuple(tokens.shape) != (self.cfg.context_len, self.cfg.context_dim):
            raise ValueError(f"context must be [{self.cfg.context_len}, {self.cfg.context_dim}], got {tuple(tokens.shape)}")
        self._check(self.lib.loco_set_context(self._ctx, _ptr(tokens), _stream()), "loco_set_context")
        torch.cuda.current_stream().synchronize()

    def masked_axpby(self, V: torch.Tensor, E: torch.Tensor, cv: float, ce: float) -> torch.Tensor:
        _chk_dev(V)
        _chk_dev(E)
        out = torch.empty_like(V)
        self._check(self.lib.loco_masked_axpby(self._ctx, _ptr(V), _ptr(E), float(cv), float(ce), V.shape[0], _ptr(out),
                                               _stream()), "loco_masked_axpby")
        return out

    def latent_sample(self, moments: torch.Tensor, noise: Optional[torch.Tensor], scale: float) -> torch.Tensor:
        _chk_dev(moments)
        B, C2, h, w = moments.shape
        if C2 * h * w != self.n_out:
            raise ValueError(f"moments must be [B, {self.cfg.out_ch}, ...] of this encoder, got {tuple(moments.shape)}")
        if noise is not None:
            _chk_dev(noise)
            if tuple(noise.shape) != (B, C2 // 2, h, w):
                raise ValueError(f"noise must be {(B, C2 // 2, h, w)}, got {tuple(noise.shape)}")
        z = torch.empty(B, C2 // 2, h, w, device=moments.device, dtype=torch.float32)
        self._check(self.lib.loco_latent_sample(self._ctx, _ptr(moments), _ptr(noise) if noise is not None else None,
                                                float(scale), B, _ptr(z), _stream()), "loco_latent_sample")
        return z

    def lincomb(self, terms, out: Optional[torch.Tensor] = None) -> torch.Tensor:
        for _, t in terms:
            _chk_dev(t)
        out = torch.empty_like(terms[0][1]) if out is None else out
        n = len(terms)
        ptrs = (C.c_void_p * n)(*[t.data_ptr() for _, t in terms])
        coef = (C.c_float * n)(*[float(c) for c, _ in terms])
        self._check(self.lib.loco_lincomb(self._ctx, ptrs, coef, n, _ptr(out), out.numel(), _stream()), "loco_lincomb")
        return out

    def diffedit_mask(self, eps_a: torch.Tensor, eps_b: torch.Tensor, scale: float, rule: str = "reference",
                      want_map: bool = False):
        _chk_dev(eps_a)
        _chk_dev(eps_b)
        if eps_a.shape != eps_b.shape or eps_a.dim() < 3:
            raise ValueError(f"two [B, C, ...] tensors of one shape, got {tuple(eps_a.shape)} and {tuple(eps_b.shape)}")
        if rule not in DIFFEDIT_RULES:
            raise ValueError(f"rule must be one of {sorted(DIFFEDIT_RULES)}, got {rule!r}")
        B, Cc = eps_a.shape[0], eps_a.shape[1]
        HW = eps_a.numel() // (B * Cc)
        mask = torch.empty(HW, device=eps_a.device, dtype=torch.uint8)
        m = torch.empty(HW, device=eps_a.device, dtype=torch.float32) if want_map else None
        rc = self.lib.loco_diffedit_mask(self._ctx, _ptr(eps_a), _ptr(eps_b), float(scale), B, Cc, HW, DIFFEDIT_RULES[rule],
                                         _ptr(m), _ptr(mask), _stream())
        if rc in (-4, -5):
            raise ValueError(self.lib.loco_last_error(self._ctx).decode())
        self._check(rc, "loco_diffedit_mask")
        return (mask, m) if want_map else mask

    def cfg_masked_step(self, x, ef, ee, en, g: float, at: float, at_next: float, mask: torch.Tensor,
                        out: Optional[torch.Tensor] = None) -> torch.Tensor:
        for t_ in (x, ef, ee, en):
            _chk_dev(t_)
            if t_.shape != x.shape:
                raise ValueError(f"x and the three noise predictions must share a shape, got {tuple(t_.shape)} vs {tuple(x.shape)}")
        _chk_dev(mask, torch.uint8)
        B = x.shape[0]
        n = x.numel() // B
        if mask.numel() != n:
            raise ValueError(f"mask must hold the {n} elements of one frame, got {tuple(mask.shape)}")
        if out is None:
            out = torch.empty_like(x)
        else:
            _chk_dev(out)
            if out.shape != x.shape:
                raise ValueError(f"out must be {tuple(x.shape)}, got {tuple(out.shape)}")
        self._check(self.lib.loco_cfg_masked_step(self._ctx, _ptr(x), _ptr(ef), _ptr(ee), _ptr(en), float(g), float(at),
                                                  float(at_next), _ptr(mask), B, n, _ptr(out), _stream()),
                    "loco_cfg_masked_step")
        return out

    def version(self) -> str:
        return self.lib.loco_version().decode()

    def clock_stamp(self) -> torch.Tensor:
        out = torch.zeros(2, device=self.device, dtype=torch.int64)
        self._check(self.lib.loco_clock_stamp(self._ctx, _ptr(out), _stream()), "loco_clock_stamp")
        return out

    @staticmethod
    def sclk_mhz(stamp0: torch.Tensor, stamp1: torch.Tensor) -> float:
        d = (stamp1 - stamp0).tolist()
        return 100.0 * d[0] / max(d[1], 1)

    def unet_flops(self) -> float:
        return float(self.lib.loco_unet_flops(self._ctx))

    def workspace_bytes(self) -> int:
        return int(self.lib.loco_workspace_bytes(self._ctx))

    def timer_start(self):
        self._check(self.lib.loco_timer_start(self._ctx, _stream()), "loco_timer_start")

    def timer_stop(self) -> float:
        ms = C.c_float()
        self._check(self.lib.loco_timer_stop(self._ctx, _stream(), C.byref(ms)), "loco_timer_stop")
        return float(ms.value)

    PRECISIONS = {"f32": 0, "bf16x3": 1, "f16": 2}

    def set_precision(self, mode: str):
        self._check(self.lib.loco_set_precision(self._ctx, self.PRECISIONS[mode]), "loco_set_precision")

    def set_streams(self, n: int):
        self._check(self.lib.loco_set_streams(self._ctx, int(n)), "loco_set_streams")

    def set_chip_share(self, n: int):
        self._check(self.lib.loco_set_chip_share(self._ctx, int(n)), "loco_set_chip_share")

    def set_side_stream(self, stream: "Optional[torch.cuda.Stream]"):
        self._side_stream = stream
        ptr = C.c_void_p(stream.cuda_stream) if stream is not None else None
        self._check(self.lib.loco_set_side_stream(self._ctx, ptr), "loco_set_side_stream")

    def set_streams_measured(self, n: int):
        if n == 2:
            from .tloco import BranchStreams
            side = BranchStreams._pick(1, self.device)
            if not side:
                self.set_streams(1)
                return 1
            self.set_side_stream(side[0])
        self.set_streams(n)
        return n

    def get_precision(self) -> str:
        m = self.lib.loco_get_precision(self._ctx)
        return {v: k for k, v in self.PRECISIONS.items()}[m]

    def _need_diag(self, sym):
        if not hasattr(self.lib, sym):
            raise RuntimeError(f"{sym} is a diagnostic of include/loco_hip_diag.h: build `make -C loco-edit_amd/csrc diag` "
                               "and set LOCO_HIP_LIB=<repo>/loco-edit_amd/libloco_hip_diag.so")

    def bench_conv(self, cin, cout, H, W, B, mode, taps=9, tile=-1, iters=20) -> float:
        self._need_diag("loco_bench_conv")
        ms = C.c_float()
        self._check(self.lib.loco_bench_conv(self._ctx, cin, cout, H, W, B, mode, taps, tile, iters, C.byref(ms),
                                             _stream()), "loco_bench_conv")
        return float(ms.value)

    def profile_enable(self, on):
        self._check(self.lib.loco_profile_enable(self._ctx, int(on)), "loco_profile_enable")

    def profile_report(self):
        buf = C.create_string_buffer(1 << 18)
        self._check(self.lib.loco_profile_report(self._ctx, buf, len(buf)), "loco_profile_report")
        out = {}
        for line in buf.value.decode().splitlines():
            name, n, ms, fl = line.rsplit(" ", 3)
            out[name] = dict(launches=int(float(n)), ms=float(ms), flops=float(fl))
        return out

    def debug_tensor(self, name: str, numel: int) -> torch.Tensor:
        self._need_diag("loco_debug_tensor")
        dst = torch.empty(numel, device=self.device, dtype=torch.float32)
        got = self.lib.loco_debug_tensor(self._ctx, name.encode(), _ptr(dst), numel, _stream())
        if got < 0:
            raise RuntimeError(f"loco_debug_tensor({name}) failed: {self.lib.loco_last_error(self._ctx).decode()}")
        return dst[:got]


class LocoTextEngine:

    def __init__(self, cfg, max_prompts: int = 8, device: Optional[torch.device] = None):
        self.lib = load_library()
        if not torch.cuda.is_available() or self.lib.loco_device_count() < 1:
            raise RuntimeError("loco_hip: no HIP device visible; the text encoder has no CPU fallback")
        self.device = torch.device(device if device is not None else "cuda:0")
        if self.device.index is None:
            self.device = torch.device("cuda", torch.cuda.current_device())
        self.cfg, self.max_prompts = cfg, int(max_prompts)
        self.is_t5 = hasattr(cfg, "d_kv")
        self._t = C.c_void_p()
        if self.is_t5:
            if cfg.act != "gated-gelu":
                raise ValueError(f"feed_forward_proj {cfg.act!r}: the T5 encoder builds gated-gelu only")
            c = LocoT5Cfg(vocab=cfg.vocab, d_model=cfg.d_model, d_kv=cfg.d_kv, heads=cfg.heads, d_ff=cfg.d_ff, layers=cfg.layers,
                          positions=cfg.positions, buckets=cfg.buckets, max_distance=cfg.max_distance, act=0, ln_eps=cfg.ln_eps)
            rc, what = self.lib.loco_t5_create(C.byref(c), self.device.index, self.max_prompts, C.byref(self._t)), "loco_t5_create"
        else:
            c = LocoTextCfg(vocab=cfg.vocab, width=cfg.width, layers=cfg.layers, heads=cfg.heads, ffn=cfg.ffn,
                            positions=cfg.positions, act={"quick_gelu": 0, "gelu": 1}[cfg.act], ln_eps=cfg.ln_eps)
            rc, what = self.lib.loco_text_create(C.byref(c), self.device.index, self.max_prompts, C.byref(self._t)), "loco_text_create"
        if rc != 0:
            raise RuntimeError(f"{what} failed ({rc}): {self.lib.loco_text_last_error(None).decode()}")

    def __del__(self):
        try:
            if getattr(self, "_t", None):
                self.lib.loco_text_destroy(self._t)
                self._t = None
        except Exception:
            pass

    def _check(self, rc, what):
        if rc != 0:
            raise RuntimeError(f"{what} failed ({rc}): {self.lib.loco_text_last_error(self._t).decode()}")

    def load_params(self, sd: Dict[str, "np.ndarray | torch.Tensor"]):
        if any(isinstance(v, torch.Tensor) and v.is_cuda for v in sd.values()):
            torch.cuda.synchronize()
        for name, v in sd.items():
            t = torch.as_tensor(np.asarray(v) if not isinstance(v, torch.Tensor) else v).detach().to(torch.float32).contiguous()
            if not t.is_cuda:
                t = t.cpu()
            shape = (C.c_int64 * max(t.dim(), 1))(*t.shape)
            self._check(self.lib.loco_text_load_param(self._t, name.encode(), C.c_void_p(t.data_ptr()), shape, t.dim()),
                        f"loco_text_load_param({name})")

    def check_complete(self):
        missing = self.lib.loco_text_params_missing(self._t)
        if missing:
            raise RuntimeError(f"text encoder: {missing} parameters missing ({self.lib.loco_text_last_error(self._t).decode()})")

    def load_state_dict(self, sd: Dict[str, "np.ndarray | torch.Tensor"]):
        self.load_params(sd)
        self.check_complete()

    @property
    def width(self) -> int:
        return self.cfg.d_model if self.is_t5 else self.cfg.width

    def encode_ids(self, ids: torch.Tensor, out: Optional[torch.Tensor] = None, lens=None) -> torch.Tensor:
        ids = torch.as_tensor(ids)
        if ids.dim() != 2 or ids.shape[1] != self.cfg.positions:
            raise ValueError(f"ids must be [n, {self.cfg.positions}], got {tuple(ids.shape)}")
        n = ids.shape[0]
        ids = ids.to(device=self.device, dtype=torch.int32).contiguous()
        if out is None:
            out = torch.empty(n, self.cfg.positions, self.width, device=self.device, dtype=torch.float32)
        _chk_dev(out)
        if tuple(out.shape) != (n, self.cfg.positions, self.width):
            raise ValueError(f"out must be [{n}, {self.cfg.positions}, {self.width}], got {tuple(out.shape)}")
        with torch.cuda.device(self.device):
            if lens is None and not self.is_t5:
                self._check(self.lib.loco_text_encode(self._t, _ptr(ids), n, _ptr(out), _stream()), "loco_text_encode")
            else:
                larr = None
                if lens is not None:
                    lens = [int(v) for v in (lens.tolist() if isinstance(lens, torch.Tensor) else lens)]
                    if len(lens) != n:
                        raise ValueError(f"lens must hold {n} lengths, got {len(lens)}")
                    larr = (C.c_int32 * n)(*lens)
                self._check(self.lib.loco_text_encode_masked(self._t, _ptr(ids), larr, n, _ptr(out), _stream()),
                            "loco_text_encode_masked")
        return out
```

Measured before the change: 19.98 edit-directions/s.

## Add polyphase conv kernels for upsample, zero-insert and pooled-gradient convs

Adds a polyphase bf16x3 MFMA conv kernel that splits nearest-upsample and zero-inserted 3x3 convolutions into four output phases. Each phase uses folded 2x2 (or fewer) effective taps, so MACs on inserted zeros and duplicated pixels are skipped. A gather variant computes the upsample-block cotangent directly at the pooled resolution using 4x4 folded weights. This removes the full-resolution dgrad conv plus the separate pool2x2 sum. The cost is precomputed folded weight buffers, strided scalar stores in the epilogue, and a new code path that must match the reference numerically.

```diff
diff --git a/include/loco_hip_diag.h b/include/loco_hip_diag.h
--- a/include/loco_hip_diag.h
+++ b/include/loco_hip_diag.h
@@ -10,6 +10,9 @@
 
 int64_t loco_debug_tensor(loco_ctx* ctx, const char* name, float* dst, int64_t cap, void* stream);
 
+int  loco_debug_updown_conv(loco_ctx* ctx, int32_t kind, int32_t cin, int32_t cout, int32_t H, int32_t W, int32_t B,
+                            const float* w_host, const float* in_dev, float* out_dev, void* stream);
+
 #ifdef __cplusplus
 }
 #endif
diff --git a/loco-edit_amd/csrc/conv_bf16.hip b/loco-edit_amd/csrc/conv_bf16.hip
--- a/loco-edit_amd/csrc/conv_bf16.hip
+++ b/loco-edit_amd/csrc/conv_bf16.hip
@@ -10,6 +10,7 @@
 template <int PR, int MODE> void launch_pair_b(const ConvArgs& a, hipStream_t st);
 template <int PR, int MODE> void launch_dual_b(const ConvArgs& a, hipStream_t st);
 void launch_conv_gemm(const ConvArgs& a, hipStream_t st);
+void launch_poly_b(const ConvArgs& a, hipStream_t st);
 
 template <int PR>
 static void launch_lowp(const ConvArgs& a, int taps, hipStream_t st) {
@@ -22,6 +23,9 @@
 #endif
     if constexpr (PR == PR_BF16X3) {
         if (taps == 1 && a.gemm) { launch_conv_gemm(a, st); return; }
+    }
+    if constexpr (PR == PR_BF16X3) {
+        if (taps == 9 && a.poly) { launch_poly_b(a, st); return; }
     }
     if (taps == 9 && a.Cin2 > 0) {
         if (a.mode == CM_GN_SILU) launch_kcat_b<PR, CM_GN_SILU>(a, st);
diff --git a/loco-edit_amd/csrc/conv_bf16_inst_l.hip b/loco-edit_amd/csrc/conv_bf16_inst_l.hip
--- /dev/null
+++ b/loco-edit_amd/csrc/conv_bf16_inst_l.hip
@@ -0,0 +1 @@
+#include "conv_poly_kernel.h"
diff --git a/loco-edit_amd/csrc/conv_bf16_kernel.h b/loco-edit_amd/csrc/conv_bf16_kernel.h
--- a/loco-edit_amd/csrc/conv_bf16_kernel.h
+++ b/loco-edit_amd/csrc/conv_bf16_kernel.h
@@ -98,10 +98,10 @@
 }
 
 constexpr int EPI_COT1 = 1, EPI_STATS = 2;
-template <int WM, int WN, int TM, int TN, int EPI = EPI_STATS, class StageRound>
+template <int WM, int WN, int TM, int TN, int EPI = EPI_STATS, int OSTR = 1, class StageRound>
 __device__ __forceinline__ void conv_lowp_epilogue_staged(const ConvArgs& a, StageRound&& stage_round, unsigned char* smem_b, const int co0,
                                                           const int oy0, const int ox0, const int TW, const int tile_id, const int b,
-                                                          const int split);
+                                                          const int split, const int ph = 0);
 template <int WM, int WN, int TM, int TN>
 __device__ __forceinline__ void conv_lowp_epilogue_direct(const ConvArgs& a, f32x16 (&acc)[TM][TN], const int co0, const int oy0,
                                                           const int ox0, const int TW, const int b, const int split);
@@ -124,10 +124,11 @@
     }
     conv_lowp_epilogue_direct<WM, WN, TM, TN>(a, acc, co0, oy0, ox0, TW, b, split);
 }
-template <int WM, int WN, int TM, int TN, int EPI, class StageRound>
+template <int WM, int WN, int TM, int TN, int EPI, int OSTR, class StageRound>
 __device__ __forceinline__ void conv_lowp_epilogue_staged(const ConvArgs& a, StageRound&& stage_round, unsigned char* smem_b, const int co0,
                                                           const int oy0, const int ox0, const int TW, const int tile_id, const int b,
-                                                          const int split) {
+                                                          const int split, const int ph) {
+    static_assert(OSTR == 1 || (OSTR == 2 && !(EPI & EPI_COT1)), "output stride of the staged epilogue");
     constexpr int NTHR = WM * WN * 64;
     constexpr bool COT1 = (EPI & EPI_COT1) != 0, STATS = (EPI & EPI_STATS) != 0;
     constexpr int MT = WM * TM * 32;
@@ -158,7 +159,12 @@
         constexpr int RSTEP = NTHR / NQ;
         static_assert(NTHR % NQ == 0 && 32 % RSTEP == 0, "epilogue task rows");
         const int row0 = tid / NQ, quad0 = tid & (NQ - 1);
-        const unsigned pix0 = (unsigned)((oy0 + ((quad0 * 4) >> twsh)) * a.Wout + ox0 + ((quad0 * 4) & (TW - 1)));
+        const unsigned pix0 = OSTR == 1 ? (unsigned)((oy0 + ((quad0 * 4) >> twsh)) * a.Wout + ox0 + ((quad0 * 4) & (TW - 1)))
+                                        : (unsigned)((2 * (oy0 + ((quad0 * 4) >> twsh)) + (ph >> 1)) * a.Wout + 2 * (ox0 + ((quad0 * 4) & (TW - 1))) + (ph & 1));
+        auto ld4 = [](const float* p) -> f32x4 {
+            if constexpr (OSTR == 1) return *reinterpret_cast<const f32x4*>(p);
+            else return f32x4{p[0], p[2], p[4], p[6]};
+        };
         auto co_of = [&](int h, int q) -> int { return co0 + row0 + (((q * RSTEP) >> 5) * TM + h) * 32 + ((q * RSTEP) & 31); };
         auto off_of = [&](int h, int q) -> unsigned {
             const unsigned crow = (unsigned)((((q * RSTEP) >> 5) * TM + h) * 32 + ((q * RSTEP) & 31));
@@ -196,7 +202,7 @@
                         xs[q][0] = sp4[0];
                         xs[q][1] = sp4[1];
                     } else {
-                        xs[q][0] = *reinterpret_cast<const f32x4*>(a.st_x + o);
+                        xs[q][0] = ld4(a.st_x + o);
                     }
                 }
             }
@@ -209,8 +215,8 @@
 #pragma unroll
                 for (int q = 0; q < NTASK; ++q) {
                     f32x4 t4 = {0.f, 0.f, 0.f, 0.f};
-                    if (rb) t4 = a.res_scale * *reinterpret_cast<const f32x4*>(rb + off_of(h, q));
-                    if (accu) t4 += *reinterpret_cast<const f32x4*>(ob + off_of(h, q));
+                    if (rb) t4 = a.res_scale * ld4(rb + off_of(h, q));
+                    if (accu) t4 += ld4(ob + off_of(h, q));
                     rv[q] = t4;
                 }
 #pragma unroll
@@ -235,7 +241,12 @@
                 if (b1) add += b1[co_of(h, q)];
                 if (b2) add += b2[co_of(h, q)];
                 v[q] += add;
-                __builtin_nontemporal_store(v[q], reinterpret_cast<f32x4*>(ob + off_of(h, q)));
+                if constexpr (OSTR == 1) {
+                    __builtin_nontemporal_store(v[q], reinterpret_cast<f32x4*>(ob + off_of(h, q)));
+                } else {
+                    float* const o4 = ob + off_of(h, q);
+                    o4[0] = v[q][0]; o4[2] = v[q][1]; o4[4] = v[q][2]; o4[6] = v[q][3];
+                }
             }
             if constexpr (STATS) if (lin_st) {
 #pragma unroll
diff --git a/loco-edit_amd/csrc/conv_plan.hip b/loco-edit_amd/csrc/conv_plan.hip
--- a/loco-edit_amd/csrc/conv_plan.hip
+++ b/loco-edit_amd/csrc/conv_plan.hip
@@ -56,7 +56,7 @@
     int tile = conv_bf16_pick_tile(a.Cout, a.Hout * a.Wout, a.B, tile_override);
     if (tile == 4) tile = 5;
     if (tile == 5 && a.taps == 1 && !a.gemm && a.B >= 2 && a.Hout * a.Wout <= kTile0MaxHW) return 0;
-    if (tile == 5 && two_per_cu && a.taps == 9 && a.stride == 1 && !a.upsample && !a.zins && (a.Cin % BKC) == 0 &&
+    if (tile == 5 && two_per_cu && a.taps == 9 && a.stride == 1 && !a.pool2 && !a.upsample && !a.zins && (a.Cin % BKC) == 0 &&
         a.in_padded && a.pad == 1 && a.Wout >= 32) return 6;
     if (a.stride == 2 && tile == 5) tile = 0;
     return tile;
@@ -96,7 +96,7 @@
 
 static bool conv_pair_ok(const ConvArgs& a) {
     static const bool on = env_int("LOCO_CONV_PAIR", 1) != 0;
-    if (!on || a.Hout * a.Wout < 16384 || a.taps != 9 || a.Cin2 > 0 || a.nsplit != 1 || a.stride != 1 || a.upsample || a.zins ||
+    if (!on || a.Hout * a.Wout < 16384 || a.taps != 9 || a.Cin2 > 0 || a.nsplit != 1 || a.stride != 1 || a.upsample || a.zins || a.pool2 ||
         a.pad != 1 || !a.in_padded || (a.Cin % (2 * BKC)) != 0 || (a.Cout % 128) != 0 || (a.Wout % 32) != 0 || (a.Hout % 8) != 0 ||
         a.pers_groups || a.dual)
         return false;
@@ -104,9 +104,25 @@
     return a.tile == 5;
 }
 
+static int conv_poly_ok(const ConvArgs& a) {
+    static const bool on = env_int("LOCO_CONV_POLY", 1) != 0;
+    if (!on || a.taps != 9 || a.stride != 1 || a.Cin2 > 0 || a.nsplit != 1 || a.mode != CM_NONE || !a.in_padded || (a.Cin % BKC) != 0 ||
+        (a.Cout % 128) != 0 || a.pers_groups || a.dual || a.gemm || a.cot_d || a.tile != 5)
+        return 0;
+    if (a.pool2) {
+        return (!a.upsample && !a.zins && a.pad == 1 && a.wb_poly && (a.Wout % 32) == 0 && (a.Hout % 8) == 0 && a.Hin == 2 * a.Hout &&
+                a.Win == 2 * a.Wout) ? 2 : 0;
+    }
+    if ((a.upsample != 0) == (a.zins != 0) || (a.Win % 32) != 0 || (a.Hin % 8) != 0 || a.Hout != 2 * a.Hin || a.Wout != 2 * a.Win ||
+        a.st_kind == ST_COT)
+        return 0;
+    if (a.upsample ? (a.pad != 1 || !a.wb_poly) : (a.pad != 1 && a.pad != 2)) return 0;
+    return 1;
+}
+
 static bool conv_dual_ok(const ConvArgs& a) {
     static const bool on = diag_switch("LOCO_CONV_DUAL") != 0;
-    if (!on || a.taps != 9 || a.Cin2 > 0 || a.nsplit != 1 || a.stride != 1 || a.upsample || a.zins || a.pad != 1 || (a.Cin % BKC) != 0 ||
+    if (!on || a.taps != 9 || a.Cin2 > 0 || a.nsplit != 1 || a.stride != 1 || a.upsample || a.zins || a.pool2 || a.pad != 1 || (a.Cin % BKC) != 0 ||
         !a.in_padded || a.Wout < 32 || (a.Wout % 32) != 0 || (a.Hout % 8) != 0 || (a.Cout % 128) != 0 || a.B < 2 || a.cot_d)
         return false;
     if (!(a.mode == CM_NONE || a.mode == CM_GN_SILU || a.mode == CM_TAN_SILU || a.mode == CM_COT_SILU)) return false;
@@ -135,7 +151,7 @@
 static void conv_pers_plan(ConvArgs& a) {
     a.pers_groups = 0;
     static const int on = diag_switch("LOCO_CONV_PERS");
-    if (!on || a.taps != 9 || a.Cin2 > 0 || a.nsplit != 1 || a.stride != 1 || a.upsample || a.zins || a.pad != 1 || !a.in_padded ||
+    if (!on || a.taps != 9 || a.Cin2 > 0 || a.nsplit != 1 || a.stride != 1 || a.upsample || a.zins || a.pool2 || a.pad != 1 || !a.in_padded ||
         (a.Cin % (2 * BKC)) != 0 || (a.Cout % 128) != 0 || a.B < 2 || a.cot_d || bf16_tile_of(a) != 5)
         return;
     if (!(a.mode == CM_NONE || a.mode == CM_GN_SILU || a.mode == CM_GN_GELU ||
@@ -187,6 +203,7 @@
     a.dual = 0;
     a.tile = tile_for(a, prec, tile_override);
     a.pair = 0;
+    a.poly = 0;
     parts[0] = a;
     int n = 1;
     if (prec == 1 && a.taps == 9 && conv_dual_ok(a)) {
@@ -202,6 +219,7 @@
         ConvArgs& p = parts[i];
         p.tile = tile_for(p, prec, tile_override);
         p.pair = prec == 1 && conv_pair_ok(p);
+        p.poly = prec == 1 ? conv_poly_ok(p) : 0;
     }
     return n;
 }
@@ -303,7 +321,7 @@
     conv_plan_family(a, e.prec);
     a.tile = tile_for(a, e.prec, -1);
     int split = 1;
-    const int tail = e.prec >= 1 && a.nsplit == 1 && a.B >= 2 && !a.gemm && !a.pers_groups ? tail_split(a, e.partial_floats, &split) : 0;
+    const int tail = e.prec >= 1 && a.nsplit == 1 && a.B >= 2 && !a.gemm && !a.pers_groups && !a.pool2 ? tail_split(a, e.partial_floats, &split) : 0;
     const bool want = q && q->kind != ST_NONE && e.prec >= 1 && e.fuse_stats;
     if (!tail) {
         p.l[0] = plan_launch(e, q, want, a, 0, a.B, &p.keep_ntile);
@@ -325,7 +343,7 @@
 const char* conv_variant_name(const ConvArgs& a, int taps, int prec) {
     static const char* tiles[6] = {"2,2,2,2", "4,1,1,2", "1,4,1,1", "2,2,1,1", "2,2,2,4", "2,4,2,2"};
     static char names[3][2][6][6][56];
-    static char others[5][3][6][40];
+    static char others[6][3][6][40];
     const int mode = (a.mode < 0 || a.mode > 5) ? 2 : a.mode;
     const char* other = nullptr;
     int k = 0, v = mode;
@@ -334,6 +352,7 @@
     else if (prec == 1 && taps == 9 && a.pers_groups > 0 && !a.dual) { k = 2; other = "conv_pers_bf16x3<9,2,4,2,2,%d>"; }
     else if (prec == 1 && taps == 9 && a.pair) { k = 3; other = "conv_pair_bf16x3<%d>"; }
     else if (prec == 1 && taps == 9 && a.dual) { k = 4; other = "conv_dual_bf16x3<%d>"; }
+    else if (prec == 1 && taps == 9 && a.poly) { k = 5; other = "conv_mfma_bf16x3<9,2,4,2,2,%d,poly>"; }
     if (other) {
         char* n = others[k][prec][v];
         if (!n[0]) snprintf(n, 40, other, v);
diff --git a/loco-edit_amd/csrc/conv_poly.h b/loco-edit_amd/csrc/conv_poly.h
--- /dev/null
+++ b/loco-edit_amd/csrc/conv_poly.h
@@ -0,0 +1,56 @@
+#pragma once
+
+#if defined(__HIPCC__)
+#define LOCO_POLY_HD __host__ __device__ inline
+#else
+#define LOCO_POLY_HD inline
+#endif
+
+namespace loco {
+
+LOCO_POLY_HD int poly_axis(const int upsample, const int pad, const int p, int k[2], int d[2]) {
+    if (upsample) { k[0] = 0; k[1] = 1; d[0] = p - 1; d[1] = p; return 2; }
+    if ((p + pad) & 1) { k[0] = k[1] = 1; d[0] = d[1] = (p - pad + 1) >> 1; return 1; }
+    k[0] = 0; k[1] = 2; d[0] = (p - pad) >> 1; d[1] = (p - pad + 2) >> 1;
+    return 2;
+}
+
+LOCO_POLY_HD int poly_up_set(const int p, const int j, int k[2]) {
+    if (p == 0) {
+        if (j == 0) { k[0] = k[1] = 0; return 1; }
+        k[0] = 1; k[1] = 2; return 2;
+    }
+    if (j == 0) { k[0] = 0; k[1] = 1; return 2; }
+    k[0] = k[1] = 2; return 1;
+}
+
+template <class T, class F>
+inline T poly_up_weight(F w, const int ph, const int jy, const int jx) {
+    int ky[2], kx[2];
+    const int ny = poly_up_set(ph >> 1, jy, ky), nx = poly_up_set(ph & 1, jx, kx);
+    double s = 0.0;
+    for (int a = 0; a < ny; ++a)
+        for (int b = 0; b < nx; ++b) s += (double)w(ky[a], kx[b]);
+    return (T)s;
+}
+
+LOCO_POLY_HD void poly_gather_axis(const int p, int a[2], int d[2]) {
+    if (p == 0) { a[0] = 1; d[0] = 0; a[1] = 3; d[1] = 1; }
+    else { a[0] = 0; d[0] = -1; a[1] = 2; d[1] = 0; }
+}
+LOCO_POLY_HD int poly_gather_set(const int a, int k[2]) {
+    if (a == 0) { k[0] = k[1] = 0; return 1; }
+    if (a == 3) { k[0] = k[1] = 2; return 1; }
+    k[0] = a - 1; k[1] = a; return 2;
+}
+template <class T, class F>
+inline T poly_gather_weight(F wd, const int a, const int b) {
+    int ky[2], kx[2];
+    const int ny = poly_gather_set(a, ky), nx = poly_gather_set(b, kx);
+    double s = 0.0;
+    for (int i = 0; i < ny; ++i)
+        for (int j = 0; j < nx; ++j) s += (double)wd(ky[i], kx[j]);
+    return (T)s;
+}
+
+}
diff --git a/loco-edit_amd/csrc/conv_poly_kernel.h b/loco-edit_amd/csrc/conv_poly_kernel.h
--- /dev/null
+++ b/loco-edit_amd/csrc/conv_poly_kernel.h
@@ -0,0 +1,283 @@
+#pragma once
+#include "conv_bf16_kernel.h"
+#include "conv_poly.h"
+
+namespace loco {
+
+constexpr int PP_NTHR = 512, PP_MT = 128, PP_NT = 256;
+constexpr int PP_HW = 34, PP_HSZ = 340;
+constexpr int PP_HBYTES = (PP_HSZ + NDUMMY) * 80;
+constexpr int PP_TAPB = PP_MT * 64;
+constexpr int PP_WBYTES = 4 * PP_TAPB;
+constexpr int PP_LDS = 2 * PP_WBYTES + 2 * PP_HBYTES;
+
+template <bool GATHER>
+__global__ __launch_bounds__(PP_NTHR, 1) void conv_poly_bf16x3(ConvArgs a) {
+    constexpr int PR = PR_BF16X3;
+    extern __shared__ __attribute__((aligned(16))) unsigned char smem_b[];
+    unsigned char* const Wsb = smem_b;
+    unsigned char* const Hsb = smem_b + 2 * PP_WBYTES;
+
+    const int tid = threadIdx.x, lane = tid & 63, wave = tid >> 6;
+    const int l31 = lane & 31, khalf = lane >> 5;
+    const int wm = wave >> 2, wn = wave & 3;
+
+    const int CH = GATHER ? a.Hout : a.Hin, CW = GATHER ? a.Wout : a.Win;
+    int tile_id, cot_id, zid;
+    {
+        const int ntile = (CH * CW) / PP_NT, ncot = a.Cout / PP_MT, Z = GATHER ? a.B : a.B * 4;
+        const int NTC = ntile * ncot, L = blockIdx.x;
+        int T = 0;
+        if ((ntile & 7) == 0) {
+            int q = L >> 3, q2, t8;
+            idivmod_small(q, ncot, q2, cot_id);
+            idivmod_small(q2, Z, t8, zid);
+            tile_id = t8 * 8 + (L & 7);
+        } else {
+            if ((NTC & 7) == 0) { int q = L >> 3, t8; idivmod_small(q, Z, t8, zid); T = t8 * 8 + (L & 7); }
+            else idivmod_small(L, Z, T, zid);
+            idivmod_small(T, ntile, cot_id, tile_id);
+        }
+        tile_id = __builtin_amdgcn_readfirstlane(tile_id);
+        cot_id = __builtin_amdgcn_readfirstlane(cot_id);
+        zid = __builtin_amdgcn_readfirstlane(zid);
+    }
+    const int tiles_x = CW >> 5;
+    int ty0_, tx0_;
+    idivmod_small(tile_id, tiles_x, ty0_, tx0_);
+    const int oy0 = __builtin_amdgcn_readfirstlane(ty0_ * 8);
+    const int ox0 = __builtin_amdgcn_readfirstlane(tx0_ * 32);
+    const int co0 = cot_id * PP_MT;
+    const int b = GATHER ? zid : zid >> 2, ph = GATHER ? 0 : zid & 3;
+    const int nch = a.Cin >> 4;
+    const int nv = GATHER ? nch * 4 : nch;
+    const long in_plane = (long)a.Hin * a.Win;
+
+    auto taps_of = [&](const int p4, int (&h)[4], int (&w)[4]) -> int {
+        int ky[2], dy[2], kx[2], dx[2];
+        int ny = 2, nx = 2;
+        if constexpr (GATHER) {
+            poly_gather_axis(p4 >> 1, ky, dy);
+            poly_gather_axis(p4 & 1, kx, dx);
+        } else {
+            ny = poly_axis(a.upsample, a.pad, p4 >> 1, ky, dy);
+            nx = poly_axis(a.upsample, a.pad, p4 & 1, kx, dx);
+        }
+        auto hof = [&](int iy, int ix) { return (1 + dy[iy]) * PP_HW + 1 + dx[ix]; };
+        auto wof = [&](int iy, int ix) {
+            return GATHER ? ky[iy] * 4 + kx[ix] : (a.upsample ? p4 * 4 + ky[iy] * 2 + kx[ix] : ky[iy] * 3 + kx[ix]);
+        };
+        h[0] = hof(0, 0); w[0] = wof(0, 0);
+        h[1] = nx == 2 ? hof(0, 1) : hof(1, 0); w[1] = nx == 2 ? wof(0, 1) : wof(1, 0);
+        h[2] = hof(1, 0); w[2] = wof(1, 0);
+        h[3] = hof(1, 1); w[3] = wof(1, 1);
+        return ny * nx;
+    };
+    int th[4], tw[4];
+    int ntap = taps_of(ph, th, tw);
+    const int tpc = (GATHER || a.upsample) ? 16 : 9;
+
+    typedef __attribute__((address_space(3))) unsigned char lds_u8;
+    typedef const __attribute__((address_space(1))) unsigned char glb_u8;
+    const int wpitch = (a.Cout + 31) & ~31;
+    const unsigned wtap = (unsigned)wpitch * 64u;
+    const unsigned wrel = (unsigned)(co0 + (tid >> 2)) * 64u + (unsigned)((tid & 3) << 4);
+    const unsigned char* const wgb = reinterpret_cast<const unsigned char*>((GATHER || a.upsample) ? a.wb_poly : a.wb);
+    auto dma_w = [&](const int v, unsigned char* const Wd) {
+        int hh[4], ww[4];
+        const int chunk = GATHER ? v >> 2 : v;
+        const int nt = GATHER ? taps_of(v & 3, hh, ww) : ntap;
+#pragma unroll
+        for (int t = 0; t < 4; ++t)
+            if (t < nt)
+                __builtin_amdgcn_global_load_lds((glb_u8*)(wgb + (unsigned)(chunk * tpc + (GATHER ? ww[t] : tw[t])) * wtap + wrel),
+                                                 (lds_u8*)(Wd + t * PP_TAPB + wave * 1024), 16, 0, 0);
+    };
+    dma_w(0, Wsb);
+
+    int v_q4 = (tid >> 3) & 3;
+    unsigned v_pm = 0, v_goff;
+    int v_rec[4];
+    bool v_shl = false, v_shr = false;
+    {
+        const int hi_ = tid >> 5;
+        int hq_, hr_;
+        idivmod_small(hi_, 3, hq_, hr_);
+        const int sg = hr_ * 4 + (tid & 3), hy = hq_ * 2 + ((tid >> 2) & 1);
+        const bool have = hi_ < 15 && sg < 9 && hy < 10;
+        if (!have) v_q4 = 0;
+        int v_voff = 0, v_cnt = 0, v_pos0 = 0;
+        if (have) {
+            const int Y = oy0 - 1 + hy, X0 = ox0 - 1 + 4 * sg;
+            const bool rowok = (Y >= 0 && Y < CH);
+            v_pos0 = hy * PP_HW + 4 * sg;
+            v_cnt = PP_HW - 4 * sg < 4 ? PP_HW - 4 * sg : 4;
+            if constexpr (GATHER) {
+                v_shl = rowok && X0 < 0;
+                v_shr = rowok && 2 * X0 + 8 > 2 * CW;
+                v_voff = rowok ? 2 * Y * a.Win + 2 * X0 + (v_shl ? 2 : 0) - (v_shr ? 6 : 0) : 0;
+            } else {
+                v_voff = rowok ? Y * a.Win + X0 : 0;
+            }
+#pragma unroll
+            for (int pxi = 0; pxi < 4; ++pxi)
+                if (rowok && X0 + pxi >= 0 && X0 + pxi < CW && pxi < v_cnt) v_pm |= 1u << pxi;
+        }
+#pragma unroll
+        for (int pxi = 0; pxi < 4; ++pxi) v_rec[pxi] = pxi < v_cnt ? v_pos0 + pxi : PP_HSZ + (tid & (NDUMMY - 1));
+        v_goff = (unsigned)(((long)v_q4 * 4 * in_plane + v_voff + 16) * 4);
+    }
+    const float* const inb = a.in + (long)b * a.in_bs;
+    f32x4 dq[GATHER ? 8 : 4];
+    auto prefetch_hv = [&](const int chunk, const int p) {
+        const char* pk = reinterpret_cast<const char*>(inb - 16) + (unsigned)chunk * (64u * (unsigned)in_plane);
+        const unsigned pl = (unsigned)in_plane * 4u;
+        if constexpr (GATHER) {
+            pk += (unsigned)(p * a.Win) * 4u;
+#pragma unroll
+            for (int kk = 0; kk < 4; ++kk) {
+                dq[2 * kk] = *reinterpret_cast<const f32x4_u*>(pk + v_goff + (unsigned)kk * pl);
+                dq[2 * kk + 1] = *reinterpret_cast<const f32x4_u*>(pk + v_goff + (unsigned)kk * pl + 16);
+            }
+        } else {
+#pragma unroll
+            for (int kk = 0; kk < 4; ++kk) dq[kk] = *reinterpret_cast<const f32x4_u*>(pk + v_goff + (unsigned)kk * pl);
+        }
+    };
+    auto stage_hv = [&](unsigned char* const Hd, auto qtag) {
+        constexpr int Q = decltype(qtag)::value;
+        const int oct = v_q4 >> 1, half = v_q4 & 1;
+        float r[4][4];
+#pragma unroll
+        for (int kk = 0; kk < 4; ++kk) {
+            if constexpr (GATHER) {
+                const float w0 = dq[2 * kk][Q], w1 = dq[2 * kk][2 + Q], w2 = dq[2 * kk + 1][Q], w3 = dq[2 * kk + 1][2 + Q];
+                r[0][kk] = v_shr ? w3 : w0;
+                r[1][kk] = v_shl ? w0 : w1;
+                r[2][kk] = v_shl ? w1 : w2;
+                r[3][kk] = v_shl ? w2 : w3;
+            } else {
+#pragma unroll
+                for (int pxi = 0; pxi < 4; ++pxi) r[pxi][kk] = dq[kk][pxi];
+            }
+        }
+#pragma unroll
+        for (int pxi = 0; pxi < 4; ++pxi) {
+            const bool on = ((v_pm >> pxi) & 1u) != 0;
+            uint2 h, l;
+            cvt2<PR>(on ? r[pxi][0] : 0.0f, on ? r[pxi][1] : 0.0f, h.x, l.x);
+            cvt2<PR>(on ? r[pxi][2] : 0.0f, on ? r[pxi][3] : 0.0f, h.y, l.y);
+            unsigned char* dst = Hd + hrec_off<PR>(v_rec[pxi], oct) + half * 8;
+            *reinterpret_cast<uint2*>(dst) = h;
+            *reinterpret_cast<uint2*>(dst + 32) = l;
+        }
+    };
+    using Q0 = std::integral_constant<int, 0>;
+    using Q1 = std::integral_constant<int, 1>;
+
+    struct Frag { s16x8 ah[2], al[2], bh[2], bl[2]; };
+    int aoff_hi[2], aoff_lo[2], hbyte[2];
+#pragma unroll
+    for (int i = 0; i < 2; ++i) {
+        const int p = (wm * 2 + i) * 32 + l31;
+        aoff_hi[i] = rec_off<PR>(p, khalf);
+        aoff_lo[i] = rec_off<PR>(p, 2 + khalf);
+    }
+#pragma unroll
+    for (int j = 0; j < 2; ++j) hbyte[j] = hrec_off<PR>((wn * 2 + j) * PP_HW + l31, khalf);
+    auto load_frag = [&](Frag& f, const unsigned char* const Wc, const unsigned char* const Hc, const int t) {
+#pragma unroll
+        for (int i = 0; i < 2; ++i) {
+            f.ah[i] = *reinterpret_cast<const s16x8*>(Wc + t * PP_TAPB + aoff_hi[i]);
+            f.al[i] = *reinterpret_cast<const s16x8*>(Wc + t * PP_TAPB + aoff_lo[i]);
+        }
+#pragma unroll
+        for (int j = 0; j < 2; ++j) {
+            const unsigned char* hp = Hc + th[t] * 80 + hbyte[j];
+            f.bh[j] = *reinterpret_cast<const s16x8*>(hp);
+            f.bl[j] = *reinterpret_cast<const s16x8*>(hp + 32);
+        }
+    };
+    f32x16 acc[2][2];
+#pragma unroll
+    for (int i = 0; i < 2; ++i)
+#pragma unroll
+        for (int j = 0; j < 2; ++j)
+#pragma unroll
+            for (int r = 0; r < 16; ++r) acc[i][j][r] = 0.0f;
+    auto mma_frag = [&](const Frag& f) {
+#pragma unroll
+        for (int i = 0; i < 2; ++i)
+#pragma unroll
+            for (int j = 0; j < 2; ++j) {
+                const bf16x8 ah = __builtin_bit_cast(bf16x8, f.ah[i]), al = __builtin_bit_cast(bf16x8, f.al[i]);
+                const bf16x8 bh = __builtin_bit_cast(bf16x8, f.bh[j]), bl = __builtin_bit_cast(bf16x8, f.bl[j]);
+                acc[i][j] = __builtin_amdgcn_mfma_f32_32x32x16_bf16(al, bh, acc[i][j], 0, 0, 0);
+                acc[i][j] = __builtin_amdgcn_mfma_f32_32x32x16_bf16(ah, bl, acc[i][j], 0, 0, 0);
+                acc[i][j] = __builtin_amdgcn_mfma_f32_32x32x16_bf16(ah, bh, acc[i][j], 0, 0, 0);
+            }
+    };
+
+    prefetch_hv(0, 0);
+    stage_hv(Hsb, Q0{});
+    asm volatile("s_waitcnt vmcnt(0)" ::: "memory");
+    if (nv > 1) {
+        dma_w(1, Wsb + PP_WBYTES);
+        if constexpr (!GATHER) prefetch_hv(1, 0);
+    }
+    asm volatile("s_waitcnt lgkmcnt(0)" ::: "memory");
+    __builtin_amdgcn_s_barrier();
+
+    for (int v = 0; v < nv; ++v) {
+        unsigned char* const Wc = Wsb + (v & 1) * PP_WBYTES;
+        unsigned char* const Hc = Hsb + (v & 1) * PP_HBYTES;
+        unsigned char* const Hn = Hsb + ((v + 1) & 1) * PP_HBYTES;
+        if constexpr (GATHER) ntap = taps_of(v & 3, th, tw);
+        Frag f0, f1;
+        load_frag(f0, Wc, Hc, 0);
+        if (ntap > 1) load_frag(f1, Wc, Hc, 1);
+        mma_frag(f0);
+        if (ntap > 2) load_frag(f0, Wc, Hc, 2);
+        if (v + 1 < nv) {
+            if (GATHER && !(v & 1)) stage_hv(Hn, Q1{});
+            else stage_hv(Hn, Q0{});
+        }
+        if (ntap > 1) mma_frag(f1);
+        if (ntap > 2) {
+            load_frag(f1, Wc, Hc, 3);
+            mma_frag(f0);
+            mma_frag(f1);
+        }
+        asm volatile("s_waitcnt vmcnt(0)" ::: "memory");
+        asm volatile("s_waitcnt lgkmcnt(0)" ::: "memory");
+        __builtin_amdgcn_s_barrier();
+        asm volatile("" ::: "memory");
+        if (v + 2 < nv) {
+            dma_w(v + 2, Wc);
+            if constexpr (GATHER) { if (!(v & 1)) prefetch_hv((v + 2) >> 2, ((v + 2) >> 1) & 1); }
+            else prefetch_hv(v + 2, 0);
+        }
+    }
+    auto stage_round = [&](const int h, float* S) {
+#pragma unroll
+        for (int j = 0; j < 2; ++j)
+#pragma unroll
+            for (int r = 0; r < 16; ++r)
+                S[(wm * 32 + (r & 3) + 8 * (r >> 2) + 4 * khalf) * PP_NT + (wn * 2 + j) * 32 + l31] = acc[h][j][r];
+    };
+    if constexpr (GATHER) conv_lowp_epilogue_staged<2, 4, 2, 2, EPI_STATS, 1>(a, stage_round, smem_b, co0, oy0, ox0, 32, tile_id, b, 0);
+    else conv_lowp_epilogue_staged<2, 4, 2, 2, EPI_STATS, 2>(a, stage_round, smem_b, co0, oy0, ox0, 32, tile_id * 4 + ph, b, 0, ph);
+}
+
+void launch_poly_b(const ConvArgs& a, hipStream_t st) {
+    const bool gather = a.poly == 2;
+    void (*kern)(ConvArgs) = gather ? &conv_poly_bf16x3<true> : &conv_poly_bf16x3<false>;
+    static DeviceOnce once[2];
+    if (first_on_device(once[gather]))
+        (void)hipFuncSetAttribute(reinterpret_cast<const void*>(kern), hipFuncAttributeMaxDynamicSharedMemorySize, 160 * 1024);
+    const int coarse = gather ? a.Hout * a.Wout : a.Hin * a.Win;
+    dim3 grid((coarse / PP_NT) * (a.Cout / PP_MT) * a.B * (gather ? 1 : 4));
+    hipLaunchKernelGGL(kern, grid, dim3(PP_NTHR), PP_LDS, st, a);
+}
+
+}
diff --git a/loco-edit_amd/csrc/engine.hip b/loco-edit_amd/csrc/engine.hip
--- a/loco-edit_amd/csrc/engine.hip
+++ b/loco-edit_amd/csrc/engine.hip
@@ -18,6 +18,7 @@
 #include "../../include/loco_hip_diag.h"
 #endif
 #include "kernels.h"
+#include "conv_poly.h"
 #include "program.h"
 
 using namespace loco;
@@ -41,6 +42,8 @@
     float* wbd = nullptr;
     float* whf = nullptr;
     float* whd = nullptr;
+    float* wbu = nullptr;
+    float* wbg = nullptr;
     float* bias = nullptr;
     int cin = 0, cout = 0, taps = 0;
 };
@@ -259,7 +262,7 @@
 }
 
 int make_conv(loco_ctx* c, const std::vector<const HostParam*>& ws, const std::vector<const HostParam*>& bs,
-              ConvP* out, int row_limit = -1) {
+              ConvP* out, int row_limit = -1, bool up_poly = false) {
     int cin = (int)ws[0]->shape[1], k = ws[0]->shape.size() > 2 ? (int)ws[0]->shape[2] : 1;
     int taps = ws[0]->shape.size() == 4 ? k * k : k;
     int cout = 0;
@@ -292,13 +295,25 @@
     std::vector<float> rf = build_records(cin, cout, taps, fwd);
     std::vector<float> rd = build_records(cout, cin, taps, dgr);
     if (upload(c, &out->wbf, rf) || upload(c, &out->wbd, rd)) return -1;
+    if (up_poly && taps == 9) {
+        auto up = [&](int o, int i, int t) {
+            return poly_up_weight<float>([&](int ky, int kx) { return fwd(o, i, ky * 3 + kx); }, t >> 2, (t >> 1) & 1, t & 1);
+        };
+        std::vector<float> ru = build_records(cin, cout, 16, up);
+        if (upload(c, &out->wbu, ru)) return -1;
+        auto gat = [&](int o, int i, int t) {
+            return poly_gather_weight<float>([&](int ky, int kx) { return dgr(o, i, ky * 3 + kx); }, t >> 2, t & 3);
+        };
+        std::vector<float> rg = build_records(cout, cin, 16, gat);
+        if (upload(c, &out->wbg, rg)) return -1;
+    }
     std::vector<float> hf = build_records_f16(cin, cout, taps, fwd);
     std::vector<float> hd = build_records_f16(cout, cin, taps, dgr);
     if (upload(c, &out->whf, hf) || upload(c, &out->whd, hd)) return -1;
     return 0;
 }
-int make_conv1(loco_ctx* c, const std::string& name, ConvP* out, int row_limit = -1) {
-    return make_conv(c, {&c->params[name + ".weight"]}, {&c->params[name + ".bias"]}, out, row_limit);
+int make_conv1(loco_ctx* c, const std::string& name, ConvP* out, int row_limit = -1, bool up_poly = false) {
+    return make_conv(c, {&c->params[name + ".weight"]}, {&c->params[name + ".bias"]}, out, row_limit, up_poly);
 }
 int make_conv1_scaled(loco_ctx* c, const std::string& name, ConvP* out, float s) {
     if (s == 1.f) return make_conv1(c, name, out);
@@ -404,7 +419,7 @@
                 }
                 break;
             }
-            case OP_DOWN: case OP_UP: if (make_conv1(c, op.pn_conv, &ow.conv)) return -1; break;
+            case OP_DOWN: case OP_UP: if (make_conv1(c, op.pn_conv, &ow.conv, -1, op.kind == OP_UP)) return -1; break;
             case OP_XFMR: {
                 const int C = c->tens[op.in].C, NH = op.heads, CH = C / NH;
                 const std::string b = op.name + ".transformer_blocks.0";
@@ -557,19 +572,27 @@
     }
 }
 
+ConvEnv conv_env(const loco_ctx* c) {
+    ConvEnv e;
+    e.prec = c->prec; e.chip_share = c->chip_share; e.lanes = c->lanes_active; e.lane_s0 = c->lane_s0;
+    e.partial = c->partial; e.partial_floats = c->partial_floats; e.stpart = c->stpart; e.stpart_floats = c->stpart_floats;
+    e.fuse_stats = c->fuse_stats; e.fuse_lin = c->fuse_lin; e.deep1 = c->deep1; e.max_batch = c->cfg.max_batch;
+    return e;
+}
+bool arena_padded(const loco_ctx* c, const float* p) {
+    const size_t span = (size_t)c->cfg.max_batch * c->prog->per_sample;
+    return (p >= c->arenaP && p < c->arenaP + span) || (p >= c->arenaT && p < c->arenaT + span);
+}
+
 bool run_conv(loco_ctx* c, const ConvArgs& a0, int taps, hipStream_t st, const StatReq* rq = nullptr,
               const ConvArgs* second = nullptr) {
-    const size_t span = (size_t)c->cfg.max_batch * c->prog->per_sample;
-    auto padded = [&](const float* p) { return (p >= c->arenaP && p < c->arenaP + span) || (p >= c->arenaT && p < c->arenaT + span); };
+    auto padded = [&](const float* p) { return arena_padded(c, p); };
     ConvArgs a = a0, sc;
     a.act = c->cfg.act;
     if (a.mode == CM_GN_SILU && c->cfg.act == ACT_GELU) a.mode = CM_GN_GELU;
     a.in_padded = padded(a.in);
     if (second) { sc = *second; sc.in_padded = padded(sc.in); }
-    ConvEnv e;
-    e.prec = c->prec; e.chip_share = c->chip_share; e.lanes = c->lanes_active; e.lane_s0 = c->lane_s0;
-    e.partial = c->partial; e.partial_floats = c->partial_floats; e.stpart = c->stpart; e.stpart_floats = c->stpart_floats;
-    e.fuse_stats = c->fuse_stats; e.fuse_lin = c->fuse_lin; e.deep1 = c->deep1; e.max_batch = c->cfg.max_batch;
+    const ConvEnv e = conv_env(c);
     StatAsk q;
     if (rq) {
         q.kind = rq->kind; q.norm = rq->n != nullptr; q.prim = rq->prim; q.keep = rq->keep; q.keep_floats = rq->keep_floats;
@@ -599,6 +622,7 @@
             const ConvArgs& y = l.parts[pi];
             double flops = 2.0 * (y.Cin * taps + y.Cin2) * y.Cout * (double)y.Hout * y.Wout * y.B;
             if (y.zins) flops *= 0.25;
+            if (y.pool2) flops *= 4.0;
             timed(c->prof_on ? conv_variant_name(y, taps, c->prec) : nullptr, flops, y, [&] {
                 if (c->prec == 1) launch_conv_bf16x3(y, taps, st);
                 else if (c->prec == 2) launch_conv_f16(y, taps, st);
@@ -633,10 +657,27 @@
     return p.cot;
 }
 
+void run_up_cotangent(loco_ctx* c, const ConvArgs& a, float* up, long up_bs, float* out, long out_bs, hipStream_t st) {
+    const int Hc = a.Hin / 2, Wc = a.Win / 2;
+    if (c->prec == 1 && a.wb_poly) {
+        ConvArgs g = a;
+        g.pool2 = 1; g.out = out; g.out_bs = out_bs; g.Hout = Hc; g.Wout = Wc;
+        ConvArgs t = g;
+        t.act = c->cfg.act; t.in_padded = arena_padded(c, t.in);
+        const ConvPlan p = plan_conv(conv_env(c), t, 9, nullptr, nullptr);
+        if (p.nl == 1 && p.l[0].nparts == 1 && p.l[0].parts[0].poly == 2) { run_conv(c, g, 9, st); return; }
+    }
+    ConvArgs f = a;
+    f.out = up; f.out_bs = up_bs;
+    run_conv(c, f, 9, st);
+    launch_pool2x2_sum(up, up_bs, out, out_bs, 0, a.B, a.Cout, Hc, Wc, st);
+}
+
 inline void setw(ConvArgs& a, const ConvP& p, bool dgrad) {
     a.w = dgrad ? p.wd : p.wf;
     a.wb = dgrad ? (const void*)p.wbd : (const void*)p.wbf;
     a.wh = dgrad ? (const void*)p.whd : (const void*)p.whf;
+    a.wb_poly = dgrad ? (const void*)p.wbg : (const void*)p.wbu;
 }
 
 NormP* consumer_norm(loco_ctx* c, int tid) {
@@ -1458,8 +1499,7 @@
                 a.in = TG(op.out); a.in_bs = PS; a.Cin = to.C; a.Hin = to.H; a.Win = to.W;
                 setw(a, op.conv, true);
                 a.out = TG(op.up); a.out_bs = PS; a.Cout = ti.C; a.Hout = to.H; a.Wout = to.W; a.B = B;
-                run_conv(c, a, 9, st);
-                launch_pool2x2_sum(TG(op.up), PS, TG(op.in), PS, 0, B, ti.C, ti.H, ti.W, st);
+                run_up_cotangent(c, a, TG(op.up), PS, TG(op.in), PS, st);
                 break;
             }
             case OP_DOWN: {
@@ -2426,6 +2466,47 @@
     return 0;
 }
 
+int loco_debug_updown_conv(loco_ctx* c, int32_t kind, int32_t cin, int32_t cout, int32_t H, int32_t W, int32_t B,
+                           const float* w_host, const float* in_dev, float* out_dev, void* stream) {
+    if (!c || kind < 0 || kind > 3 || !w_host || !in_dev || !out_dev || B < 1) return -2;
+    if (finalize_params(c)) return -3;
+    hipStream_t st = (hipStream_t)stream;
+    HostParam w, zb;
+    w.shape = {cout, cin, 3, 3};
+    w.data.assign(w_host, w_host + (size_t)cout * cin * 9);
+    zb.shape = {cout};
+    zb.data.assign((size_t)cout, 0.f);
+    ConvP cp;
+    if (make_conv(c, {&w}, {&zb}, &cp, -1, true)) return -1;
+    const long lo = (long)H * W, hi = 4 * lo;
+    const long in_e = kind == 0 ? cin * lo : (kind == 3 ? cout * hi : cout * lo);
+    const long out_e = kind == 0 ? cout * hi : (kind == 3 ? cin * lo : cin * hi);
+    const long up_e = kind == 3 ? cin * hi : 0;
+    if ((in_e + out_e + up_e) * B > (long)c->cfg.max_batch * c->prog->per_sample) { c->err = "debug_updown_conv: shape exceeds the arena"; return -2; }
+    float* in = c->arenaT;
+    float* out = in + in_e * B;
+    float* up = out + out_e * B;
+    HIPCHK(c, hipMemcpyAsync(in, in_dev, (size_t)in_e * B * sizeof(float), hipMemcpyDeviceToDevice, st));
+    ConvArgs a; conv_defaults(a);
+    a.in = in; a.in_bs = in_e; a.B = B;
+    if (kind == 0) {
+        a.Cin = cin; a.Hin = H; a.Win = W; setw(a, cp, false); a.upsample = 1;
+        a.out = out; a.out_bs = out_e; a.Cout = cout; a.Hout = 2 * H; a.Wout = 2 * W;
+    } else if (kind == 3) {
+        a.Cin = cout; a.Hin = 2 * H; a.Win = 2 * W; setw(a, cp, true);
+        a.out = up; a.out_bs = up_e; a.Cout = cin; a.Hout = 2 * H; a.Wout = 2 * W;
+    } else {
+        a.Cin = cout; a.Hin = H; a.Win = W; setw(a, cp, true); a.zins = 1; a.pad = kind == 2 ? 1 : 2;
+        a.out = out; a.out_bs = out_e; a.Cout = cin; a.Hout = 2 * H; a.Wout = 2 * W;
+    }
+    if (kind == 3) run_up_cotangent(c, a, up, up_e, out, out_e, st);
+    else run_conv(c, a, 9, st);
+    HIPCHK(c, hipMemcpyAsync(out_dev, out, (size_t)out_e * B * sizeof(float), hipMemcpyDeviceToDevice, st));
+    HIPCHK(c, hipStreamSynchronize(st));
+    HIPCHK(c, hipGetLastError());
+    return 0;
+}
+
 #endif
 
 int loco_set_streams(loco_ctx* c, int32_t n) {
diff --git a/loco-edit_amd/csrc/kernels.h b/loco-edit_amd/csrc/kernels.h
--- a/loco-edit_amd/csrc/kernels.h
+++ b/loco-edit_amd/csrc/kernels.h
@@ -77,6 +77,9 @@
     size_t partial_floats;
     int pers_groups;
     int tile, pair;
+    int poly;
+    const void* wb_poly;
+    int pool2;
 };
 
 void launch_conv(const ConvArgs& a, int taps, hipStream_t st);
diff --git a/loco-edit_amd/hip.py b/loco-edit_amd/hip.py
--- a/loco-edit_amd/hip.py
+++ b/loco-edit_amd/hip.py
@@ -12,7 +12,7 @@
 _LIB_PATH = os.environ.get("LOCO_HIP_LIB") or os.path.join(os.path.dirname(os.path.abspath(__file__)), "libloco_hip.so")
 _lib = None
 
-DIAG_SYMBOLS = ["loco_bench_conv", "loco_debug_tensor"]
+DIAG_SYMBOLS = ["loco_bench_conv", "loco_debug_tensor", "loco_debug_updown_conv"]
 
 SYMBOLS = [
     "loco_version", "loco_device_count", "loco_create", "loco_fork", "loco_destroy", "loco_last_error",
@@ -133,6 +133,8 @@
         lib.loco_bench_conv.argtypes = [vp, i32, i32, i32, i32, i32, i32, i32, i32, i32, C.POINTER(f32), vp]
         lib.loco_debug_tensor.argtypes = [vp, C.c_char_p, vp, i64, vp]
         lib.loco_debug_tensor.restype = i64
+    if hasattr(lib, "loco_debug_updown_conv"):
+        lib.loco_debug_updown_conv.argtypes = [vp, i32, i32, i32, i32, i32, i32, vp, vp, vp, vp]
     _lib = lib
     return lib
 
@@ -542,6 +544,20 @@
         self._check(self.lib.loco_bench_conv(self._ctx, cin, cout, H, W, B, mode, taps, tile, iters, C.byref(ms),
                                              _stream()), "loco_bench_conv")
         return float(ms.value)
+
+    def debug_updown_conv(self, kind: int, w: torch.Tensor, x: torch.Tensor) -> torch.Tensor:
+        self._need_diag("loco_debug_updown_conv")
+        w = w.detach().to("cpu", torch.float32).contiguous()
+        x = x.to(self.device, torch.float32).contiguous()
+        cout, cin = int(w.shape[0]), int(w.shape[1])
+        B, _, h, wd = (int(v) for v in x.shape)
+        H, W = (h // 2, wd // 2) if kind == 3 else (h, wd)
+        oc, oh, ow = (cout, 2 * H, 2 * W) if kind == 0 else ((cin, H, W) if kind == 3 else (cin, 2 * H, 2 * W))
+        assert int(x.shape[1]) == (cin if kind == 0 else cout)
+        out = torch.empty(B, oc, oh, ow, device=self.device, dtype=torch.float32)
+        self._check(self.lib.loco_debug_updown_conv(self._ctx, kind, cin, cout, H, W, B, C.c_void_p(w.data_ptr()), _ptr(x), _ptr(out),
+                                                    _stream()), "loco_debug_updown_conv")
+        return out
 
     def profile_enable(self, on):
         self._check(self.lib.loco_profile_enable(self._ctx, int(on)), "loco_profile_enable")
```

Measured after the change: 20.16 edit-directions/s (median of 6 runs). Within noise of the previous version (+0.9%).
